# wgurecky/bipymc

Hardware: AMD Instinct MI355X
Metric: chain-updates/sec (higher is better)
Workload: dtype f64

## Files before the change

bipymc_amd/csrc/kernels.h:

```cpp
#pragma once
#ifndef __HIPCC_RTC__
#include <hip/hip_runtime.h>
#include <stdint.h>
#endif

#include "philox.h"
#include "accept_test.h"
#ifndef BPM_ACCEPT_FILTER_DIVERGENT
#define BPM_ACCEPT_FILTER_DIVERGENT 0
#endif

#ifdef BPM_STAMPS
#define BPM_STAMP(i)                                                                          \
    do {                                                                                      \
        __builtin_amdgcn_sched_barrier(0);                                                    \
        unsigned long long _t;                                                                \
        asm volatile("s_memtime %0\n\ts_waitcnt lgkmcnt(0)" : "=s"(_t)::"memory");            \
        __builtin_amdgcn_sched_barrier(0);                                                    \
        bpm_stamp[i] = _t;                                                                    \
    } while (0)
#else
#define BPM_STAMP(i) do { } while (0)
#endif

#if defined(__HIP_DEVICE_COMPILE__) && !defined(__gfx942__) && !defined(__gfx950__)
#error "kernels.h: the ticket hand-overs rely on gfx942 / gfx950 memory behaviour (vmcnt counts stores; agent-scope atomics bypass the L2s): use __ATOMIC_RELEASE / __ATOMIC_ACQUIRE tickets on other targets"
#endif

namespace bpm {
inline namespace BPM_VARIANT_NS {

constexpr int ALGO_DEMC = 0, ALGO_DREAM = 1;
constexpr int TARGET_HOST = 0, TARGET_GAUSS = 1, TARGET_MIXTURE = 2, TARGET_BANANA = 3;
constexpr int STAGE_FUSED = 0, STAGE_PROPOSE = 1, STAGE_COMMIT = 2;
constexpr int WAVE = 64;
#ifndef BPM_BLOCK_WAVE
#define BPM_BLOCK_WAVE 128
#endif
constexpr int block_for(int lpc) { return (lpc == 4 || lpc == 16) ? 256 : BPM_BLOCK_WAVE; }
constexpr bool hot_is_adapt(int hot) { return hot == 3 || hot == 4; }
constexpr bool crp_shape(int lpc, int dpl) { return lpc < WAVE || dpl == 2; }
constexpr int block_for_hot(int lpc, int hot, int dpl) { return (lpc == WAVE && dpl == 2 && hot_is_adapt(hot)) ? 1024 : block_for(lpc); }
constexpr int cr_g1(int lpc) { return lpc == WAVE ? 16 : WAVE / lpc; }
constexpr int MAX_CR = 8;
constexpr int TRACE_I32 = 32;
constexpr int TRACE_F64 = 4;
constexpr int MAX_PARTNERS = 2 * MAX_PAIRS + 3;

struct Layout {
    double* G;
    uint64_t blk;
    uint32_t n_local;
    uint32_t ld;
    uint32_t dim;
    uint32_t world;
    uint32_t magic;
};

__device__ __forceinline__ uint32_t rank_of(const Layout& L, uint32_t c) {
    if (L.world == 1) return 0u;
    uint32_t r = __umulhi(c, L.magic);
    r -= (r * L.n_local > c) ? 1u : 0u;
    return r;
}
__device__ __forceinline__ double* row_ptr(const Layout& L, uint32_t c) {
    return L.G + (c * L.ld + rank_of(L, c) * (2u * L.n_local));
}
__device__ __forceinline__ double* delta_ptr(const Layout& L, uint32_t c) {
    return L.G + (c + rank_of(L, c) * (L.n_local * (L.ld + 1u)) + L.n_local * L.ld);
}
__device__ __forceinline__ double* cridx_ptr(const Layout& L, uint32_t c) {
    return L.G + (c + rank_of(L, c) * (L.n_local * (L.ld + 1u)) + L.n_local * (L.ld + 1u));
}

constexpr int ACC_SHARDS = 1024;
template <int TARGET, int LPC>
constexpr bool lean_scalars() { return LPC < WAVE && TARGET != TARGET_HOST; }
template <int TARGET>
constexpr bool lean_always() { return TARGET == TARGET_BANANA; }

constexpr int PLAN_WORDS = 16;
constexpr int MAX_SEG = 16;
constexpr int MAX_PEERS = MAX_SEG - 1;

constexpr unsigned long long PUSH_CLOSING = 1ull << 62;
constexpr unsigned long long PUSH_ERR_CLOSED = 0x100ull;
struct PushCtrl {
    unsigned long long flag[MAX_SEG];
    unsigned long long err;
    unsigned long long arena_bad[2];
    unsigned long long pad[5];
    unsigned long long probe[MAX_SEG];
};
struct PhaseArgs {
    Layout L;
    double* ll;
    double* hist_row;
    double* llhist_row;
    double* w_mean;
    double* w_m2;
    const double* tparams;
    const double* cr_state;
    unsigned long long* counters;
    uint32_t* acc_count;
    double* prop_buf;
    double* aux_buf;
    int32_t* ids_buf;
#ifdef BPM_TEST_HOOKS
    int32_t* trace_i32;
    double* trace_f64;
    uint8_t* trace_mask;
#endif
    PermKey pk;
    const uint32_t* perm_tab;
    const uint32_t* inv_tab;
    const double* gamma_tab;
    const uint32_t* plan;
    const uint32_t* rec_tab;
    uint32_t rec_off;
    uint32_t thr[MAX_CR];
    unsigned long long* stamps;
    double* pack;
    uint32_t pack_cap, pack_nsub, pack_stride;
    double* x_next;
    uint8_t* accbits;
    const uint8_t* accbits_all;
    uint32_t replay;
    const uint32_t* rec_sorted;
    uint32_t seg_off[MAX_SEG + 1];
    uint32_t n_seg, seg_me;
    uint32_t acc_by_item;
    const unsigned long long* peer_tab;
    uint32_t n_peers;
    uint32_t hist_by_pos;
#ifndef BPM_LEAN_LAST
    uint32_t lean;
#endif
    uint32_t wt;
    uint64_t seed;
    uint64_t t;
    uint32_t k;
    uint32_t N, lo;
    uint32_t upd_off, n_upd, pool_off, M;
    uint32_t mode;
    uint32_t n_items;
    uint32_t algo;
    uint32_t P, n_cr;
    double* cr_part1;
    const double* cr_fold_part;
    const double* cr_fold_tot;
    double* cr_fold_out;
    uint32_t cr_fold_nb;
    uint32_t cr_chunk0, cr_n1;
    uint32_t adapt_on;
    uint32_t cr_gate;
    uint32_t hist_len;
    double gamma_scale, gamma_demc, epsilon, u_epsilon, p_snooker;
#ifdef BPM_LEAN_LAST
    uint32_t lean, pad_lean;
#endif
};

#ifdef BPM_TEST_HOOKS
__host__ __device__ __forceinline__ int32_t* trace_i32_of(const PhaseArgs& a) { return a.trace_i32; }
__host__ __device__ __forceinline__ double* trace_f64_of(const PhaseArgs& a) { return a.trace_f64; }
__host__ __device__ __forceinline__ uint8_t* trace_mask_of(const PhaseArgs& a) { return a.trace_mask; }
__host__ __device__ __forceinline__ void trace_set(PhaseArgs& a, int32_t* i, double* f, uint8_t* m) { a.trace_i32 = i; a.trace_f64 = f; a.trace_mask = m; }
#else
__host__ __device__ constexpr int32_t* trace_i32_of(const PhaseArgs&) { return nullptr; }
__host__ __device__ constexpr double* trace_f64_of(const PhaseArgs&) { return nullptr; }
__host__ __device__ constexpr uint8_t* trace_mask_of(const PhaseArgs&) { return nullptr; }
__host__ __device__ __forceinline__ void trace_set(PhaseArgs&, int32_t*, double*, uint8_t*) {}
#endif

template <int CTRL>
__device__ __forceinline__ int dpp_i32(int v) {
    return __builtin_amdgcn_mov_dpp(v, CTRL, 0xF, 0xF, true);
}
template <int CTRL>
__device__ __forceinline__ double dpp_f64(double v) {
    const int lo = dpp_i32<CTRL>(__double2loint(v));
    const int hi = dpp_i32<CTRL>(__double2hiint(v));
    return __hiloint2double(hi, lo);
}
__device__ __forceinline__ double readlane_f64(double v, int lane) {
    return __hiloint2double(__builtin_amdgcn_readlane(__double2hiint(v), lane),
                            __builtin_amdgcn_readlane(__double2loint(v), lane));
}
constexpr int DPP_ROW_BCAST15 = 0x142, DPP_ROW_BCAST31 = 0x143;
__device__ __forceinline__ double row_sums_step1_f64(double v) { return v + dpp_f64<DPP_ROW_BCAST15>(v); }
__device__ __forceinline__ double row_sums_step2_f64(double v) { return v + dpp_f64<DPP_ROW_BCAST31>(v); }
__device__ __forceinline__ double row_sums_f64(double v) {
    return readlane_f64(row_sums_step2_f64(row_sums_step1_f64(v)), WAVE - 1);
}
template <int LPC>
__device__ __forceinline__ double gsum(double v) {
    static_assert(LPC == 1 || LPC == 4 || LPC == 16 || LPC == 32 || LPC == 64, "subgroup sizes");
    if (LPC >= 4) {
        v += dpp_f64<0xB1>(v);
        v += dpp_f64<0x4E>(v);
    }
    if (LPC >= 16) {
        v += dpp_f64<0x141>(v);
        v += dpp_f64<0x140>(v);
    }
    if (LPC == 32) v += __shfl_xor(v, 16);
    if (LPC == 64) v = row_sums_f64(v);
    return v;
}
template <int LPC>
__device__ __forceinline__ void gsum2(double& v, double& w) {
    static_assert(LPC == 1 || LPC == 4 || LPC == 16 || LPC == 32 || LPC == 64, "subgroup sizes");
    if (LPC >= 4) {
        const double v1 = dpp_f64<0xB1>(v), w1 = dpp_f64<0xB1>(w);
        v += v1; w += w1;
        const double v2 = dpp_f64<0x4E>(v), w2 = dpp_f64<0x4E>(w);
        v += v2; w += w2;
    }
    if (LPC >= 16) {
        const double v3 = dpp_f64<0x141>(v), w3 = dpp_f64<0x141>(w);
        v += v3; w += w3;
        const double v4 = dpp_f64<0x140>(v), w4 = dpp_f64<0x140>(w);
        v += v4; w += w4;
    }
    if (LPC == 32) { const double vs = __shfl_xor(v, 16), ws = __shfl_xor(w, 16); v += vs; w += ws; }
    if (LPC == 64) {
        v = row_sums_step1_f64(v); w = row_sums_step1_f64(w);
        v = row_sums_step2_f64(v); w = row_sums_step2_f64(w);
        v = readlane_f64(v, WAVE - 1); w = readlane_f64(w, WAVE - 1);
    }
}
template <int LPC>
__device__ __forceinline__ int gsum_i(int v) {
    if (LPC >= 4) {
        v += dpp_i32<0xB1>(v);
        v += dpp_i32<0x4E>(v);
    }
    if (LPC >= 16) {
        v += dpp_i32<0x141>(v);
        v += dpp_i32<0x140>(v);
    }
    if (LPC == 32) v += __shfl_xor(v, 16);
    if (LPC == 64) {
        v += dpp_i32<DPP_ROW_BCAST15>(v);
        v += dpp_i32<DPP_ROW_BCAST31>(v);
        v = __builtin_amdgcn_readlane(v, WAVE - 1);
    }
    return v;
}

constexpr uint32_t CR_FINAL_MAX = 512;
__host__ __device__ inline uint32_t cr_chunks_of(uint32_t n_half, uint32_t g1) { return (n_half + g1 - 1u) / g1; }
struct CrTotals { double p[MAX_CR], d[MAX_CR], n[MAX_CR]; };
__device__ __forceinline__ void cr_finalize(bool any, uint32_t n_cr, CrTotals& T) {
    if (!any) return;
    uint32_t nz = 0;
#pragma unroll
    for (int m = 0; m < MAX_CR; ++m) nz += (m < (int)n_cr && T.n[m] != 0.0) ? 1u : 0u;
    if (nz == n_cr) {
#pragma unroll
        for (int m = 0; m < MAX_CR; ++m) if (m < (int)n_cr) T.p[m] = T.d[m] / T.n[m];
    }
    double sum = 0.0;
#pragma unroll
    for (int m = 0; m < MAX_CR; ++m) if (m < (int)n_cr) sum += T.p[m];
#pragma unroll
    for (int m = 0; m < MAX_CR; ++m) if (m < (int)n_cr) T.p[m] = T.p[m] / sum;
}
template <int ROUNDS>
__device__ __forceinline__ double cr_array_sum(const double* arr, uint32_t nb) {
    const uint32_t lane = threadIdx.x & (WAVE - 1);
    double v[ROUNDS];
#pragma unroll
    for (int r = 0; r < ROUNDS; ++r) {
        const uint32_t b = (uint32_t)r * WAVE + lane;
        const double x = arr[b < nb ? b : nb - 1u];
        v[r] = b < nb ? x : 0.0;
    }
    double s = 0.0;
#pragma unroll
    for (int r = 0; r < ROUNDS; ++r) s += v[r];
    return gsum<WAVE>(s);
}
template <int ROUNDS, bool PLAIN = false>
__device__ __forceinline__ void cr_fold(const double* tot, const double* part, uint32_t nb, uint32_t stride, uint32_t n_cr, CrTotals& T) {
    const uint32_t lane = threadIdx.x & (WAVE - 1);
#pragma unroll
    for (int m = 0; m < MAX_CR; ++m) { T.p[m] = tot[m]; T.d[m] = tot[MAX_CR + m]; T.n[m] = tot[2 * MAX_CR + m]; }
    bool any = false;
#pragma unroll
    for (int m0 = 0; m0 < MAX_CR; m0 += 4) {
        if (m0 < (int)n_cr) {
            double vd[4][ROUNDS], vn[4][ROUNDS];
#pragma unroll
            for (int mm = 0; mm < 4; ++mm) {
#pragma unroll
                for (int r = 0; r < ROUNDS; ++r) {
                    const uint32_t b = (uint32_t)r * WAVE + lane;
                    vd[mm][r] = 0.0; vn[mm][r] = 0.0;
                    if (m0 + mm < (int)n_cr && b < nb) {
                        if (PLAIN) {
                            vd[mm][r] = part[(uint64_t)(m0 + mm) * stride + b];
                            vn[mm][r] = part[(uint64_t)(MAX_CR + m0 + mm) * stride + b];
                        } else {
                            vd[mm][r] = __hip_atomic_load(&part[(uint64_t)(m0 + mm) * stride + b], __ATOMIC_RELAXED, __HIP_MEMORY_SCOPE_AGENT);
                            vn[mm][r] = __hip_atomic_load(&part[(uint64_t)(MAX_CR + m0 + mm) * stride + b], __ATOMIC_RELAXED, __HIP_MEMORY_SCOPE_AGENT);
                        }
                    }
                }
            }
#pragma unroll
            for (int mm = 0; mm < 4; ++mm) {
                if (m0 + mm < (int)n_cr) {
// ... 166 lines not shown
template <int LPC, int DPL>
__device__ __forceinline__ void store_row_wt(double* row, int q, uint32_t ld, const double* v) {
#pragma unroll
    for (int u = 0; u < DPL / 2; ++u) {
        const uint32_t pi = (uint32_t)(q + u * LPC);
        if (2 * pi < ld) {
            __hip_atomic_store(row + 2 * pi, v[2 * u], __ATOMIC_RELAXED, __HIP_MEMORY_SCOPE_AGENT);
            __hip_atomic_store(row + 2 * pi + 1, v[2 * u + 1], __ATOMIC_RELAXED, __HIP_MEMORY_SCOPE_AGENT);
        }
    }
}

template <int LPC, int DPL>
__device__ __forceinline__ void store_row_wt16(double* row, int q, uint32_t ld, const double* v) {
#pragma unroll
    for (int u = 0; u < DPL / 2; ++u) {
        const uint32_t pi = (uint32_t)(q + u * LPC);
        if (2 * pi < ld) {
            bpm_d2v t = {v[2 * u], v[2 * u + 1]};
            bpm_d2v* p = reinterpret_cast<bpm_d2v*>(row) + pi;
            asm volatile("global_store_dwordx4 %0, %1, off sc1" ::"v"(p), "v"(t) : "memory");
        }
    }
}

template <int LPC, int DPL>
__device__ __forceinline__ void store_row_sys(double* row, int q, uint32_t ld, const double* v) {
#pragma unroll
    for (int u = 0; u < DPL / 2; ++u) {
        const uint32_t pi = (uint32_t)(q + u * LPC);
        if (2 * pi < ld) {
            __hip_atomic_store(row + 2 * pi, v[2 * u], __ATOMIC_RELAXED, __HIP_MEMORY_SCOPE_SYSTEM);
            __hip_atomic_store(row + 2 * pi + 1, v[2 * u + 1], __ATOMIC_RELAXED, __HIP_MEMORY_SCOPE_SYSTEM);
        }
    }
}

template <int LPC, int DPL>
__device__ __forceinline__ void store_row_stream(double* row, int q, uint32_t ld, const double* v) {
#pragma unroll
    for (int u = 0; u < DPL / 2; ++u) {
        const uint32_t pi = (uint32_t)(q + u * LPC);
        if (2 * pi < ld) {
            bpm_d2v t = {v[2 * u], v[2 * u + 1]};
            __builtin_nontemporal_store(t, reinterpret_cast<bpm_d2v*>(row) + pi);
        }
    }
}

__device__ __forceinline__ void box_muller_pair_f32(uint32_t w1, uint32_t w2, double& n0, double& n1) {
    const float u1 = ((float)w1 + 1.0f) * 2.3283064365386963e-10f;
    const float u2 = (float)w2 * 2.3283064365386963e-10f;
    const float r = __builtin_amdgcn_sqrtf(-2.0f * 0.6931471805599453f * __builtin_amdgcn_logf(u1));
    n0 = (double)(r * __builtin_amdgcn_cosf(u2));
    n1 = (double)(r * __builtin_amdgcn_sinf(u2));
}

template <int K>
__device__ __forceinline__ uint32_t quad_bcast(uint32_t v) {
    return (uint32_t)dpp_i32<K * 0x55>((int)v);
}

template <int LPC, int NPART_CT>
struct Partners {
    uint32_t r[NPART_CT > 0 ? NPART_CT : 1];
    const uint32_t* lds;
    __device__ __forceinline__ uint32_t get(int i) const { return NPART_CT > 0 ? r[i] : lds[i]; }
};

__device__ __forceinline__ uint32_t partner_pos(const PhaseArgs& a, uint32_t c, uint32_t idx, uint32_t n_pair_idx) {
    if (idx < n_pair_idx) {
        const uint32_t p = idx >> 1;
        const u32x4 wb = chain_block(a.seed, c, a.t, SLOT_PAIR0 + (p >> 1));
        uint32_t ia, ib;
        distinct_pair((p & 1) ? wb.z : wb.x, (p & 1) ? wb.w : wb.y, a.M, ia, ib);
        uint32_t pos = (idx & 1) ? ib : ia;
        if (a.mode == 2) pos += (pos >= c) ? 1u : 0u;
        return pos;
    }
    const u32x4 ws = chain_block(a.seed, c, a.t, SLOT_SNK);
    uint32_t iz, i1, i2;
    distinct_three(ws.x, ws.y, ws.z, a.M, iz, i1, i2);
    const uint32_t s = idx - n_pair_idx;
    return s == 0 ? iz : (s == 1 ? i1 : i2);
}

__device__ __forceinline__ uint32_t pos_to_chain(const PhaseArgs& a, uint32_t pos) {
#if defined(BPM_TEST_HOOKS) && defined(BPM_FAKE_NO_PARTNER_HOP)
    return pos;
#else
    return a.perm_tab ? a.perm_tab[pos] : perm_fwd(pos, a.pk);
#endif
}
__device__ __forceinline__ uint32_t own_pos_to_chain(const PhaseArgs& a, uint32_t pos) {
#if defined(BPM_TEST_HOOKS) && defined(BPM_FAKE_NO_OWN_HOP)
    return pos;
#else
    return a.perm_tab ? a.perm_tab[pos] : perm_fwd(pos, a.pk);
#endif
}
__device__ __forceinline__ uint32_t chain_to_pos(const PhaseArgs& a, uint32_t c) {
    return a.inv_tab ? a.inv_tab[c] : perm_inv(c, a.pk);
}

template <int DPL, int NPX>
struct PlanFront {
    uint32_t rec[PLAN_WORDS];
    double x[DPL], ra[NPX][DPL], rb[NPX][DPL];
    double ll_cur, pcr[3], gl[DPL];
    uint32_t acc_prev;
};
typedef uint32_t bpm_u32x16 __attribute__((ext_vector_type(16)));
__device__ __forceinline__ bpm_u32x16 plan_record(const uint32_t* recp) {
    return *reinterpret_cast<const bpm_u32x16*>(__builtin_assume_aligned(recp, 4 * PLAN_WORDS));
}
template <int DPL, int NP>
__device__ __forceinline__ void plan_front(const Layout& L, const bpm_u32x16 rv, int q, PlanFront<DPL, (NP > 0 ? NP : 1)>& fr) {
    static_assert(PLAN_WORDS == 16 && DPL == 2, "one 64-byte record, one 16-byte load per lane and row");
#pragma unroll
    for (int i = 0; i < PLAN_WORDS; ++i) fr.rec[i] = rv[i];
    typedef const __attribute__((address_space(1))) bpm_d2v* grow_t;
    const double* base[1 + 2 * (NP > 0 ? NP : 1)];
    base[0] = row_ptr(L, fr.rec[0]);
#pragma unroll
    for (int i = 0; i < 2 * NP; ++i) base[1 + i] = row_ptr(L, fr.rec[5 + i]);
#ifndef BPM_STAMPS
#pragma unroll
    for (int i = 0; i < 1 + 2 * NP; ++i) asm("" : "+s"(base[i]));
#endif
    const uint32_t last = (L.ld >> 1) - 1u, pi = (uint32_t)q < last ? (uint32_t)q : last;
    bpm_d2v t = ((grow_t)base[0])[pi];
    fr.x[0] = t.x; fr.x[1] = t.y;
#pragma unroll
    for (int p = 0; p < NP; ++p) {
        t = ((grow_t)base[1 + 2 * p])[pi];
        fr.ra[p][0] = t.x; fr.ra[p][1] = t.y;
        t = ((grow_t)base[2 + 2 * p])[pi];
        fr.rb[p][0] = t.x; fr.rb[p][1] = t.y;
    }
    __builtin_amdgcn_sched_barrier(0);
}

struct NoEarly { template <class W> __device__ __forceinline__ void operator()(W&) const {} };
struct PcrGiven { bool on = false; double p[MAX_CR]; };
template <int ALGO, int LPC, int DPL, int NP, int LOAD_LL = 1 , class EARLY = NoEarly, bool FRONT = false>
__device__ __forceinline__ void make_proposal(const PhaseArgs& a, uint32_t c, bool active, int q, int cw,
                                              uint32_t* s_part, Work<DPL>& wk, const uint32_t* rec = nullptr,
                                              unsigned long long* bpm_stamp = nullptr, EARLY early = EARLY(), const PcrGiven pcr_ovr = PcrGiven(),
                                              const PlanFront<DPL, (NP > 0 ? NP : 1)>* fr = nullptr) {
    static_assert(!FRONT || (LPC == WAVE && DPL == 2), "the planned front serves one wavefront per chain with one coordinate pair per lane");
    constexpr bool DREAM = ALGO == ALGO_DREAM;
    constexpr bool FAST = (NP > 0) && (LPC == 1);
    constexpr bool SNK_DIRECT = (LPC == 1);
    const uint32_t dim = a.L.dim, ld = a.L.ld;
    const uint32_t P = NP > 0 ? (uint32_t)NP : a.P;
    if constexpr (FRONT) {
        const bool in_row = 2u * (uint32_t)q < ld;
#pragma unroll
        for (int s = 0; s < DPL; ++s) wk.x[s] = in_row ? fr->x[s] : 0.0;
    } else
    load_row<LPC, DPL>(row_ptr(a.L, c), q, ld, wk.x);
    wk.ll_cur = 0.0;
    wk.acc_prev = 0u;
    if (!a.replay) {
#if defined(BPM_TEST_HOOKS) && defined(BPM_FAKE_NO_LL)
        if (LPC < WAVE) wk.ll_cur = wk.x[0] * 1e-300; else
#endif
        if constexpr (FRONT) wk.ll_cur = fr->ll_cur; else
        if (LOAD_LL == 1 || (LOAD_LL == 2 && !a.lean)) wk.ll_cur = a.ll[c - a.lo];
        if constexpr (FRONT) wk.acc_prev = fr->acc_prev; else
        if (LPC == WAVE) wk.acc_prev = a.acc_count[c - a.lo];
    }
    if (DREAM && a.adapt_on) {
        load_row<LPC, DPL>(a.w_mean + (uint32_t)((c - a.lo) * 2u * ld), q, ld, wk.w_mean);
        load_row<LPC, DPL>(a.w_m2 + (uint32_t)((c - a.lo) * 2u * ld), q, ld, wk.w_m2);
    }
    double pcr[MAX_CR];
    if (DREAM) {
#pragma unroll
        for (int m = 0; m < MAX_CR; ++m)
            pcr[m] = pcr_ovr.on ? pcr_ovr.p[m] : (FRONT ? (m < 3 ? fr->pcr[m < 3 ? m : 0] : 0.0) : a.cr_state[m]);
    }
    double gtab[DPL];
    if (DREAM && LPC == WAVE) {
#pragma unroll
        for (int u = 0; u < DPL; ++u) {
            const uint32_t gi = (uint32_t)(q + u * WAVE);
            const double gl = FRONT ? fr->gl[u] : a.gamma_tab[gi <= dim ? gi : dim];
            gtab[u] = (FRONT || gi <= dim) ? gl : 0.0;
        }
    }
    double gt_lane = 0.0;
    if (DREAM && LPC * DPL < WAVE) {
        const uint32_t wl = (uint32_t)threadIdx.x & (uint32_t)(WAVE - 1);
        gt_lane = a.gamma_tab[wl <= dim ? wl : dim];
    }
    const bool snk_possible = !DREAM && a.p_snooker > 0.0 && a.M >= 3;
    const uint32_t npart = 2 * P + (snk_possible ? 3u : 0u);
    constexpr bool RL = (LPC == WAVE) && (NP > 0) && !FAST;
    const uint32_t npairs = (dim + 1u) >> 1;
    const bool merged = !FRONT && RL && DPL == 2 && (npairs + 2u * (uint32_t)NP + 1u <= (uint32_t)WAVE);
    u32x4 wpair[DPL / 2];
    u32x4 h0;
    constexpr bool QUAD = DREAM && LPC == 4 && DPL == 2 && NP == 3;
    constexpr bool REGS = FAST || RL || QUAD;
    Partners<LPC, REGS ? 2 * NP : 0> part;
    part.lds = s_part + cw * MAX_PARTNERS;
    const bool planned = FRONT || ((LPC == WAVE) && rec != nullptr);
    const bool dims_late = planned && RL && DPL == 2;
    if (FRONT) {
        h0.x = fr->rec[1]; h0.y = fr->rec[2]; h0.z = fr->rec[3]; h0.w = fr->rec[4];
#pragma unroll
        for (int i = 0; i < 2 * NP; ++i) part.r[i] = fr->rec[5 + i];
        if (!dims_late) {
#pragma unroll
            for (int u = 0; u < DPL / 2; ++u) wpair[u] = chain_block<true>(a.seed, c, a.t, SLOT_DIM0 + (uint32_t)(q + u * LPC));
        }
    } else if (planned) {
        h0.x = rec[1]; h0.y = rec[2]; h0.z = rec[3]; h0.w = rec[4];
        if (FAST || RL) {
#pragma unroll
            for (int i = 0; i < 2 * NP; ++i) part.r[i] = rec[5 + i];
        }
        if (!dims_late) {
#pragma unroll
            for (int u = 0; u < DPL / 2; ++u) wpair[u] = chain_block<true>(a.seed, c, a.t, SLOT_DIM0 + (uint32_t)(q + u * LPC));
        }
    } else if (merged) {
        const uint32_t uq = (uint32_t)q, hdr_lane = npairs + 2u * (uint32_t)NP;
        const uint32_t pidx = uq - npairs;
        const uint32_t slot = uq < npairs ? SLOT_DIM0 + uq : (uq < hdr_lane ? SLOT_PAIR0 + (pidx >> 2) : SLOT_HDR0);
        const u32x4 wb = chain_block<true>(a.seed, c, a.t, slot);
        wpair[0] = wb;
        h0.x = (uint32_t)__builtin_amdgcn_readlane((int)wb.x, hdr_lane);
        h0.y = (uint32_t)__builtin_amdgcn_readlane((int)wb.y, hdr_lane);
        h0.z = (uint32_t)__builtin_amdgcn_readlane((int)wb.z, hdr_lane);
        h0.w = (uint32_t)__builtin_amdgcn_readlane((int)wb.w, hdr_lane);
        BPM_STAMP(2);
        uint32_t mine = 0;
        if (uq >= npairs && uq < hdr_lane) {
            const uint32_t p = pidx >> 1;
            uint32_t ia, ib;
            distinct_pair((p & 1) ? wb.z : wb.x, (p & 1) ? wb.w : wb.y, a.M, ia, ib);
            uint32_t pos = (pidx & 1) ? ib : ia;
            if (a.mode == 2) pos += (pos >= c) ? 1u : 0u;
            mine = pos_to_chain(a, a.pool_off + pos);
        }
#pragma unroll
        for (int i = 0; i < 2 * NP; ++i) part.r[i] = (uint32_t)__builtin_amdgcn_readlane((int)mine, npairs + i);
    } else if (QUAD) {
        wpair[0] = chain_block<true>(a.seed, c, a.t, SLOT_DIM0 + (uint32_t)q);
        const u32x4 wb = chain_block<true>(a.seed, c, a.t, q == 1 ? SLOT_PAIR0 : (q == 2 ? SLOT_PAIR0 + 1u : SLOT_HDR0));
        h0.x = quad_bcast<0>(wb.x); h0.y = quad_bcast<0>(wb.y); h0.z = quad_bcast<0>(wb.z); h0.w = quad_bcast<0>(wb.w);
        uint32_t i0 = 0, i1 = 0, i2 = 0, i3 = 0;
        if (q == 1 || q == 2) {
            uint32_t ia, ib;
            distinct_pair(wb.x, wb.y, a.M, ia, ib);
            i0 = pos_to_chain(a, a.pool_off + ia); i1 = pos_to_chain(a, a.pool_off + ib);
            if (q == 1) {
                distinct_pair(wb.z, wb.w, a.M, ia, ib);
                i2 = pos_to_chain(a, a.pool_off + ia); i3 = pos_to_chain(a, a.pool_off + ib);
            }
        }
        part.r[0] = quad_bcast<1>(i0); part.r[1] = quad_bcast<1>(i1); part.r[2] = quad_bcast<1>(i2); part.r[3] = quad_bcast<1>(i3);
        part.r[4] = quad_bcast<2>(i0); part.r[5] = quad_bcast<2>(i1);
    } else {
        h0 = chain_block<(LPC < WAVE)>(a.seed, c, a.t, SLOT_HDR0);
#pragma unroll
        for (int u = 0; u < DPL / 2; ++u) wpair[u] = chain_block<true>(a.seed, c, a.t, SLOT_DIM0 + (uint32_t)(q + u * LPC));
        if (FAST) {
#pragma unroll
            for (int i = 0; i < 2 * NP; ++i) part.r[i] = pos_to_chain(a, a.pool_off + partner_pos(a, c, (uint32_t)i, 2u * NP));
        }
        if (RL) {
            uint32_t mine = 0;
            if (q < 2 * NP) mine = pos_to_chain(a, a.pool_off + partner_pos(a, c, (uint32_t)q, 2u * NP));
#pragma unroll
            for (int i = 0; i < 2 * NP; ++i) part.r[i] = (uint32_t)__builtin_amdgcn_readlane((int)mine, i);
        }
    }
    BPM_STAMP(3);
    wk.u_acc = u01_53(h0.z, h0.w);
    const double u_sel = (double)(h0.x >> 16) * 1.52587890625e-05;
    const double u_gam = (double)(h0.x & 0xFFFFu) * 1.52587890625e-05;
    uint32_t snk_id[3] = {0u, 0u, 0u};
    if (SNK_DIRECT && snk_possible && planned) {
        snk_id[0] = rec[5 + 2 * P]; snk_id[1] = rec[6 + 2 * P]; snk_id[2] = rec[7 + 2 * P];
    } else if (SNK_DIRECT && snk_possible && (u_sel < a.p_snooker || trace_i32_of(a) != nullptr)) {
        const u32x4 ws = chain_block(a.seed, c, a.t, SLOT_SNK);
        uint32_t iz, i1, i2;
        distinct_three(ws.x, ws.y, ws.z, a.M, iz, i1, i2);
        snk_id[0] = pos_to_chain(a, a.pool_off + iz);
        snk_id[1] = pos_to_chain(a, a.pool_off + i1);
        snk_id[2] = pos_to_chain(a, a.pool_off + i2);
    }
    if (!REGS || (snk_possible && !SNK_DIRECT)) {
#pragma unroll 1
        for (uint32_t idx = (uint32_t)q; idx < npart; idx += LPC)
            s_part[cw * MAX_PARTNERS + idx] = planned ? rec[5 + idx] : pos_to_chain(a, a.pool_off + partner_pos(a, c, idx, 2 * P));
        __builtin_amdgcn_fence(__ATOMIC_RELEASE, "wavefront");
        __builtin_amdgcn_wave_barrier();
        __builtin_amdgcn_fence(__ATOMIC_ACQUIRE, "wavefront");
    }

    constexpr int NPX = NP > 0 ? NP : 1;
    double ra[NPX][DPL], rb[NPX][DPL];
    if (FRONT && DREAM && NP > 0) {
#pragma unroll
        for (int p = 0; p < NP; ++p) {
#pragma unroll
            for (int s = 0; s < DPL; ++s) { ra[p][s] = fr->ra[p][s]; rb[p][s] = fr->rb[p][s]; }
        }
    } else if (DREAM && NP > 0) {
#pragma unroll
        for (int p = 0; p < NP; ++p) {
            if (LPC == WAVE) {
                load_row_all<LPC, DPL>(row_ptr(a.L, part.get(2 * p)), q, ld, ra[p]);
                load_row_all<LPC, DPL>(row_ptr(a.L, part.get(2 * p + 1)), q, ld, rb[p]);
            } else {
                load_row<LPC, DPL>(row_ptr(a.L, part.get(2 * p)), q, ld, ra[p]);
                load_row<LPC, DPL>(row_ptr(a.L, part.get(2 * p + 1)), q, ld, rb[p]);
            }
        }
    }
    if (!FRONT) BPM_STAMP(7);
    if (dims_late) wpair[0] = chain_block<true>(a.seed, c, a.t, SLOT_DIM0 + (uint32_t)q);
    if (DREAM) early(wk);

    double eps_n[DPL], eps_u[DPL];
    uint32_t maskbits = 0;
    wk.cr_idx = -1; wk.d_prime = (int)dim; wk.jump = 0; wk.snk = 0; wk.delta = 0.0; wk.log_corr = 0.0;
    uint32_t thr = 65536u;
    if (DREAM) {
        const double uc = u_sel;
        double cum = 0.0;
        int idx = (int)a.n_cr - 1;
        bool found = false;
#pragma unroll
        for (int m = 0; m < MAX_CR; ++m) {
            if (m < (int)a.n_cr) {
                cum += pcr[m];
                if (!found && uc < cum) { idx = m; thr = a.thr[m]; found = true; }
            }
        }
        if (!found) {
#pragma unroll
            for (int m = 0; m < MAX_CR; ++m) if (m == (int)a.n_cr - 1) thr = a.thr[m];
        }
        wk.cr_idx = idx;
    }
    int cnt = 0;
#pragma unroll
    for (int u = 0; u < DPL / 2; ++u) {
        const uint32_t pi = (uint32_t)(q + u * LPC);
        const uint32_t j0 = 2u * pi;
        eps_n[2 * u] = 0.0; eps_n[2 * u + 1] = 0.0; eps_u[2 * u] = 0.0; eps_u[2 * u + 1] = 0.0;
        if (j0 < dim) {
            const u32x4 wj = wpair[u];
            const bool two = j0 + 1 < dim;
            const bool two_eps = two || (FRONT && DREAM);
            if (a.epsilon > 0.0) {
                double n0, n1;
                box_muller_pair_f32(wj.z, wj.w, n0, n1);
                eps_n[2 * u] = a.epsilon * n0;
                if (two_eps) eps_n[2 * u + 1] = a.epsilon * n1;
            }
            if (DREAM) {
                if (a.u_epsilon > 0.0) {
                    eps_u[2 * u] = -a.u_epsilon + (2.0 * a.u_epsilon) * (((double)(wj.y >> 16) + 0.5) * 1.52587890625e-05);
                    if (two_eps) eps_u[2 * u + 1] = -a.u_epsilon + (2.0 * a.u_epsilon) * (((double)(wj.y & 0xFFFFu) + 0.5) * 1.52587890625e-05);
                }
                if ((wj.x >> 16) <= thr) { maskbits |= 1u << (2 * u); ++cnt; }
                if (two && (wj.x & 0xFFFFu) <= thr) { maskbits |= 1u << (2 * u + 1); ++cnt; }
            }
        }
    }
    if (DREAM) {
        if (LPC == WAVE) {
            cnt = 0;
#pragma unroll
            for (int sb = 0; sb < DPL; ++sb) cnt += (int)__popcll(__ballot((maskbits >> sb) & 1u));
        } else {
            cnt = gsum_i<LPC>(cnt);
        }
        if (cnt == 0) {
            const uint32_t f = mulhi32(h0.y, dim);
#pragma unroll
            for (int s = 0; s < DPL; ++s) {
                const uint32_t j = 2u * (uint32_t)(q + (s >> 1) * LPC) + (s & 1);
                if (j == f) maskbits |= 1u << s;
            }
            cnt = 1;
        }
        wk.d_prime = cnt;
    }
    wk.maskbits = maskbits;

    if (DREAM) {
        double gamma;
        if (LPC == WAVE && (uint32_t)cnt < (uint32_t)(WAVE * DPL)) {
            double gsel = gtab[0];
#pragma unroll
            for (int u = 1; u < DPL; ++u) gsel = ((cnt >> 6) == u) ? gtab[u] : gsel;
            gamma = readlane_f64(gsel, cnt & 63);
        } else if (LPC * DPL < WAVE) {
            gamma = __shfl(gt_lane, cnt);
        } else {
            gamma = a.gamma_tab[cnt];
        }
        if (a.k % 5 == 0 && !(u_gam < 0.2)) { gamma = 1.0; wk.jump = 1; }
        wk.gamma = gamma;
        if (LPC == WAVE) {
            int u_hi = __builtin_amdgcn_readfirstlane(__double2hiint(wk.u_acc)), u_lo = __builtin_amdgcn_readfirstlane(__double2loint(wk.u_acc));
            asm volatile("" : "+s"(u_hi), "+s"(u_lo));
            wk.u_acc = __hiloint2double(u_hi, u_lo);
            asm volatile("" ::"s"(a.wt), "s"(a.hist_by_pos), "s"(a.upd_off), "s"(a.hist_row), "s"(a.llhist_row), "s"(a.ll), "s"(a.acc_count));
        }
        double sum[DPL];
        if (NP > 0) {
#pragma unroll
            for (int s = 0; s < DPL; ++s) {
                sum[s] = ra[0][s] - rb[0][s];
#pragma unroll
                for (int p = 1; p < NP; ++p) sum[s] = sum[s] + (ra[p][s] - rb[p][s]);
            }
        } else {
#pragma unroll
            for (int s = 0; s < DPL; ++s) sum[s] = 0.0;
#pragma unroll 1
            for (uint32_t p = 0; p < P; ++p) {
                double ra[DPL], rb[DPL];
                load_row<LPC, DPL>(row_ptr(a.L, part.lds[2 * p]), q, ld, ra);
                load_row<LPC, DPL>(row_ptr(a.L, part.lds[2 * p + 1]), q, ld, rb);
#pragma unroll
                for (int s = 0; s < DPL; ++s) sum[s] = (p == 0) ? (ra[s] - rb[s]) : (sum[s] + (ra[s] - rb[s]));
            }
        }
#pragma unroll
        for (int s = 0; s < DPL; ++s) {
            const double jump = (1.0 + eps_u[s]) * gamma * sum[s] + eps_n[s];
            wk.p[s] = ((maskbits >> s) & 1u) ? (jump + wk.x[s]) : wk.x[s];
        }
        BPM_STAMP(4);
        if (a.adapt_on && a.cr_gate) {
            const double* m2 = wk.w_m2;
            double dl = 0.0;
#pragma unroll
            for (int s = 0; s < DPL; ++s) {
                const uint32_t j = 2u * (uint32_t)(q + (s >> 1) * LPC) + (s & 1);
                if (j < dim) {
                    const double df = wk.x[s] - wk.p[s];
                    dl += m2[s] > 0.0 ? (df * df * (double)a.hist_len) / m2[s] : (df * df) / 1e-24;
                }
            }
            wk.delta = gsum<LPC>(dl);
        }
    } else {
        double gamma = a.gamma_demc;
        if (a.mode != 2 && a.k % 10 == 0 && !(u_gam < 0.1)) { gamma = 1.0; wk.jump = 1; }
        wk.gamma = gamma;
        double ra[DPL], rb[DPL];
        const bool ids_in_regs = REGS && (!snk_possible || SNK_DIRECT);
        const uint32_t ca = ids_in_regs ? part.get(0) : part.lds[0];
        const uint32_t cb = ids_in_regs ? part.get(1) : part.lds[1];
        const bool do_snk = snk_possible && u_sel < a.p_snooker;
        if (LPC == 1) asm volatile("" ::"v"(ca), "v"(cb), "v"(snk_id[0]), "v"(snk_id[1]), "v"(snk_id[2]));
        if constexpr (FRONT && NP == 1) {
            const bool in_row = 2u * (uint32_t)q < ld;
#pragma unroll
            for (int s = 0; s < DPL; ++s) { ra[s] = in_row ? fr->ra[0][s] : 0.0; rb[s] = in_row ? fr->rb[0][s] : 0.0; }
        } else {
        load_row<LPC, DPL>(row_ptr(a.L, ca), q, ld, ra);
        load_row<LPC, DPL>(row_ptr(a.L, cb), q, ld, rb);
        }
        double rz[DPL], r1[DPL], r2[DPL];
#pragma unroll
        for (int s = 0; s < DPL; ++s) { rz[s] = 0.0; r1[s] = 0.0; r2[s] = 0.0; }
        if (do_snk) {
            load_row<LPC, DPL>(row_ptr(a.L, SNK_DIRECT ? snk_id[0] : part.lds[2]), q, ld, rz);
            load_row<LPC, DPL>(row_ptr(a.L, SNK_DIRECT ? snk_id[1] : part.lds[3]), q, ld, r1);
            load_row<LPC, DPL>(row_ptr(a.L, SNK_DIRECT ? snk_id[2] : part.lds[4]), q, ld, r2);
        }
        early(wk);
#pragma unroll
        for (int s = 0; s < DPL; ++s) {
            double pv = gamma * (ra[s] - rb[s]);
            pv = pv + wk.x[s];
            pv = pv + eps_n[s];
            wk.p[s] = pv;
        }
        if (do_snk) {
            double n2 = 0.0, dot = 0.0;
#pragma unroll
            for (int s = 0; s < DPL; ++s) {
                const double df = wk.x[s] - rz[s];
                n2 += df * df;
                dot += (r1[s] - r2[s]) * df;
            }
            n2 = gsum<LPC>(n2);
            dot = gsum<LPC>(dot);
            if (n2 > 0.0) {
                const double gs = (1.2 + u01_32(h0.y)) * (dot / n2);
                double n2p = 0.0;
#pragma unroll
                for (int s = 0; s < DPL; ++s) {
                    const uint32_t j = 2u * (uint32_t)(q + (s >> 1) * LPC) + (s & 1);
                    const double df = wk.x[s] - rz[s];
                    double pv = wk.x[s] + gs * df;
                    pv = pv + eps_n[s];
                    if (j >= dim) pv = wk.x[s];
                    wk.p[s] = pv;
                    const double dn = pv - rz[s];
                    n2p += dn * dn;
                }
                n2p = gsum<LPC>(n2p);
                wk.log_corr = 0.5 * (double)(dim - 1) * (log(n2p) - log(n2));
                wk.snk = 1;
            }
        }
    }
    if (trace_i32_of(a) && active) {
        if (q == 0) {
            int32_t* tr = trace_i32_of(a) + (uint64_t)(c - a.lo) * TRACE_I32;
            tr[0] = wk.cr_idx; tr[1] = wk.d_prime; tr[2] = wk.jump; tr[4] = wk.snk;
            if (REGS) {
#pragma unroll
                for (int i = 0; i < 2 * NP; ++i) tr[5 + i] = (int32_t)part.get(i);
            }
            const bool regs = REGS && (!snk_possible || SNK_DIRECT);
#pragma unroll 1
            for (uint32_t i = regs ? 2u * P : 0u; i < MAX_PARTNERS; ++i) {
                int32_t v = -1;
                const uint32_t ks = i - 2u * P;
                if (i < npart) v = regs ? (int32_t)(ks == 1u ? snk_id[1] : (ks == 2u ? snk_id[2] : snk_id[0])) : (int32_t)part.lds[i];
                tr[5 + i] = v;
            }
        }
        if (trace_mask_of(a)) {
#pragma unroll
            for (int s = 0; s < DPL; ++s) {
                const uint32_t j = 2u * (uint32_t)(q + (s >> 1) * LPC) + (s & 1);
                if (j < dim) trace_mask_of(a)[(uint64_t)(c - a.lo) * dim + j] = (uint8_t)((maskbits >> s) & 1u);
            }
        }
    }
}

template <int ALGO, int LPC, int DPL, int LEAN = 0 , bool CRP_W = false>
__device__ __forceinline__ void finish_update(const PhaseArgs& a, uint32_t c, bool active, int q,
                                              const Work<DPL>& wk, double ll_prop) {
    const uint32_t ld = a.L.ld;
    const uint32_t li = c - a.lo;
    const double ll_cur = wk.ll_cur;
    const double d_acc = (ll_prop + wk.log_corr) - ll_cur;
    bool is_nan;
    constexpr bool FILTER = LPC == WAVE || BPM_ACCEPT_FILTER_DIVERGENT != 0;
    const bool accepted = FILTER ? accept_test(d_acc, wk.u_acc, &is_nan) : accept_exact(d_acc, wk.u_acc, &is_nan);
    const bool lean = LEAN == 2 || (LEAN == 1 && a.lean != 0u);
    if (lean) {
        const unsigned long long m = __ballot(active && accepted && q == 0);
        if ((threadIdx.x & (WAVE - 1)) == 0 && m != 0ull)
            __hip_atomic_fetch_add(&a.acc_count[a.L.n_local + ((blockIdx.x * (blockDim.x / WAVE) + (threadIdx.x / WAVE)) & (ACC_SHARDS - 1))],
                                   (uint32_t)__popcll(m), __ATOMIC_RELAXED, __HIP_MEMORY_SCOPE_AGENT);
    }
    if (!active) return;
    double nv[DPL];
#pragma unroll
    for (int s = 0; s < DPL; ++s) nv[s] = accepted ? wk.p[s] : wk.x[s];
    const double new_ll = accepted ? ll_prop : ll_cur;
    const uint32_t hi = a.hist_by_pos ? wk.pos_own : li;
    if (LPC == WAVE && a.hist_row) store_row_stream<LPC, DPL>(a.hist_row + (uint32_t)(hi * ld), q, ld, nv);
    if (q == 0) {
        if (accepted && !lean) {
#if defined(BPM_TEST_HOOKS) && defined(BPM_FAKE_NO_LL)
            if (LPC < WAVE) {} else
#endif
            if (LPC < WAVE) __hip_atomic_fetch_add(&a.acc_count[li], 1u, __ATOMIC_RELAXED, __HIP_MEMORY_SCOPE_AGENT);
            else if (a.wt) __hip_atomic_store(&a.acc_count[li], wk.acc_prev + 1u, __ATOMIC_RELAXED, __HIP_MEMORY_SCOPE_AGENT);
            else a.acc_count[li] = wk.acc_prev + 1u;
        }
        if (is_nan) atomicAdd(&a.counters[2], 1ull);
        if (a.accbits) a.accbits[a.acc_by_item ? wk.item : li] = accepted ? (uint8_t)1 : (uint8_t)0;
    }
    if (a.x_next) {
        store_row<LPC, DPL>(a.x_next + (uint32_t)(li * ld), q, ld, nv);
        if (accepted && q == 0 && !lean) a.ll[li] = new_ll;
    } else if (accepted) {
        if (a.wt == 2u) {
            store_row_wt16<LPC, DPL>(row_ptr(a.L, c), q, ld, nv);
#if defined(BPM_TEST_HOOKS) && defined(BPM_FAKE_NO_LL)
            if (LPC < WAVE) {} else
#endif
            if (q == 0 && !lean) __hip_atomic_store(&a.ll[li], new_ll, __ATOMIC_RELAXED, __HIP_MEMORY_SCOPE_AGENT);
        } else if (a.wt) {
            store_row_wt<LPC, DPL>(row_ptr(a.L, c), q, ld, nv);
            if (q == 0 && !lean) __hip_atomic_store(&a.ll[li], new_ll, __ATOMIC_RELAXED, __HIP_MEMORY_SCOPE_AGENT);
        } else {
            store_row<LPC, DPL>(row_ptr(a.L, c), q, ld, nv);
            if (q == 0 && !lean) a.ll[li] = new_ll;
        }
    }
    if (a.pack && accepted) {
        double* sub = a.pack + (uint32_t)((li & (a.pack_nsub - 1u)) * a.pack_stride);
        uint32_t slot = 0;
        if (q == 0) slot = atomicAdd(reinterpret_cast<uint32_t*>(sub), 1u);
        slot = __shfl(slot, (threadIdx.x & (WAVE - 1)) - q);
        if (slot < a.pack_cap) {
            if (q == 0) sub[2 + slot] = (double)c;
            store_row<LPC, DPL>(sub + 2 + a.pack_cap + (uint32_t)(slot * ld), q, ld, nv);
        }
    }
    if (a.n_peers) {
        const uint32_t row_off = (uint32_t)(row_ptr(a.L, c) - a.L.G);
        const bool slots = ALGO == ALGO_DREAM && a.adapt_on && a.cr_gate && q == 0;
        const uint32_t d_off = (uint32_t)(delta_ptr(a.L, c) - a.L.G), c_off = (uint32_t)(cridx_ptr(a.L, c) - a.L.G);
        const bool gated = a.adapt_on && a.cr_gate;
#pragma unroll 1
        for (uint32_t p = 0; p < a.n_peers; ++p) {
            double* pg = reinterpret_cast<double*>(a.peer_tab[p]);
            if (accepted) store_row_sys<LPC, DPL>(pg + row_off, q, ld, nv);
            if (slots) {
                __hip_atomic_store(pg + d_off, gated ? wk.delta : 0.0, __ATOMIC_RELAXED, __HIP_MEMORY_SCOPE_SYSTEM);
                __hip_atomic_store(pg + c_off, gated ? (double)wk.cr_idx : -1.0, __ATOMIC_RELAXED, __HIP_MEMORY_SCOPE_SYSTEM);
            }
        }
    }
    if (LPC != WAVE && a.hist_row) store_row_stream<LPC, DPL>(a.hist_row + (uint32_t)(hi * ld), q, ld, nv);
    if (a.llhist_row && q == 0) {
        double* dst_ll = &a.llhist_row[a.hist_by_pos == 1u ? wk.pos_own : li];
        if (LPC < WAVE) __builtin_nontemporal_store(new_ll, dst_ll); else *dst_ll = new_ll;
    }
    if (ALGO == ALGO_DREAM) {
        if (a.adapt_on) {
            double mean[DPL], m2[DPL];
#pragma unroll
            for (int s = 0; s < DPL; ++s) { mean[s] = wk.w_mean[s]; m2[s] = wk.w_m2[s]; }
            const double cntp = (double)(a.hist_len + 1);
#pragma unroll
            for (int s = 0; s < DPL; ++s) {
                const double d1 = nv[s] - mean[s];
                mean[s] = mean[s] + d1 / cntp;
                m2[s] = m2[s] + d1 * (nv[s] - mean[s]);
            }
            if (a.wt) {
                store_row_wt16<LPC, DPL>(a.w_mean + (uint32_t)(li * 2u * ld), q, ld, mean);
                store_row_wt16<LPC, DPL>(a.w_m2 + (uint32_t)(li * 2u * ld), q, ld, m2);
            } else {
                store_row_stream<LPC, DPL>(a.w_mean + (uint32_t)(li * 2u * ld), q, ld, mean);
                store_row_stream<LPC, DPL>(a.w_m2 + (uint32_t)(li * 2u * ld), q, ld, m2);
            }
        }
        if (q == 0 && a.adapt_on && !(CRP_W && a.cr_part1 != nullptr)) {
            const bool gated = a.adapt_on && a.cr_gate;
            if (a.wt) {
                __hip_atomic_store(delta_ptr(a.L, c), gated ? wk.delta : 0.0, __ATOMIC_RELAXED, __HIP_MEMORY_SCOPE_AGENT);
                __hip_atomic_store(cridx_ptr(a.L, c), gated ? (double)wk.cr_idx : -1.0, __ATOMIC_RELAXED, __HIP_MEMORY_SCOPE_AGENT);
            } else {
                *delta_ptr(a.L, c) = gated ? wk.delta : 0.0;
                *cridx_ptr(a.L, c) = gated ? (double)wk.cr_idx : -1.0;
            }
        }
    }
    if (trace_i32_of(a) && q == 0) {
        trace_i32_of(a)[(uint64_t)li * TRACE_I32 + 3] = accepted ? 1 : 0;
        double* tf = trace_f64_of(a) + (uint64_t)li * TRACE_F64;
        bool nan_alpha;
        tf[0] = accept_alpha(d_acc, &nan_alpha); tf[1] = ll_prop; tf[2] = wk.delta; tf[3] = wk.gamma;
    }
    if (a.n_peers) asm volatile("s_waitcnt vmcnt(0)" ::: "memory");
}

template <int LPC>
__device__ __forceinline__ void pin_args(const PhaseArgs& a) {
    if (LPC != WAVE) {
        asm volatile("" ::"s"(a.L.G), "s"(a.L.ld), "s"(a.L.dim), "s"(a.ll), "s"(a.hist_row), "s"(a.llhist_row), "s"(a.tparams),
                     "s"(a.cr_state), "s"(a.acc_count), "s"(a.perm_tab), "s"(a.inv_tab), "s"(a.gamma_tab), "s"(a.plan), "s"(a.pack),
                     "s"(a.thr[0]), "s"(a.thr[1]), "s"(a.thr[2]), "s"(a.seed), "s"(a.t), "s"(a.k), "s"(a.N),
                     "s"(a.lo), "s"(a.upd_off), "s"(a.n_upd), "s"(a.pool_off), "s"(a.M), "s"(a.mode), "s"(a.n_items), "s"(a.n_cr));
        asm volatile("" ::"s"(a.adapt_on), "s"(a.cr_gate), "s"(a.hist_len), "s"(a.epsilon), "s"(a.u_epsilon), "s"(a.L.n_local),
                     "s"(a.L.world), "s"(a.L.magic), "s"(a.counters), "s"(a.pack_cap), "s"(a.pack_nsub), "s"(a.pack_stride));
    }
}

__device__ __forceinline__ bool resolve_chain(const PhaseArgs& a, uint32_t w, uint32_t& c) {
    bool active = w < a.n_items;
    if (a.mode == 0) {
        c = own_pos_to_chain(a, a.upd_off + (active ? w : 0u));
    } else if (a.mode == 2) {
        c = a.lo + (active ? w : 0u);
    } else {
        c = a.lo + (active ? w : 0u);
        const uint32_t pos = chain_to_pos(a, c);
        active = active && (pos - a.upd_off) < a.n_upd;
    }
    return active;
}

#ifdef BPM_STAMPS
__host__ inline bool stamps_allow_hot(const PhaseArgs&) { return true; }
#else
__host__ inline bool stamps_allow_hot(const PhaseArgs& a) { return a.stamps == nullptr; }
#endif
enum Flavour {
    FLAVOUR_GENERAL = 0,
    FLAVOUR_STEADY_PLAN = 1,
    FLAVOUR_STEADY = 2,
    FLAVOUR_ADAPT_PLAN = 3,
    FLAVOUR_ADAPT = 4,
    FLAVOUR_SHARD_PLAN = 5,
    N_FLAVOURS = 7
};
__host__ inline Flavour choose_flavour(const PhaseArgs& a, bool dream, bool can_plan) {
    const bool plan = can_plan && a.rec_tab != nullptr;
    if (!(a.mode == 0 && (a.rec_tab != nullptr) == plan && trace_i32_of(a) == nullptr && a.pack == nullptr && a.x_next == nullptr && a.epsilon > 0.0 &&
          a.perm_tab != nullptr && a.inv_tab != nullptr && a.replay == 0 && (!dream || (a.u_epsilon > 0.0 && a.n_cr == 3))))
        return FLAVOUR_GENERAL;
    const bool single = a.n_peers == 0 && a.L.world == 1 && a.lo == 0 && stamps_allow_hot(a) && a.accbits == nullptr;
    if (single && a.adapt_on == 0) return plan ? FLAVOUR_STEADY_PLAN : FLAVOUR_STEADY;
    if (plan && a.adapt_on == 0 && a.L.world > 1 && a.stamps == nullptr && (a.accbits != nullptr || a.n_peers > 0)) return FLAVOUR_SHARD_PLAN;
    if (single && a.adapt_on != 0 && dream) return plan ? FLAVOUR_ADAPT_PLAN : FLAVOUR_ADAPT;
    return FLAVOUR_GENERAL;
}
constexpr bool flavour_is_steady(int f) { return f == FLAVOUR_STEADY_PLAN || f == FLAVOUR_STEADY; }
template <int ALGO, int TARGET, int LPC, int DPL, int NP, int HOT = 0>
__global__ __launch_bounds__(block_for_hot(LPC, HOT, DPL)) void phase_fused_kernel(
#ifdef BPM_PRELOAD
    const uint32_t* pl_plan, uint32_t pl_upd_off, uint32_t pl_n_items, uint32_t pl_mode,
#endif
    const PhaseArgs a_in) {
    constexpr bool COPY = (HOT != 0);
    constexpr bool SHARD = (HOT == 5 || HOT == 6), ADAPT = (HOT == 3 || HOT == 4), NOPLAN = (HOT == 2 || HOT == 4 || HOT == 6);
    constexpr bool FRONT_CT = LPC == WAVE && DPL == 2 && (HOT == 1 || HOT == 3 || HOT == 5);
#ifdef BPM_PRELOAD
    if (HOT) { __builtin_assume(pl_mode == 0u); __builtin_assume((pl_plan != nullptr) == !NOPLAN); }
#else
    const uint32_t* pl_plan = (HOT && NOPLAN) ? nullptr : a_in.rec_tab;
    const uint32_t pl_upd_off = a_in.rec_off, pl_n_items = a_in.n_items, pl_mode = HOT ? 0u : a_in.mode;
#endif
    constexpr int BLK = block_for_hot(LPC, HOT, DPL);
    constexpr bool CRP = ALGO == ALGO_DREAM && hot_is_adapt(HOT) && crp_shape(LPC, DPL);
    __shared__ uint32_t s_part[(BLK / LPC) * MAX_PARTNERS];
    const int lane = threadIdx.x;
    const int cw = lane / LPC, q = lane % LPC;
    const uint32_t w = blockIdx.x * (BLK / LPC) + cw;
#ifdef BPM_STAMPS
    unsigned long long bpm_stamp[8] = {0, 0, 0, 0, 0, 0, 0, 0};
    unsigned long long bpm_rt0;
    asm volatile("s_memrealtime %0\n\ts_waitcnt lgkmcnt(0)" : "=s"(bpm_rt0)::"memory");
    BPM_STAMP(0);
#endif
    PlanFront<DPL, (NP > 0 ? NP : 1)> fr;
    uint32_t f_c = 0u;
    const uint32_t* f_rec = nullptr;
    Layout f_L = {};
    double *f_ll = nullptr, *f_wm = nullptr, *f_w2 = nullptr;
    const double *f_crs = nullptr, *f_tp = nullptr, *f_gt = nullptr;
    uint32_t* f_acc = nullptr;
    unsigned long long* f_cnt = nullptr;
    uint32_t f_lo = 0u;
    typename Target<TARGET, LPC, DPL>::Consts tc_front;
    if constexpr (FRONT_CT) {
        if (w < pl_n_items) {
            f_L = a_in.L;
            if (SHARD) __builtin_assume(f_L.world > 1u); else f_L.world = 1;
            typedef uint32_t u32x4_a4 __attribute__((ext_vector_type(4), aligned(4)));
            typedef uint32_t u32x2_a4 __attribute__((ext_vector_type(2), aligned(4)));
            u32x4_a4 lw4 = {0u, 0u, 0u, 0u};
            u32x2_a4 lw2 = {0u, 0u};
            if (SHARD) {
                lw4 = *reinterpret_cast<const u32x4_a4*>(&a_in.L.n_local);
                lw2 = *reinterpret_cast<const u32x2_a4*>(&a_in.L.magic);
                f_L.n_local = lw4.x; f_L.ld = lw4.y; f_L.dim = lw4.z; f_L.world = lw4.w; f_L.magic = lw2.x;
                __builtin_assume(f_L.world > 1u);
            }
            f_ll = a_in.ll; f_acc = a_in.acc_count; f_crs = a_in.cr_state; f_tp = a_in.tparams; f_gt = a_in.gamma_tab; f_cnt = a_in.counters;
            if (ADAPT) { f_wm = a_in.w_mean; f_w2 = a_in.w_m2; }
            if (SHARD) f_lo = a_in.lo;
            const uint32_t pos = (uint32_t)__builtin_amdgcn_readfirstlane((int)(pl_upd_off + w));
            f_rec = pl_plan + (uint32_t)(pos * PLAN_WORDS);
            bpm_u32x16 rv = plan_record(f_rec);
#ifndef BPM_STAMPS
#define BPM_FRONT_ALL "s"(f_L.G), "s"(f_L.ld), "s"(f_L.dim), "s"(f_ll), "s"(f_acc), "s"(f_tp), "s"(f_cnt), "s"(a_in.seed), "s"(a_in.t), "s"(a_in.k), "s"(a_in.upd_off), \
                      "s"(a_in.epsilon), "s"(a_in.wt), "s"(a_in.hist_by_pos), "s"(a_in.hist_row), "s"(a_in.llhist_row)
#define BPM_FRONT_DREAM "s"(f_crs), "s"(f_gt), "s"(a_in.u_epsilon), "s"(a_in.thr[0]), "s"(a_in.thr[1]), "s"(a_in.thr[2]), "s"(a_in.thr[3])
            if (ALGO == ALGO_DREAM && ADAPT) asm("" : "+s"(rv) : BPM_FRONT_ALL, BPM_FRONT_DREAM, "s"(f_wm), "s"(f_w2), "s"(a_in.cr_gate), "s"(a_in.hist_len));
            else if (ALGO == ALGO_DREAM && SHARD) asm("" : "+s"(rv) : BPM_FRONT_ALL, BPM_FRONT_DREAM, "s"(f_lo), "s"(lw4), "s"(lw2));
            else if (ALGO == ALGO_DREAM) asm("" : "+s"(rv) : BPM_FRONT_ALL, BPM_FRONT_DREAM);
            else if (SHARD) asm("" : "+s"(rv) : BPM_FRONT_ALL, "s"(a_in.gamma_demc), "s"(a_in.p_snooker), "s"(a_in.M), "s"(a_in.pool_off), "s"(f_lo), "s"(lw4), "s"(lw2));
            else asm("" : "+s"(rv) : BPM_FRONT_ALL, "s"(a_in.gamma_demc), "s"(a_in.p_snooker), "s"(a_in.M), "s"(a_in.pool_off));
#undef BPM_FRONT_ALL
#undef BPM_FRONT_DREAM
#endif
            __builtin_amdgcn_sched_barrier(0);
            f_c = rv[0];
            fr.ll_cur = f_ll[f_c - f_lo];
            fr.acc_prev = f_acc[f_c - f_lo];
            if (ALGO == ALGO_DREAM) {
#pragma unroll
                for (int m = 0; m < 3; ++m) fr.pcr[m] = f_crs[m];
#pragma unroll
                for (int u = 0; u < DPL; ++u) {
                    const uint32_t gi = (uint32_t)(q + u * WAVE);
                    fr.gl[u] = f_gt[gi <= f_L.dim ? gi : f_L.dim];
                }
            }
            tc_front = Target<TARGET, LPC, DPL>::load(q, f_L.dim, f_tp);
            plan_front<DPL, NP>(f_L, rv, q, fr);
#ifndef BPM_STAMPS
            if constexpr (ALGO == ALGO_DREAM && TARGET == TARGET_GAUSS)
                asm("" : "+s"(f_c) : "s"(fr.ll_cur), "s"(fr.acc_prev), "s"(fr.pcr[0]), "s"(fr.pcr[1]), "s"(fr.pcr[2]), "s"(tc_front.c0), "s"(tc_front.a), "s"(tc_front.b));
            else if (ALGO == ALGO_DREAM) asm("" : "+s"(f_c) : "s"(fr.ll_cur), "s"(fr.acc_prev), "s"(fr.pcr[0]), "s"(fr.pcr[1]), "s"(fr.pcr[2]));
            else if constexpr (TARGET == TARGET_GAUSS) asm("" : "+s"(f_c) : "s"(fr.ll_cur), "s"(fr.acc_prev), "s"(tc_front.c0), "s"(tc_front.a), "s"(tc_front.b));
            else asm("" : "+s"(f_c) : "s"(fr.ll_cur), "s"(fr.acc_prev));
#endif
#ifdef BPM_STAMPS
            BPM_STAMP(7);
#endif
        } else if (!CRP) {
            return;
        }
    }
    PhaseArgs a_hot;
    if (COPY) {
        if constexpr (FRONT_CT) {
            a_hot = a_in;
            a_hot.L = f_L; a_hot.ll = f_ll; a_hot.acc_count = f_acc; a_hot.cr_state = f_crs; a_hot.tparams = f_tp; a_hot.gamma_tab = f_gt; a_hot.counters = f_cnt;
            if (ADAPT) { a_hot.w_mean = f_wm; a_hot.w_m2 = f_w2; }
            if (SHARD) a_hot.lo = f_lo;
        } else
        a_hot = a_in;
        a_hot.mode = 0u; trace_set(a_hot, nullptr, nullptr, nullptr); a_hot.pack = nullptr;
        a_hot.replay = 0u; a_hot.x_next = nullptr; a_hot.adapt_on = ADAPT ? 1u : 0u;
#ifndef BPM_STAMPS
        a_hot.stamps = nullptr;
#else
        if (SHARD) a_hot.stamps = nullptr;
#endif
        if (!ADAPT) a_hot.cr_fold_part = nullptr;
        if (!SHARD) { a_hot.accbits = nullptr; a_hot.lo = 0; a_hot.L.world = 1; a_hot.acc_by_item = 0u; a_hot.n_peers = 0u; a_hot.peer_tab = nullptr; }
        if (ALGO == ALGO_DREAM) a_hot.n_cr = 3;
        if (NOPLAN) { a_hot.plan = nullptr; a_hot.rec_tab = nullptr; }
    }
    const PhaseArgs& a = COPY ? a_hot : a_in;
    static_assert(!FRONT_CT || COPY, "the planned front reads the argument block through the private copy");
    if (HOT) {
        __builtin_assume(a_in.mode == 0u); __builtin_assume(a_in.pack == nullptr);
#ifdef BPM_TEST_HOOKS
        __builtin_assume(a_in.trace_i32 == nullptr);
#endif
        __builtin_assume(a_in.x_next == nullptr); __builtin_assume(a_in.adapt_on == (ADAPT ? 1u : 0u));
#ifndef BPM_STAMPS
        __builtin_assume(a_in.stamps == nullptr);
#endif
        if (!SHARD) { __builtin_assume(a_in.lo == 0); __builtin_assume(a_in.L.world == 1); }
        __builtin_assume(a_in.epsilon > 0.0);
        __builtin_assume(a_in.perm_tab != nullptr); __builtin_assume(a_in.inv_tab != nullptr);
        if (ALGO == ALGO_DREAM) { __builtin_assume(a_in.u_epsilon > 0.0); __builtin_assume(a_in.n_cr == 3); }
    }
    pin_args<LPC>(a);
    uint32_t c;
    bool active;
    const uint32_t* rec = nullptr;
    bool run = true;
    double cr_d = 0.0;
    int cr_i = -1;
    if constexpr (FRONT_CT) {
        active = w < pl_n_items;
        c = f_c;
        rec = f_rec;
    } else if (LPC == WAVE && pl_plan && !(CRP && w >= pl_n_items)) {
        active = w < pl_n_items;
        if (!active) return;
        uint32_t pos;
        if (pl_mode == 0) {
            pos = pl_upd_off + w;
        } else {
            pos = a.inv_tab[a.lo + w];
            if ((pos - pl_upd_off) >= a.n_upd) return;
        }
        pos = __builtin_amdgcn_readfirstlane(pos);
        rec = pl_plan + (uint32_t)(pos * PLAN_WORDS);
        c = rec[0];
    } else {
        active = resolve_chain(a, w, c);
    }
    if (LPC == WAVE && !active) {
        if (CRP) run = false; else return;
    }
    PcrGiven pcr_fold;
    if constexpr (CRP) {
        pcr_fold.on = a.cr_fold_part != nullptr;
        if (pcr_fold.on) {
            __shared__ double s_tot[2 * MAX_CR];
            constexpr uint32_t NWV = (uint32_t)(BLK / WAVE);
            const uint32_t n_cr = a.n_cr, wv = (uint32_t)lane / (uint32_t)WAVE;
            for (uint32_t k = wv; k < 2u * n_cr; k += NWV) {
                const uint32_t arr = k < n_cr ? k : (uint32_t)MAX_CR + (k - n_cr);
                const double tsum = cr_array_sum<CR_FINAL_MAX / WAVE>(a.cr_fold_part + (uint64_t)arr * a.cr_fold_nb, a.cr_fold_nb);
                if ((lane & (WAVE - 1)) == 0) s_tot[arr] = tsum;
            }
            __syncthreads();
            CrTotals T;
#pragma unroll
            for (int m = 0; m < MAX_CR; ++m) { T.p[m] = a.cr_fold_tot[m]; T.d[m] = a.cr_fold_tot[MAX_CR + m]; T.n[m] = a.cr_fold_tot[2 * MAX_CR + m]; }
            bool any = false;
#pragma unroll
            for (int m = 0; m < MAX_CR; ++m) {
                if (m < (int)n_cr) {
                    const double td = s_tot[m], tn = s_tot[MAX_CR + m];
                    if (tn > 0.0) { any = true; T.n[m] += tn; T.d[m] += td; }
                }
            }
            cr_finalize(any, n_cr, T);
            if (blockIdx.x == 0 && lane == 0) cr_write_totals(T, n_cr, a.cr_fold_out);
#pragma unroll
            for (int m = 0; m < MAX_CR; ++m)
                pcr_fold.p[m] = __hiloint2double(__builtin_amdgcn_readfirstlane(__double2hiint(T.p[m])), __builtin_amdgcn_readfirstlane(__double2loint(T.p[m])));
        }
    }
  if (run) {
    if (LPC == WAVE) c = __builtin_amdgcn_readfirstlane(c);
    const typename Target<TARGET, LPC, DPL>::Consts tc = FRONT_CT ? tc_front : Target<TARGET, LPC, DPL>::load(q, a.L.dim, a.tparams);
    Work<DPL> wk;
    wk.item = w;
    wk.pos_own = a.upd_off + (active ? w : 0u);
    if (LPC == WAVE) wk.pos_own = (uint32_t)__builtin_amdgcn_readfirstlane((int)wk.pos_own);
    constexpr bool LEAN = lean_scalars<TARGET, LPC>();
    const uint32_t dim_early = a.L.dim;
    constexpr bool LEAN_CT = LEAN && lean_always<TARGET>();
#ifdef BPM_STAMPS
    bpm_stamp[1] = 0; BPM_STAMP(1);
    unsigned long long* const stamp_arg = bpm_stamp;
#else
    unsigned long long* const stamp_arg = nullptr;
#endif
    if constexpr (LEAN) {
        const bool lean_early = LEAN_CT || a.lean != 0u;
        auto early = [tc, q, dim_early, lean_early](Work<DPL>& k) { if (lean_early) k.ll_cur = Target<TARGET, LPC, DPL>::eval(k.x, q, dim_early, tc); };
        make_proposal<ALGO, LPC, DPL, NP, (LEAN_CT ? 0 : 2)>(a, c, active, q, cw, s_part, wk, rec, stamp_arg, early, pcr_fold);
    } else if constexpr (CRP) {
        make_proposal<ALGO, LPC, DPL, NP, 1, NoEarly, FRONT_CT>(a, c, active, q, cw, s_part, wk, rec, stamp_arg, NoEarly(), pcr_fold, &fr);
    } else {
        make_proposal<ALGO, LPC, DPL, NP, 1, NoEarly, FRONT_CT>(a, c, active, q, cw, s_part, wk, rec, stamp_arg, NoEarly(), PcrGiven(), &fr);
    }
    double ll_prop;
    if constexpr (FRONT_CT && TARGET == TARGET_GAUSS && ALGO == ALGO_DREAM) ll_prop = Target<TARGET_GAUSS, LPC, DPL>::template eval<true>(wk.p, q, a.L.dim, tc);
    else ll_prop = Target<TARGET, LPC, DPL>::eval(wk.p, q, a.L.dim, tc);
    BPM_STAMP(5);
    finish_update<ALGO, LPC, DPL, (LEAN_CT ? 2 : (LEAN ? 1 : 0)), CRP>(a, c, active, q, wk, ll_prop);
    if (CRP && active && a.adapt_on && a.cr_gate) { cr_d = wk.delta; cr_i = wk.cr_idx; }
    BPM_STAMP(6);
#ifdef BPM_STAMPS
    if (bpm_stamp[2] == 0) { bpm_stamp[2] = bpm_rt0; bpm_stamp[1] = bpm_stamp[7]; }
    {
        unsigned long long rt;
        asm volatile("s_memrealtime %0\n\ts_waitcnt lgkmcnt(0)" : "=s"(rt)::"memory");
        bpm_stamp[7] = (rt & 0x0FFFFFFFFFFFFFFFull) | ((unsigned long long)(__builtin_amdgcn_s_getreg((31 << 11) | 20) & 0xF) << 60);
    }
    if (a.stamps && lane == 0) for (int i = 0; i < 8; ++i) a.stamps[(uint64_t)w * 8 + i] = bpm_stamp[i];
#endif
  }
    if (CRP && a.cr_part1) {
        constexpr int G1 = cr_g1(LPC);
        if (LPC == WAVE) {
            __shared__ double s_crd[G1];
            __shared__ int s_cri[G1];
            if (q == 0) { s_crd[cw] = cr_d; s_cri[cw] = cr_i; }
            __syncthreads();
            if (cw == 0 && q < (int)a.n_cr) {
                double sd = 0.0, sn = 0.0;
#pragma unroll
                for (int k = 0; k < G1; ++k) cr_chunk_add(sd, sn, q, s_cri[k], s_crd[k]);
                const uint32_t ch = a.cr_chunk0 + blockIdx.x;
                __hip_atomic_store(&a.cr_part1[(uint64_t)q * a.cr_n1 + ch], sd, __ATOMIC_RELAXED, __HIP_MEMORY_SCOPE_AGENT);
                __hip_atomic_store(&a.cr_part1[(uint64_t)(MAX_CR + q) * a.cr_n1 + ch], sn, __ATOMIC_RELAXED, __HIP_MEMORY_SCOPE_AGENT);
            }
        } else {
            const int wl = lane & (WAVE - 1);
            double sd = 0.0, sn = 0.0;
#pragma unroll
            for (int k = 0; k < G1; ++k) {
                const double dk = readlane_f64(cr_d, k * LPC);
                const int ik = __builtin_amdgcn_readlane(cr_i, k * LPC);
                cr_chunk_add(sd, sn, wl, ik, dk);
            }
            const uint32_t ch = a.cr_chunk0 + (blockIdx.x * (BLK / WAVE) + (uint32_t)(lane / WAVE));
            if (wl < (int)a.n_cr && (ch - a.cr_chunk0) * (uint32_t)G1 < a.n_items) {
                __hip_atomic_store(&a.cr_part1[(uint64_t)wl * a.cr_n1 + ch], sd, __ATOMIC_RELAXED, __HIP_MEMORY_SCOPE_AGENT);
                __hip_atomic_store(&a.cr_part1[(uint64_t)(MAX_CR + wl) * a.cr_n1 + ch], sn, __ATOMIC_RELAXED, __HIP_MEMORY_SCOPE_AGENT);
            }
        }
    }
}

template <int ALGO, int LPC, int DPL, int NP>
__global__ __launch_bounds__(block_for(LPC)) void phase_replay_kernel(const PhaseArgs a_in) {
    PhaseArgs a_rep;
    if (LPC == WAVE) {
        a_rep = a_in;
        a_rep.replay = 1u; a_rep.adapt_on = 0u; trace_set(a_rep, nullptr, nullptr, nullptr);
        a_rep.pack = nullptr; a_rep.x_next = nullptr; a_rep.stamps = nullptr; a_rep.mode = 1u; a_rep.n_peers = 0u;
    }
    const PhaseArgs& a = (LPC == WAVE) ? a_rep : a_in;
    __shared__ uint32_t s_part[(block_for(LPC) / LPC) * MAX_PARTNERS];
    const int lane = threadIdx.x;
    const int cw = lane / LPC, q = lane % LPC;
    const uint32_t w = blockIdx.x * (block_for(LPC) / LPC) + cw;
    bool active = w < a.n_upd;
    uint32_t pos = a.upd_off + (active ? w : 0u);
    const uint32_t* rec = nullptr;
    uint32_t c;
    if (LPC == WAVE && a.plan) {
        if (!active) return;
        pos = __builtin_amdgcn_readfirstlane(pos);
        rec = a.plan + (uint32_t)(pos * PLAN_WORDS);
        c = rec[0];
    } else {
        c = pos_to_chain(a, pos);
    }
    active = active && (c - a.lo) >= a.L.n_local && a.accbits_all[c] != 0;
    if (LPC == WAVE && !active) return;
    if (LPC == WAVE) c = __builtin_amdgcn_readfirstlane(c);
    Work<DPL> wk;
    make_proposal<ALGO, LPC, DPL, NP>(a, c, active, q, cw, s_part, wk, rec);
    if (active) store_row<LPC, DPL>(row_ptr(a.L, c), q, a.L.ld, wk.p);
}

#ifndef BPM_REPLAY_WG
#define BPM_REPLAY_WG 256
#endif
constexpr int REPLAY_WG = BPM_REPLAY_WG;
template <int ALGO, int DPL, int NP>
__global__ __launch_bounds__(REPLAY_WG) void phase_replay_sorted_kernel(const PhaseArgs a_in) {
    constexpr int LPC = WAVE;
    PhaseArgs a_rep = a_in;
    a_rep.replay = 1u; a_rep.adapt_on = 0u; trace_set(a_rep, nullptr, nullptr, nullptr);
    a_rep.pack = nullptr; a_rep.x_next = nullptr; a_rep.stamps = nullptr; a_rep.mode = 1u; a_rep.accbits = nullptr;
    const PhaseArgs& a = a_rep;
    __shared__ uint32_t s_part[(REPLAY_WG / WAVE) * MAX_PARTNERS];
    const int lane = threadIdx.x % WAVE, wv = threadIdx.x / WAVE;
    const uint32_t r = blockIdx.y, k = blockIdx.x * (REPLAY_WG / WAVE) + (uint32_t)__builtin_amdgcn_readfirstlane(wv);
    const uint32_t lo = a_in.seg_off[r], hi = a_in.seg_off[r + 1];
    if (r == a_in.seg_me || k >= hi - lo) return;
    const uint32_t e = lo + k;
    const uint32_t* rec = a.rec_sorted + (uint32_t)(e * PLAN_WORDS);
    const uint32_t acc = a.accbits_all[(uint64_t)r * a.L.n_local + k];
    uint32_t c = rec[0];
    if (acc == 0u) return;
    c = (uint32_t)__builtin_amdgcn_readfirstlane((int)c);
    Work<DPL> wk;
    make_proposal<ALGO, LPC, DPL, NP>(a, c, true, lane, wv, s_part, wk, rec);
    store_row<LPC, DPL>(row_ptr(a.L, c), lane, a.L.ld, wk.p);
}

template <int ALGO, int LPC, int DPL, int NP = 0>
__global__ __launch_bounds__(block_for(LPC)) void phase_propose_kernel(const PhaseArgs a) {
    __shared__ uint32_t s_part[(block_for(LPC) / LPC) * MAX_PARTNERS];
    const int lane = threadIdx.x;
    const int cw = lane / LPC, q = lane % LPC;
    const uint32_t w = blockIdx.x * (block_for(LPC) / LPC) + cw;
    uint32_t c;
    const bool active = resolve_chain(a, w, c);
    if (w < a.n_items && q == 0) a.ids_buf[w] = active ? (int32_t)c : -1;
    if (LPC == WAVE && !active) return;
    if (LPC == WAVE) c = __builtin_amdgcn_readfirstlane(c);
    Work<DPL> wk;
    make_proposal<ALGO, LPC, DPL, NP>(a, c, active, q, cw, s_part, wk);
    if (!active) return;
    store_row<LPC, DPL>(a.prop_buf + (uint64_t)w * a.L.ld, q, a.L.ld, wk.p);
    if (q == 0) {
        a.aux_buf[w] = wk.log_corr;
        if (ALGO == ALGO_DREAM) {
            const bool gated = a.adapt_on && a.cr_gate;
            *delta_ptr(a.L, c) = gated ? wk.delta : 0.0;
            *cridx_ptr(a.L, c) = gated ? (double)wk.cr_idx : -1.0;
        }
    }
}

template <int ALGO, int LPC, int DPL>
__global__ __launch_bounds__(block_for(LPC)) void phase_commit_kernel(const PhaseArgs a) {
    const int lane = threadIdx.x;
    const int cw = lane / LPC, q = lane % LPC;
    const uint32_t w = blockIdx.x * (block_for(LPC) / LPC) + cw;
    bool active = w < a.n_items;
    int32_t id = active ? a.ids_buf[w] : -1;
    active = active && id >= 0;
    if (LPC == WAVE && !active) return;
    const uint32_t c = active ? (uint32_t)id : a.lo;
    Work<DPL> wk;
    load_row<LPC, DPL>(row_ptr(a.L, c), q, a.L.ld, wk.x);
    load_row<LPC, DPL>(a.prop_buf + (uint64_t)(active ? w : 0u) * a.L.ld, q, a.L.ld, wk.p);
    wk.log_corr = active ? a.aux_buf[w] : 0.0;
    wk.ll_cur = a.ll[c - a.lo];
    wk.acc_prev = a.acc_count[c - a.lo];
    if (ALGO == ALGO_DREAM && a.adapt_on) {
        load_row<LPC, DPL>(a.w_mean + (uint32_t)((c - a.lo) * 2u * a.L.ld), q, a.L.ld, wk.w_mean);
        load_row<LPC, DPL>(a.w_m2 + (uint32_t)((c - a.lo) * 2u * a.L.ld), q, a.L.ld, wk.w_m2);
    }
    const double ll_prop = active ? a.aux_buf[a.L.n_local + w] : 0.0;
    const u32x4 h0 = chain_block(a.seed, c, a.t, SLOT_HDR0);
    wk.u_acc = u01_53(h0.z, h0.w);
    wk.delta = 0.0; wk.gamma = 0.0; wk.cr_idx = -1; wk.d_prime = 0; wk.jump = 0; wk.snk = 0; wk.maskbits = 0; wk.item = w; wk.pos_own = 0u;
    if (ALGO == ALGO_DREAM && active) {
        wk.delta = *delta_ptr(a.L, c);
        wk.cr_idx = (int)*cridx_ptr(a.L, c);
    }
    PhaseArgs b = a;
    if (ALGO == ALGO_DREAM) b.cr_gate = (wk.cr_idx >= 0) ? 1u : 0u;
    finish_update<ALGO, LPC, DPL>(b, c, active, q, wk, ll_prop);
}

constexpr int CR_L1_THREADS = 256;
template <int G1, int J>
__device__ __forceinline__ int cr_bcast_i(int v) {
    if (G1 == 4) return dpp_i32<J * 0x55>(v);
    if (G1 == 16) return dpp_i32<0x150 + J>(v);
    return __builtin_amdgcn_readlane(v, J);
}
template <int G1, int J>
__device__ __forceinline__ void cr_l1_steps(int idx, double dl, int m0, double& sd0, double& sn0, double& sd1, double& sn1) {
    const int ij = cr_bcast_i<G1, J>(idx);
    const double dj = __hiloint2double(cr_bcast_i<G1, J>(__double2hiint(dl)), cr_bcast_i<G1, J>(__double2loint(dl)));
    cr_chunk_add(sd0, sn0, m0, ij, dj);
    if (G1 == 4) cr_chunk_add(sd1, sn1, m0 + 4, ij, dj);
    if constexpr (J + 1 < G1) cr_l1_steps<G1, J + 1>(idx, dl, m0, sd0, sn0, sd1, sn1);
}
template <int G1>
__global__ __launch_bounds__(CR_L1_THREADS) void cr_level1_kernel(Layout L, PermKey pk, const uint32_t* perm_tab, uint32_t N, uint32_t n_cr, uint32_t n1, double* part1) {
    const uint32_t t = blockIdx.x * CR_L1_THREADS + threadIdx.x;
    const uint32_t ch = t / G1, k = t % G1;
    const uint32_t n_first = (N + 1u) / 2u, c_first = cr_chunks_of(n_first, G1);
    const bool second = ch >= c_first;
    const uint32_t pos = second ? n_first + (ch - c_first) * G1 + k : ch * G1 + k;
    const bool valid = ch < n1 && pos < (second ? N : n_first);
    int idx = -1;
    double dl = 0.0;
    if (valid) {
        const uint32_t c = perm_tab ? perm_tab[pos] : perm_fwd(pos, pk);
        idx = (int)*cridx_ptr(L, c);
        dl = *delta_ptr(L, c);
    }
    static_assert(MAX_CR <= 8, "a chunk's lanes cover the CR values: lane k sums value k (and k + 4 when G1 == 4)");
    double sd0 = 0.0, sn0 = 0.0, sd1 = 0.0, sn1 = 0.0;
    cr_l1_steps<G1, 0>(idx, dl, (int)k, sd0, sn0, sd1, sn1);
    if (ch < n1) {
        if (k < n_cr) {
            __hip_atomic_store(&part1[(uint64_t)k * n1 + ch], sd0, __ATOMIC_RELAXED, __HIP_MEMORY_SCOPE_AGENT);
            __hip_atomic_store(&part1[(uint64_t)(MAX_CR + k) * n1 + ch], sn0, __ATOMIC_RELAXED, __HIP_MEMORY_SCOPE_AGENT);
        }
        if (G1 == 4 && k + 4u < n_cr) {
            __hip_atomic_store(&part1[(uint64_t)(k + 4u) * n1 + ch], sd1, __ATOMIC_RELAXED, __HIP_MEMORY_SCOPE_AGENT);
            __hip_atomic_store(&part1[(uint64_t)(MAX_CR + k + 4u) * n1 + ch], sn1, __ATOMIC_RELAXED, __HIP_MEMORY_SCOPE_AGENT);
        }
    }
}
__global__ __launch_bounds__(WAVE) void cr_mid_kernel(const double* part1, uint32_t n1, uint32_t n_cr, uint32_t n2, double* part2) {
    const uint32_t g = blockIdx.x, lane = threadIdx.x, b = g * WAVE + lane;
#pragma unroll
    for (int m = 0; m < MAX_CR; ++m) {
        if (m < (int)n_cr) {
            double d = 0.0, n = 0.0;
            if (b < n1) {
                d = __hip_atomic_load(&part1[(uint64_t)m * n1 + b], __ATOMIC_RELAXED, __HIP_MEMORY_SCOPE_AGENT);
                n = __hip_atomic_load(&part1[(uint64_t)(MAX_CR + m) * n1 + b], __ATOMIC_RELAXED, __HIP_MEMORY_SCOPE_AGENT);
            }
            d = gsum<WAVE>(d);
            n = gsum<WAVE>(n);
            if (lane == 0) {
                __hip_atomic_store(&part2[(uint64_t)m * n2 + g], d, __ATOMIC_RELAXED, __HIP_MEMORY_SCOPE_AGENT);
                __hip_atomic_store(&part2[(uint64_t)(MAX_CR + m) * n2 + g], n, __ATOMIC_RELAXED, __HIP_MEMORY_SCOPE_AGENT);
            }
        }
    }
}
template <int ROUNDS>
__global__ __launch_bounds__(WAVE) void cr_final_kernel(const double* tot, const double* part, uint32_t nb, uint32_t n_cr, double* cr_state) {
    CrTotals T;
    cr_fold<ROUNDS>(tot, part, nb, nb, n_cr, T);
    if (threadIdx.x == 0) cr_write_totals(T, n_cr, cr_state);
}

__global__ __launch_bounds__(WAVE) void exchange_scatter_kernel(Layout L, double* PK, uint32_t nsub, uint32_t stride, uint32_t cap,
                                                              uint32_t me, uint32_t* xstat) {
    const uint32_t sb = blockIdx.x / cap, slot = blockIdx.x % cap, r = blockIdx.y;
    double* blk = PK + ((uint64_t)r * nsub + sb) * stride;
    const uint32_t cnt = *reinterpret_cast<const uint32_t*>(blk);
    if (slot == 0 && threadIdx.x == 0) {
        if (cnt > cap) atomicOr(&xstat[0], 1u);
        atomicMax(&xstat[1], cnt);
    }
    if (r == me) {
        if (slot == 0 && threadIdx.x == 0) *reinterpret_cast<uint32_t*>(blk) = 0u;
        return;
    }
    if (slot >= cnt) return;
    const uint32_t id = (uint32_t)blk[2 + slot];
    const double* src = blk + 2 + cap + (uint64_t)slot * L.ld;
    double* dst = row_ptr(L, id);
    for (uint32_t j = threadIdx.x; j < L.ld; j += WAVE) dst[j] = src[j];
}

__global__ __launch_bounds__(WAVE) void queue_fence_kernel(uint32_t* sink) {
    if (sink && threadIdx.x == 0xffffu) *sink = blockIdx.x;
}

__global__ __launch_bounds__(WAVE) void push_sync_kernel(PushCtrl* mine, const unsigned long long* ctrl_tab, uint32_t world, uint32_t me,
                                                         unsigned long long seq, uint32_t do_notify, uint32_t do_wait,
                                                         unsigned long long timeout_ticks) {
    const uint32_t p = threadIdx.x;
    if (p >= world || p == me) return;
    if (do_notify) {
        PushCtrl* pc = reinterpret_cast<PushCtrl*>(ctrl_tab[p]);
        __hip_atomic_store(&pc->flag[me], seq, __ATOMIC_RELAXED, __HIP_MEMORY_SCOPE_SYSTEM);
    }
    if (do_wait) {
        if (__hip_atomic_load(&mine->err, __ATOMIC_RELAXED, __HIP_MEMORY_SCOPE_SYSTEM) != 0ull) return;
        const unsigned long long t0 = wall_clock64();
        for (;;) {
            const unsigned long long v = __hip_atomic_load(&mine->flag[p], __ATOMIC_RELAXED, __HIP_MEMORY_SCOPE_SYSTEM);
            if (v >= PUSH_CLOSING) {
                __hip_atomic_store(&mine->err, PUSH_ERR_CLOSED + p, __ATOMIC_RELAXED, __HIP_MEMORY_SCOPE_SYSTEM);
                break;
            }
            if (v >= seq) break;
            if (wall_clock64() - t0 > timeout_ticks) {
                __hip_atomic_store(&mine->err, 1ull + p, __ATOMIC_RELAXED, __HIP_MEMORY_SCOPE_SYSTEM);
                break;
            }
            __builtin_amdgcn_s_sleep(8);
        }
    }
}

__global__ __launch_bounds__(WAVE) void push_close_kernel(PushCtrl* mine, const unsigned long long* ctrl_tab, uint32_t world, uint32_t me, uint32_t do_wait,
                                                          unsigned long long timeout_ticks) {
    const uint32_t p = threadIdx.x;
    if (p >= world || p == me) return;
    PushCtrl* pc = reinterpret_cast<PushCtrl*>(ctrl_tab[p]);
    __hip_atomic_store(&pc->flag[me], PUSH_CLOSING, __ATOMIC_RELAXED, __HIP_MEMORY_SCOPE_SYSTEM);
    if (!do_wait) return;
    const unsigned long long t0 = wall_clock64();
    while (__hip_atomic_load(&mine->flag[p], __ATOMIC_RELAXED, __HIP_MEMORY_SCOPE_SYSTEM) < PUSH_CLOSING) {
        if (wall_clock64() - t0 > timeout_ticks) break;
        __builtin_amdgcn_s_sleep(32);
    }
}

struct ProbeGeo {
    uint64_t blk;
    uint32_t n_local, ld;
    uint32_t om_n;
    uint32_t world, me;
    uint32_t save_stride;
};
constexpr int PROBE_REGIONS = 5;
__device__ __forceinline__ void probe_region(const ProbeGeo& g, uint32_t b, int r, bool& in_om, uint64_t& off, uint32_t& len, uint32_t& save_off) {
    in_om = r >= 3;
    if (r == 0) { off = (uint64_t)b * g.blk; len = g.ld; save_off = 0; }
// ... 652 lines not shown
```

bipymc_amd/csrc/kernels_wide.h:

```cpp
#pragma once
#include "kernels.h"

namespace bpm {
inline namespace BPM_VARIANT_NS {

constexpr int WIDE_CP = 2;
constexpr int WIDE_CHUNK_PAIRS = WAVE * WIDE_CP;

template <int TARGET>
struct WideTarget {
    __device__ __forceinline__ void add(const double*, uint32_t, uint32_t, double, double) {}
    __device__ __forceinline__ double finish(const double*, uint32_t) { return 0.0; }
};
template <>
struct WideTarget<TARGET_GAUSS> {
    double s1 = 0.0, s2 = 0.0;
    __device__ __forceinline__ void add(const double* tp, uint32_t pi, uint32_t dim, double v0, double v1) {
        const uint32_t j0 = 2u * pi;
        if (j0 < dim) {
            const double2 is = *reinterpret_cast<const double2*>(tp + 4 + j0);
            const double z0 = v0 * is.x;
            s1 += z0; s2 += z0 * z0;
            if (j0 + 1u < dim) {
                const double z1 = v1 * is.y;
                s1 += z1; s2 += z1 * z1;
            }
        }
    }
    __device__ __forceinline__ double finish(const double* tp, uint32_t) {
        const double t1 = gsum<WAVE>(s1), t2 = gsum<WAVE>(s2);
        return tp[1] - 0.5 * (tp[2] * t2 - tp[3] * t1 * t1);
    }
};
template <>
struct WideTarget<TARGET_MIXTURE> {
    double q0 = 0.0, q1 = 0.0;
    __device__ __forceinline__ void add(const double* tp, uint32_t pi, uint32_t dim, double v0, double v1) {
        if (2u * pi + 1u < dim) {
#pragma unroll
            for (int c = 0; c < 2; ++c) {
                const double* p = tp + 2 + 7 * c;
                const double a = (v0 - p[0]) * p[2];
                const double b = (v1 - p[1]) * p[3];
                const double qq = (a * a - 2.0 * p[4] * a * b + b * b) * p[5];
                if (c == 0) q0 += qq; else q1 += qq;
            }
        }
    }
    __device__ __forceinline__ double finish(const double* tp, uint32_t dim) {
        const double t0 = gsum<WAVE>(q0), t1 = gsum<WAVE>(q1);
        const double npairs = (double)(dim / 2);
        const double c0 = tp[0] + npairs * tp[8] - 0.5 * t0;
        const double c1 = tp[1] + npairs * tp[15] - 0.5 * t1;
        const double m = fmax(c0, c1);
        return m + log(exp(c0 - m) + exp(c1 - m));
    }
};

__device__ __forceinline__ double2 wide_load2(const double* row, uint32_t pi, bool valid) {
    double2 t = make_double2(0.0, 0.0);
    if (valid) t = reinterpret_cast<const double2*>(row)[pi];
    return t;
}
__device__ __forceinline__ void wide_store2_stream(double* row, uint32_t pi, double v0, double v1) {
    bpm_d2v t = {v0, v1};
    __builtin_nontemporal_store(t, reinterpret_cast<bpm_d2v*>(row) + pi);
}
__device__ __forceinline__ void wide_store2_wt16(double* row, uint32_t pi, double v0, double v1) {
    bpm_d2v t = {v0, v1};
    bpm_d2v* p = reinterpret_cast<bpm_d2v*>(row) + pi;
    asm volatile("global_store_dwordx4 %0, %1, off sc1" ::"v"(p), "v"(t) : "memory");
}

struct WideUni {
    uint32_t dim, ld, P;
    uint32_t thr, forced;
    double gamma;
    double epsilon, u_epsilon;
    int snk;
    double gs;
};
template <int ALGO, int NP>
__device__ __forceinline__ void wide_pair_proposal(const PhaseArgs& a, const WideUni& U, uint32_t c, uint32_t pi, bool valid, double2 x, uint32_t mine,
                                                   double& p0, double& p1, uint32_t& mbits) {
    constexpr bool DREAM = ALGO == ALGO_DREAM;
    const uint32_t j0 = 2u * pi;
    const bool two = j0 + 1u < U.dim;
    const u32x4 wj = chain_block<true>(a.seed, c, a.t, SLOT_DIM0 + pi);
    double en0 = 0.0, en1 = 0.0, eu0 = 0.0, eu1 = 0.0;
    mbits = 0u;
    if (valid) {
        if (U.epsilon > 0.0) {
            double n0, n1;
            box_muller_pair_f32(wj.z, wj.w, n0, n1);
            en0 = U.epsilon * n0;
            if (two) en1 = U.epsilon * n1;
        }
        if (DREAM) {
            if (U.u_epsilon > 0.0) {
                eu0 = -U.u_epsilon + (2.0 * U.u_epsilon) * (((double)(wj.y >> 16) + 0.5) * 1.52587890625e-05);
                if (two) eu1 = -U.u_epsilon + (2.0 * U.u_epsilon) * (((double)(wj.y & 0xFFFFu) + 0.5) * 1.52587890625e-05);
            }
            if ((wj.x >> 16) <= U.thr || j0 == U.forced) mbits |= 1u;
            if (two && ((wj.x & 0xFFFFu) <= U.thr || j0 + 1u == U.forced)) mbits |= 2u;
        }
    }
    if (DREAM) {
        double s0 = 0.0, s1 = 0.0;
        if (NP > 0) {
            double2 ra[NP > 0 ? NP : 1], rb[NP > 0 ? NP : 1];
#pragma unroll
            for (int p = 0; p < NP; ++p) {
                ra[p] = wide_load2(row_ptr(a.L, (uint32_t)__builtin_amdgcn_readlane((int)mine, 2 * p)), pi, valid);
                rb[p] = wide_load2(row_ptr(a.L, (uint32_t)__builtin_amdgcn_readlane((int)mine, 2 * p + 1)), pi, valid);
            }
            s0 = ra[0].x - rb[0].x; s1 = ra[0].y - rb[0].y;
#pragma unroll
            for (int p = 1; p < NP; ++p) { s0 = s0 + (ra[p].x - rb[p].x); s1 = s1 + (ra[p].y - rb[p].y); }
        } else {
#pragma unroll 1
            for (uint32_t p = 0; p < U.P; ++p) {
                const double2 ra = wide_load2(row_ptr(a.L, (uint32_t)__shfl((int)mine, (int)(2u * p))), pi, valid);
                const double2 rb = wide_load2(row_ptr(a.L, (uint32_t)__shfl((int)mine, (int)(2u * p + 1u))), pi, valid);
                s0 = (p == 0) ? (ra.x - rb.x) : (s0 + (ra.x - rb.x));
                s1 = (p == 0) ? (ra.y - rb.y) : (s1 + (ra.y - rb.y));
            }
        }
        const double jump0 = (1.0 + eu0) * U.gamma * s0 + en0;
        const double jump1 = (1.0 + eu1) * U.gamma * s1 + en1;
        p0 = (mbits & 1u) ? (jump0 + x.x) : x.x;
        p1 = (mbits & 2u) ? (jump1 + x.y) : x.y;
    } else if (!U.snk) {
        const double2 ra = wide_load2(row_ptr(a.L, (uint32_t)__builtin_amdgcn_readlane((int)mine, 0)), pi, valid);
        const double2 rb = wide_load2(row_ptr(a.L, (uint32_t)__builtin_amdgcn_readlane((int)mine, 1)), pi, valid);
        double q0 = U.gamma * (ra.x - rb.x), q1 = U.gamma * (ra.y - rb.y);
        q0 = q0 + x.x; q1 = q1 + x.y;
        q0 = q0 + en0; q1 = q1 + en1;
        p0 = q0; p1 = q1;
    } else {
        const double2 rz = wide_load2(row_ptr(a.L, (uint32_t)__builtin_amdgcn_readlane((int)mine, 2)), pi, valid);
        double q0 = x.x + U.gs * (x.x - rz.x), q1 = x.y + U.gs * (x.y - rz.y);
        q0 = q0 + en0; q1 = q1 + en1;
        p0 = (j0 < U.dim) ? q0 : x.x;
        p1 = two ? q1 : x.y;
    }
}

template <int ALGO, int TARGET, int NP, int STAGE>
__global__ __launch_bounds__(BPM_BLOCK_WAVE) void phase_wide_kernel(
#ifdef BPM_PRELOAD
    const uint32_t* pl_plan, uint32_t pl_upd_off, uint32_t pl_n_items, uint32_t pl_mode,
#endif
    const PhaseArgs a) {
    constexpr bool DREAM = ALGO == ALGO_DREAM;
    constexpr bool FUSED = STAGE == STAGE_FUSED;
    const uint32_t lane = threadIdx.x & (WAVE - 1);
    const uint32_t w = (uint32_t)__builtin_amdgcn_readfirstlane((int)(blockIdx.x * (blockDim.x / WAVE) + (threadIdx.x / WAVE)));
    if (w >= a.n_items) return;
    uint32_t c;
    if (a.mode == 0) {
        c = own_pos_to_chain(a, a.upd_off + w);
    } else {
        c = a.lo + w;
        if (a.mode == 1) {
            const uint32_t pos = chain_to_pos(a, c);
            if ((pos - a.upd_off) >= a.n_upd) {
                if (!FUSED && lane == 0) a.ids_buf[w] = -1;
                return;
            }
        }
    }
    c = (uint32_t)__builtin_amdgcn_readfirstlane((int)c);
    if (!FUSED && lane == 0) a.ids_buf[w] = (int32_t)c;
    const uint32_t li = c - a.lo;
    WideUni U;
    U.dim = a.L.dim; U.ld = a.L.ld; U.P = NP > 0 ? (uint32_t)NP : a.P;
    U.thr = 65536u; U.forced = U.dim; U.epsilon = a.epsilon; U.u_epsilon = a.u_epsilon; U.snk = 0; U.gs = 0.0;
    const uint32_t npairs = (U.dim + 1u) >> 1;
    const uint32_t n_chunks = (npairs + WIDE_CHUNK_PAIRS - 1u) / WIDE_CHUNK_PAIRS;
    const double* xrow = row_ptr(a.L, c);
    const u32x4 h0 = chain_block(a.seed, c, a.t, SLOT_HDR0);
    const bool snk_possible = !DREAM && a.p_snooker > 0.0 && a.M >= 3;
    const uint32_t npart = 2u * U.P + (snk_possible ? 3u : 0u);
    uint32_t mine = 0;
    if (lane < npart) mine = pos_to_chain(a, a.pool_off + partner_pos(a, c, lane, 2u * U.P));
    double ll_cur = 0.0;
    uint32_t acc_prev = 0u;
    if (FUSED) { ll_cur = a.ll[li]; acc_prev = a.acc_count[li]; }
    const double u_sel = (double)(h0.x >> 16) * 1.52587890625e-05;
    const double u_gam = (double)(h0.x & 0xFFFFu) * 1.52587890625e-05;
    int cr_idx = -1, d_prime = (int)U.dim, jump = 0;
    if (DREAM) {
        double cum = 0.0;
        int idx = (int)a.n_cr - 1;
        bool found = false;
#pragma unroll
        for (int m = 0; m < MAX_CR; ++m) {
            if (m < (int)a.n_cr) {
                cum += a.cr_state[m];
                if (!found && u_sel < cum) { idx = m; found = true; }
            }
        }
        cr_idx = idx;
#pragma unroll
        for (int m = 0; m < MAX_CR; ++m) if (m == idx) U.thr = a.thr[m];
        int cnt = (int)U.dim;
        if (U.thr < 65536u) {
            cnt = 0;
#pragma unroll 1
            for (uint32_t k = 0; k < n_chunks; ++k) {
#pragma unroll
                for (int u = 0; u < WIDE_CP; ++u) {
                    const uint32_t pi = k * WIDE_CHUNK_PAIRS + (uint32_t)u * WAVE + lane;
                    const uint32_t j0 = 2u * pi;
                    bool b0 = false, b1 = false;
                    if (j0 < U.dim) {
                        const u32x4 wj = chain_block<true>(a.seed, c, a.t, SLOT_DIM0 + pi);
                        b0 = (wj.x >> 16) <= U.thr;
                        b1 = (j0 + 1u < U.dim) && (wj.x & 0xFFFFu) <= U.thr;
                    }
                    cnt += (int)__popcll(__ballot(b0)) + (int)__popcll(__ballot(b1));
                }
            }
        }
        if (cnt == 0) { U.forced = mulhi32(h0.y, U.dim); cnt = 1; }
        d_prime = cnt;
        double gamma = a.gamma_tab[cnt];
        if (a.k % 5 == 0 && !(u_gam < 0.2)) { gamma = 1.0; jump = 1; }
        U.gamma = gamma;
    } else {
        double gamma = a.gamma_demc;
        if (a.mode != 2 && a.k % 10 == 0 && !(u_gam < 0.1)) { gamma = 1.0; jump = 1; }
        U.gamma = gamma;
    }
    double sn_n2 = 0.0;
    if (snk_possible && u_sel < a.p_snooker) {
        const double* zrow = row_ptr(a.L, (uint32_t)__builtin_amdgcn_readlane((int)mine, 2));
        const double* r1row = row_ptr(a.L, (uint32_t)__builtin_amdgcn_readlane((int)mine, 3));
        const double* r2row = row_ptr(a.L, (uint32_t)__builtin_amdgcn_readlane((int)mine, 4));
        double n2 = 0.0, dot = 0.0;
#pragma unroll 1
        for (uint32_t k = 0; k < n_chunks; ++k) {
#pragma unroll
            for (int u = 0; u < WIDE_CP; ++u) {
                const uint32_t pi = k * WIDE_CHUNK_PAIRS + (uint32_t)u * WAVE + lane;
                const bool valid = 2u * pi < U.dim;
                const double2 x = wide_load2(xrow, pi, valid), z = wide_load2(zrow, pi, valid), r1 = wide_load2(r1row, pi, valid), r2 = wide_load2(r2row, pi, valid);
                const double d0 = x.x - z.x, d1 = x.y - z.y;
                n2 += d0 * d0; dot += (r1.x - r2.x) * d0;
                n2 += d1 * d1; dot += (r1.y - r2.y) * d1;
            }
        }
        n2 = gsum<WAVE>(n2);
        dot = gsum<WAVE>(dot);
        if (n2 > 0.0) { U.snk = 1; U.gs = (1.2 + u01_32(h0.y)) * (dot / n2); sn_n2 = n2; }
    }
    WideTarget<TARGET> T;
    double dl = 0.0, n2p = 0.0;
    const bool cr_stat = DREAM && a.adapt_on && a.cr_gate;
    const double* m2row = a.w_m2 + (uint32_t)(li * 2u * U.ld);
    double* hrow = (FUSED && a.hist_row) ? a.hist_row + (uint32_t)(li * U.ld) : nullptr;
    double* prow = FUSED ? nullptr : a.prop_buf + (uint64_t)w * U.ld;
    const double* zrow_b = U.snk ? row_ptr(a.L, (uint32_t)__builtin_amdgcn_readlane((int)mine, 2)) : xrow;
#pragma unroll 1
    for (uint32_t k = 0; k < n_chunks; ++k) {
#pragma unroll
        for (int u = 0; u < WIDE_CP; ++u) {
            const uint32_t pi = k * WIDE_CHUNK_PAIRS + (uint32_t)u * WAVE + lane;
            const bool valid = 2u * pi < U.dim;
            const double2 x = wide_load2(xrow, pi, valid);
            double2 m2 = make_double2(0.0, 0.0);
            if (cr_stat) m2 = wide_load2(m2row, pi, valid);
            double p0, p1;
            uint32_t mb;
            wide_pair_proposal<ALGO, NP>(a, U, c, pi, valid, x, mine, p0, p1, mb);
            if (FUSED) T.add(a.tparams, pi, U.dim, p0, p1);
            if (cr_stat && valid) {
                const double f0 = x.x - p0, f1 = x.y - p1;
                dl += m2.x > 0.0 ? (f0 * f0 * (double)a.hist_len) / m2.x : (f0 * f0) / 1e-24;
                if (2u * pi + 1u < U.dim) dl += m2.y > 0.0 ? (f1 * f1 * (double)a.hist_len) / m2.y : (f1 * f1) / 1e-24;
            }
            if (U.snk) {
                const double2 z = wide_load2(zrow_b, pi, valid);
                const double e0 = p0 - z.x, e1 = p1 - z.y;
                n2p += e0 * e0; n2p += e1 * e1;
            }
            if (valid) {
                if (hrow) wide_store2_stream(hrow, pi, x.x, x.y);
                if (prow) reinterpret_cast<double2*>(prow)[pi] = make_double2(p0, p1);
                if (trace_mask_of(a)) {
                    const uint32_t j0 = 2u * pi;
                    trace_mask_of(a)[(uint64_t)li * U.dim + j0] = (uint8_t)(mb & 1u);
                    if (j0 + 1u < U.dim) trace_mask_of(a)[(uint64_t)li * U.dim + j0 + 1u] = (uint8_t)((mb >> 1) & 1u);
                }
            }
        }
    }
    const double delta = cr_stat ? gsum<WAVE>(dl) : 0.0;
    double log_corr = 0.0;
    if (U.snk) {
        n2p = gsum<WAVE>(n2p);
        log_corr = 0.5 * (double)(U.dim - 1u) * (log(n2p) - log(sn_n2));
    }
    if (trace_i32_of(a)) {
        int32_t* tr = trace_i32_of(a) + (uint64_t)li * TRACE_I32;
        if (lane == 0) { tr[0] = cr_idx; tr[1] = d_prime; tr[2] = jump; tr[4] = U.snk; }
        if (lane < (uint32_t)MAX_PARTNERS) tr[5 + lane] = lane < npart ? (int32_t)mine : -1;
    }
    if (!FUSED) {
        if (lane == 0) {
            a.aux_buf[w] = log_corr;
            if (DREAM) {
                *delta_ptr(a.L, c) = cr_stat ? delta : 0.0;
                *cridx_ptr(a.L, c) = cr_stat ? (double)cr_idx : -1.0;
            }
        }
        return;
    }
    const double ll_prop = T.finish(a.tparams, U.dim);
    const double d_acc = (ll_prop + log_corr) - ll_cur;
    bool is_nan;
    const bool accepted = __builtin_amdgcn_readfirstlane(accept_test(d_acc, u01_53(h0.z, h0.w), &is_nan) ? 1 : 0) != 0;
    const double new_ll = accepted ? ll_prop : ll_cur;
    if (lane == 0) {
        if (accepted) {
            if (a.wt) __hip_atomic_store(&a.acc_count[li], acc_prev + 1u, __ATOMIC_RELAXED, __HIP_MEMORY_SCOPE_AGENT);
            else a.acc_count[li] = acc_prev + 1u;
            if (a.wt) __hip_atomic_store(&a.ll[li], new_ll, __ATOMIC_RELAXED, __HIP_MEMORY_SCOPE_AGENT);
            else a.ll[li] = new_ll;
        }
        if (is_nan) atomicAdd(&a.counters[2], 1ull);
        if (a.llhist_row) a.llhist_row[li] = new_ll;
        if (DREAM && a.adapt_on) {
            if (a.wt) {
                __hip_atomic_store(delta_ptr(a.L, c), cr_stat ? delta : 0.0, __ATOMIC_RELAXED, __HIP_MEMORY_SCOPE_AGENT);
                __hip_atomic_store(cridx_ptr(a.L, c), cr_stat ? (double)cr_idx : -1.0, __ATOMIC_RELAXED, __HIP_MEMORY_SCOPE_AGENT);
            } else {
                *delta_ptr(a.L, c) = cr_stat ? delta : 0.0;
                *cridx_ptr(a.L, c) = cr_stat ? (double)cr_idx : -1.0;
            }
            if (a.n_peers && a.adapt_on && a.cr_gate) {
                const uint32_t d_off = (uint32_t)(delta_ptr(a.L, c) - a.L.G), c_off = (uint32_t)(cridx_ptr(a.L, c) - a.L.G);
#pragma unroll 1
                for (uint32_t p = 0; p < a.n_peers; ++p) {
                    double* pg = reinterpret_cast<double*>(a.peer_tab[p]);
                    __hip_atomic_store(pg + d_off, delta, __ATOMIC_RELAXED, __HIP_MEMORY_SCOPE_SYSTEM);
                    __hip_atomic_store(pg + c_off, (double)cr_idx, __ATOMIC_RELAXED, __HIP_MEMORY_SCOPE_SYSTEM);
                }
            }
        }
        if (trace_i32_of(a)) {
            trace_i32_of(a)[(uint64_t)li * TRACE_I32 + 3] = accepted ? 1 : 0;
            double* tf = trace_f64_of(a) + (uint64_t)li * TRACE_F64;
            bool nan_alpha;
            tf[0] = accept_alpha(d_acc, &nan_alpha); tf[1] = ll_prop; tf[2] = delta; tf[3] = U.gamma;
        }
    }
    const bool welford = DREAM && a.adapt_on;
    if (accepted || welford || a.x_next) {
        double* srow = row_ptr(a.L, c);
        double* nrow = a.x_next ? a.x_next + (uint32_t)(li * U.ld) : nullptr;
        double* wm = a.w_mean + (uint32_t)(li * 2u * U.ld);
        double* w2 = a.w_m2 + (uint32_t)(li * 2u * U.ld);
        const uint32_t row_off = (uint32_t)(srow - a.L.G);
        const double cntp = (double)(a.hist_len + 1);
#pragma unroll 1
        for (uint32_t k = 0; k < n_chunks; ++k) {
#pragma unroll
            for (int u = 0; u < WIDE_CP; ++u) {
                const uint32_t pi = k * WIDE_CHUNK_PAIRS + (uint32_t)u * WAVE + lane;
                const bool valid = 2u * pi < U.dim;
                const double2 x = wide_load2(xrow, pi, valid);
                double n0 = x.x, n1 = x.y;
                if (accepted) {
                    uint32_t mb;
                    wide_pair_proposal<ALGO, NP>(a, U, c, pi, valid, x, mine, n0, n1, mb);
                }
                double2 mean = make_double2(0.0, 0.0), m2 = make_double2(0.0, 0.0);
                if (welford) { mean = wide_load2(wm, pi, valid); m2 = wide_load2(w2, pi, valid); }
                if (valid) {
                    if (nrow) {
                        reinterpret_cast<double2*>(nrow)[pi] = make_double2(n0, n1);
                    } else if (accepted) {
                        if (a.wt == 2u) wide_store2_wt16(srow, pi, n0, n1);
                        else if (a.wt) {
                            __hip_atomic_store(srow + 2u * pi, n0, __ATOMIC_RELAXED, __HIP_MEMORY_SCOPE_AGENT);
                            __hip_atomic_store(srow + 2u * pi + 1u, n1, __ATOMIC_RELAXED, __HIP_MEMORY_SCOPE_AGENT);
                        } else reinterpret_cast<double2*>(srow)[pi] = make_double2(n0, n1);
#pragma unroll 1
                        for (uint32_t p = 0; p < a.n_peers; ++p) {
                            double* pg = reinterpret_cast<double*>(a.peer_tab[p]) + row_off;
                            __hip_atomic_store(pg + 2u * pi, n0, __ATOMIC_RELAXED, __HIP_MEMORY_SCOPE_SYSTEM);
                            __hip_atomic_store(pg + 2u * pi + 1u, n1, __ATOMIC_RELAXED, __HIP_MEMORY_SCOPE_SYSTEM);
                        }
                    }
                    if (accepted && hrow) wide_store2_stream(hrow, pi, n0, n1);
                    if (welford) {
                        const double d0 = n0 - mean.x, d1 = n1 - mean.y;
                        mean.x = mean.x + d0 / cntp; mean.y = mean.y + d1 / cntp;
                        m2.x = m2.x + d0 * (n0 - mean.x); m2.y = m2.y + d1 * (n1 - mean.y);
                        if (a.wt) { wide_store2_wt16(wm, pi, mean.x, mean.y); wide_store2_wt16(w2, pi, m2.x, m2.y); }
                        else { wide_store2_stream(wm, pi, mean.x, mean.y); wide_store2_stream(w2, pi, m2.x, m2.y); }
                    }
                }
            }
        }
    }
    if (a.n_peers) asm volatile("s_waitcnt vmcnt(0)" ::: "memory");
}

template <int ALGO>
__global__ __launch_bounds__(BPM_BLOCK_WAVE) void phase_wide_commit_kernel(const PhaseArgs a) {
    constexpr bool DREAM = ALGO == ALGO_DREAM;
    const uint32_t lane = threadIdx.x & (WAVE - 1);
    const uint32_t w = (uint32_t)__builtin_amdgcn_readfirstlane((int)(blockIdx.x * (blockDim.x / WAVE) + (threadIdx.x / WAVE)));
    if (w >= a.n_items) return;
    const int32_t id = a.ids_buf[w];
    if (id < 0) return;
    const uint32_t c = (uint32_t)__builtin_amdgcn_readfirstlane(id), li = c - a.lo;
    const uint32_t dim = a.L.dim, ld = a.L.ld, npairs = (dim + 1u) >> 1;
    const uint32_t n_chunks = (npairs + WIDE_CHUNK_PAIRS - 1u) / WIDE_CHUNK_PAIRS;
    const double ll_cur = a.ll[li], ll_prop = a.aux_buf[a.L.n_local + w], log_corr = a.aux_buf[w];
    const uint32_t acc_prev = a.acc_count[li];
    const u32x4 h0 = chain_block(a.seed, c, a.t, SLOT_HDR0);
    const double d_acc = (ll_prop + log_corr) - ll_cur;
    bool is_nan;
    const bool accepted = __builtin_amdgcn_readfirstlane(accept_test(d_acc, u01_53(h0.z, h0.w), &is_nan) ? 1 : 0) != 0;
    const double new_ll = accepted ? ll_prop : ll_cur;
    if (lane == 0) {
        if (accepted) { a.acc_count[li] = acc_prev + 1u; a.ll[li] = new_ll; }
        if (is_nan) atomicAdd(&a.counters[2], 1ull);
        if (a.llhist_row) a.llhist_row[li] = new_ll;
        if (trace_i32_of(a)) {
            trace_i32_of(a)[(uint64_t)li * TRACE_I32 + 3] = accepted ? 1 : 0;
            double* tf = trace_f64_of(a) + (uint64_t)li * TRACE_F64;
            bool nan_alpha;
            tf[0] = accept_alpha(d_acc, &nan_alpha); tf[1] = ll_prop; tf[2] = DREAM ? *delta_ptr(a.L, c) : 0.0; tf[3] = 0.0;
        }
    }
    const bool welford = DREAM && a.adapt_on;
    double* srow = row_ptr(a.L, c);
    const double* prow = a.prop_buf + (uint64_t)w * ld;
    double* hrow = a.hist_row ? a.hist_row + (uint32_t)(li * ld) : nullptr;
    double* nrow = a.x_next ? a.x_next + (uint32_t)(li * ld) : nullptr;
    double* wm = a.w_mean + (uint32_t)(li * 2u * ld);
    double* w2 = a.w_m2 + (uint32_t)(li * 2u * ld);
    const double cntp = (double)(a.hist_len + 1);
#pragma unroll 1
    for (uint32_t k = 0; k < n_chunks; ++k) {
#pragma unroll
        for (int u = 0; u < WIDE_CP; ++u) {
            const uint32_t pi = k * WIDE_CHUNK_PAIRS + (uint32_t)u * WAVE + lane;
            const bool valid = 2u * pi < dim;
            const double2 nv = accepted ? wide_load2(prow, pi, valid) : wide_load2(srow, pi, valid);
            double2 mean = make_double2(0.0, 0.0), m2 = make_double2(0.0, 0.0);
            if (welford) { mean = wide_load2(wm, pi, valid); m2 = wide_load2(w2, pi, valid); }
            if (!valid) continue;
            if (nrow) reinterpret_cast<double2*>(nrow)[pi] = nv;
            else if (accepted) reinterpret_cast<double2*>(srow)[pi] = nv;
            if (hrow) wide_store2_stream(hrow, pi, nv.x, nv.y);
            if (welford) {
                const double d0 = nv.x - mean.x, d1 = nv.y - mean.y;
                mean.x = mean.x + d0 / cntp; mean.y = mean.y + d1 / cntp;
                m2.x = m2.x + d0 * (nv.x - mean.x); m2.y = m2.y + d1 * (nv.y - mean.y);
                wide_store2_stream(wm, pi, mean.x, mean.y);
                wide_store2_stream(w2, pi, m2.x, m2.y);
            }
        }
    }
}

template <int TARGET>
__global__ __launch_bounds__(BPM_BLOCK_WAVE) void eval_ll_wide_kernel(const double* X, uint32_t n, uint32_t ld, uint32_t dim, const double* tparams, double* out) {
    const uint32_t lane = threadIdx.x & (WAVE - 1);
    const uint32_t w = (uint32_t)__builtin_amdgcn_readfirstlane((int)(blockIdx.x * (blockDim.x / WAVE) + (threadIdx.x / WAVE)));
    if (w >= n) return;
    const double* row = X + (uint64_t)w * ld;
    const uint32_t npairs = (dim + 1u) >> 1, n_chunks = (npairs + WIDE_CHUNK_PAIRS - 1u) / WIDE_CHUNK_PAIRS;
    WideTarget<TARGET> T;
#pragma unroll 1
    for (uint32_t k = 0; k < n_chunks; ++k) {
#pragma unroll
        for (int u = 0; u < WIDE_CP; ++u) {
            const uint32_t pi = k * WIDE_CHUNK_PAIRS + (uint32_t)u * WAVE + lane;
            const double2 x = wide_load2(row, pi, 2u * pi < dim);
            T.add(tparams, pi, dim, x.x, x.y);
        }
    }
    const double ll = T.finish(tparams, dim);
    if (lane == 0) out[w] = ll;
}

}
}
```

bipymc_amd/csrc/sampler.hip:

```cpp
#include <dlfcn.h>
#include <sys/mman.h>
#include <unistd.h>
#include <hip/hip_runtime.h>
#include <hip/hip_ext.h>
#include <rccl/rccl.h>

#include <algorithm>
#include <cstddef>
#include <chrono>
#include <cmath>
#include <cstdio>
#include <cstdlib>
#include <cstring>
#include <string>
#include <atomic>
#include <map>
#include <mutex>
#include <thread>
#include <type_traits>
#include <vector>

#include "../../include/bipymc_hip.h"
#include "kernels.h"
#include "kernels_wide.h"
// ... 51 lines not shown

static int wait_stream(hipStream_t st, double spin_ms = 50.0) {
    const auto t0 = std::chrono::steady_clock::now();
    for (;;) {
        const hipError_t q = hipStreamQuery(st);
        if (q == hipSuccess) return 0;
        if (q != hipErrorNotReady) { (void)hipGetLastError(); break; }
        if (std::chrono::duration<double, std::milli>(std::chrono::steady_clock::now() - t0).count() > spin_ms) break;
    }
    HIPCK(hipStreamSynchronize(st));
    return 0;
}

struct Rccl {
    void* lib = nullptr;
    decltype(&ncclGetUniqueId) GetUniqueId = nullptr;
    decltype(&ncclCommInitRank) CommInitRank = nullptr;
    decltype(&ncclAllGather) AllGather = nullptr;
    decltype(&ncclAllReduce) AllReduce = nullptr;
    decltype(&ncclCommDestroy) CommDestroy = nullptr;
    decltype(&ncclGetErrorString) GetErrorString = nullptr;
};
static Rccl g_rccl;
static int load_rccl() {
    if (g_rccl.lib) return 0;
    const char* names[] = {"librccl.so.1", "librccl.so", "/opt/rocm/lib/librccl.so.1"};
    void* lib = nullptr;
    for (const char* n : names) {
        lib = dlopen(n, RTLD_NOW | RTLD_GLOBAL);
        if (lib) break;
    }
    if (!lib) return fail(std::string("cannot load RCCL: ") + dlerror());
#define SYM(f)                                                          \
    g_rccl.f = reinterpret_cast<decltype(g_rccl.f)>(dlsym(lib, "nccl" #f)); \
    if (!g_rccl.f) return fail("RCCL symbol nccl" #f " missing");
    SYM(GetUniqueId) SYM(CommInitRank) SYM(AllGather) SYM(AllReduce) SYM(CommDestroy) SYM(GetErrorString)
#undef SYM
    g_rccl.lib = lib;
    return 0;
}
#define NCCLCK(expr)                                                                              \
    do {                                                                                          \
        ncclResult_t _r = (expr);                                                                 \
        if (_r != ncclSuccess) return fail(std::string(#expr) + " failed: " + g_rccl.GetErrorString(_r)); \
    } while (0)

typedef void (*PhaseLaunch)(const PhaseArgs&, hipStream_t);
typedef void (*FusedLaunch)(const PhaseArgs&, int flavour, hipStream_t);
typedef void (*EvalLaunch)(const double*, uint32_t, uint32_t, uint32_t, const double*, double*, hipStream_t);

struct bpm_sampler;
struct Dispatch {
    bpm_sampler* user_cur = nullptr;
    bool user_launch_failed = false;

    bpm::DirectQueue* dq = nullptr;
    bool group_direct = false;
    bool dq_error = false;
    int update_fence = bpm::DirectQueue::FENCED;
    bool wt_stores = false;
    bool call_last_gen = false;
    bool dq_call_last_gen = false;

    hipEvent_t stop_event = nullptr;
    int sig = -1;
    bool release_this = false;
    bool need_acquire = false;

    int64_t n_direct = 0, n_stream = 0;
    int64_t timed_launches = 0;

    void mark_acquire(bool v) { need_acquire = v; }
    void idle() {
        user_cur = nullptr; user_launch_failed = false;
        dq = nullptr; group_direct = false; dq_error = false; update_fence = bpm::DirectQueue::FENCED;
        wt_stores = false; call_last_gen = false; dq_call_last_gen = false;
        stop_event = nullptr; sig = -1; release_this = false;
    }
};
static thread_local Dispatch g_disp;
struct DispatchScope {
    Dispatch& d;
    explicit DispatchScope(bpm_sampler* user_cur = nullptr) : d(g_disp) { d.user_cur = user_cur; }
    ~DispatchScope() { d.idle(); }
    DispatchScope(const DispatchScope&) = delete;
    DispatchScope& operator=(const DispatchScope&) = delete;
};
struct OnHipStream {
    Dispatch& d;
    bpm::DirectQueue* const dq;
    const bool group_direct;
    OnHipStream() : d(g_disp), dq(d.dq), group_direct(d.group_direct) { d.dq = nullptr; d.group_direct = false; }
    ~OnHipStream() { d.dq = dq; d.group_direct = group_direct; }
    OnHipStream(const OnHipStream&) = delete;
    OnHipStream& operator=(const OnHipStream&) = delete;
};
static inline hipEvent_t take_stop_event(Dispatch& d) {
    hipEvent_t e = d.stop_event;
    d.stop_event = nullptr;
    return e;
}
template <class... P>
struct KernargLayout {
    static constexpr size_t n = sizeof...(P);
    size_t off[n] = {}, size[n] = {sizeof(P)...}, bytes = 0;
    constexpr KernargLayout() {
        constexpr size_t al[n] = {alignof(P)...};
        size_t end = 0, al_max = 1;
        for (size_t i = 0; i < n; ++i) {
            off[i] = (end + al[i] - 1) / al[i] * al[i];
            end = off[i] + size[i];
            al_max = std::max(al_max, al[i]);
        }
        bytes = (end + al_max - 1) / al_max * al_max;
    }
};
enum class Then { KEEP, ACQUIRE, NO_ACQUIRE };
template <class... P>
static int launch_side(hipStream_t stream, void (*kernel)(P...), const char* name, dim3 grid, uint32_t block, int fence, Then then, std::common_type_t<P>... args) {
    Dispatch& d = g_disp;
    if (!d.dq) {
        hipLaunchKernelGGL(kernel, grid, dim3(block), 0, stream, args...);
        HIPCK(hipGetLastError());
        return 0;
    }
    constexpr KernargLayout<P...> lay;
    alignas(16) unsigned char ka[lay.bytes] = {};
    size_t i = 0;
    ((void)std::memcpy(ka + lay.off[i++], &args, sizeof(P)), ...);
    const bpm::DqKernel* k = d.dq->kernel(reinterpret_cast<const void*>(kernel));
    if (!k || d.dq->launch(*k, grid.x, grid.y, block, ka, lay.bytes, fence) != 0) return fail(std::string("direct AQL queue: ") + name + ": " + d.dq->why());
    if (then != Then::KEEP) d.mark_acquire(then == Then::ACQUIRE);
    return 0;
}
template <class K>
struct ModuleLaunch;
template <class... P>
struct ModuleLaunch<void(P...)> {
    static hipError_t on(hipStream_t stream, hipFunction_t fn, unsigned grid, unsigned block, unsigned lds_bytes, std::common_type_t<P>... args) {
        void* ptrs[] = {static_cast<void*>(&args)...};
        return hipModuleLaunchKernel(fn, grid, 1, 1, block, 1, 1, lds_bytes, stream, ptrs, nullptr);
    }
};
static inline uint32_t grid_for(uint32_t n_items, int lpc) {
    const uint32_t cpw = (uint32_t)(block_for(lpc) / lpc);
    return (n_items + cpw - 1) / cpw;
}
struct FusedKernarg {
    const uint32_t* pl_plan;
    uint32_t pl_upd_off, pl_n_items, pl_mode, _pad;
    PhaseArgs a;
};
static_assert(offsetof(FusedKernarg, a) == 24 && sizeof(FusedKernarg) == 24 + sizeof(PhaseArgs), "kernarg layout of phase_fused_kernel");
static inline void update_packet(Dispatch& d, const bpm::DqKernel* k, unsigned grid, unsigned block, const void* ka, size_t nbytes) {
    int fence = d.update_fence;
    const int sig = d.sig;
    d.sig = -1;
    if (d.need_acquire) { fence |= bpm::DirectQueue::ACQUIRE; d.need_acquire = false; }
    if (d.release_this) { fence |= bpm::DirectQueue::RELEASE; d.release_this = false; }
    if (!k || d.dq->launch(*k, grid, 1, block, ka, nbytes, fence, sig) != 0) d.dq_error = true;
    ++d.timed_launches; ++d.n_direct;
}
static inline void update_on_stream(Dispatch& d, hipFunction_t fn, unsigned grid, unsigned block, void* ka, size_t nbytes, hipStream_t s) {
    void* extra[] = {HIP_LAUNCH_PARAM_BUFFER_POINTER, ka, HIP_LAUNCH_PARAM_BUFFER_SIZE, &nbytes, HIP_LAUNCH_PARAM_END};
    (void)hipExtModuleLaunchKernel(fn, grid * block, 1, 1, block, 1, 1, 0, s, nullptr, extra, nullptr, take_stop_event(d), 0);
    ++d.timed_launches; ++d.n_stream;
}
template <class K>
static inline void launch_packed(K kernel, hipFunction_t& fn, const PhaseArgs& a, unsigned grid, unsigned block, hipStream_t s) {
    Dispatch& d = g_disp;
    FusedKernarg ka{a.rec_tab, a.rec_off, a.n_items, a.mode, 0u, a};
    if (d.dq) return update_packet(d, d.dq->kernel(reinterpret_cast<const void*>(kernel)), grid, block, &ka, sizeof(ka));
    if (!fn) { if (hipGetFuncBySymbol(&fn, reinterpret_cast<const void*>(kernel)) != hipSuccess) { (void)hipGetLastError(); fn = nullptr; } }
    if (fn) return update_on_stream(d, fn, grid, block, &ka, sizeof(ka), s);
    hipExtLaunchKernelGGL(kernel, dim3(grid), dim3(block), 0, s, nullptr, take_stop_event(d), 0, a.rec_tab, a.rec_off, a.n_items, a.mode, a);
    ++d.timed_launches; ++d.n_stream;
}
template <int ALGO, int T, int NP, int LPC, int DPL, int HOT>
static void launch_hot(const PhaseArgs& a, hipStream_t s) {
    static hipFunction_t fn = nullptr;
    constexpr unsigned blk = (unsigned)block_for_hot(LPC, HOT, DPL), cpw = blk / (unsigned)LPC;
    launch_packed(phase_fused_kernel<ALGO, T, LPC, DPL, NP, HOT>, fn, a, (a.n_items + cpw - 1u) / cpw, blk, s);
}
template <int ALGO, int T, int NP, int LPC, int DPL>
static void launch_fused(const PhaseArgs& a, int flavour, hipStream_t s) {
    constexpr bool CAN_PLAN = (LPC == WAVE && DPL == 2), DREAM_ = ALGO == ALGO_DREAM;
    switch (flavour) {
        case FLAVOUR_STEADY_PLAN: if constexpr (CAN_PLAN) return launch_hot<ALGO, T, NP, LPC, DPL, FLAVOUR_STEADY_PLAN>(a, s); break;
        case FLAVOUR_STEADY: return launch_hot<ALGO, T, NP, LPC, DPL, FLAVOUR_STEADY>(a, s);
        case FLAVOUR_ADAPT_PLAN: if constexpr (CAN_PLAN && DREAM_) return launch_hot<ALGO, T, NP, LPC, DPL, FLAVOUR_ADAPT_PLAN>(a, s); break;
        case FLAVOUR_ADAPT: if constexpr (DREAM_) return launch_hot<ALGO, T, NP, LPC, DPL, FLAVOUR_ADAPT>(a, s); break;
        case FLAVOUR_SHARD_PLAN: if constexpr (CAN_PLAN) return launch_hot<ALGO, T, NP, LPC, DPL, FLAVOUR_SHARD_PLAN>(a, s); break;
        default: break;
    }
    launch_hot<ALGO, T, NP, LPC, DPL, FLAVOUR_GENERAL>(a, s);
}
template <int ALGO, int LPC, int DPL>
static void launch_propose(const PhaseArgs& a, hipStream_t s) {
    constexpr int NPC = ALGO == ALGO_DREAM ? 3 : 1;
    if (a.mode != 2u && a.P == (uint32_t)NPC && !(ALGO != ALGO_DREAM && a.p_snooker > 0.0))
        hipLaunchKernelGGL((phase_propose_kernel<ALGO, LPC, DPL, NPC>), dim3(grid_for(a.n_items, LPC)), dim3(block_for(LPC)), 0, s, a);
    else
        hipLaunchKernelGGL((phase_propose_kernel<ALGO, LPC, DPL>), dim3(grid_for(a.n_items, LPC)), dim3(block_for(LPC)), 0, s, a);
}
template <int ALGO, int LPC, int DPL>
static void launch_commit(const PhaseArgs& a, hipStream_t s) {
    hipLaunchKernelGGL((phase_commit_kernel<ALGO, LPC, DPL>), dim3(grid_for(a.n_items, LPC)), dim3(block_for(LPC)), 0, s, a);
}
template <int T, int LPC, int DPL>
static void launch_eval(const double* X, uint32_t n, uint32_t ld, uint32_t dim, const double* tp, double* out,
                        hipStream_t s) {
    hipLaunchKernelGGL((eval_ll_kernel<T, LPC, DPL>), dim3(grid_for(n, LPC)), dim3(block_for(LPC)), 0, s, X, n, ld, dim, tp, out);
}

struct Shape {
    int lpc, dpl, idx;
};
static bool pick_shape(uint32_t ld, Shape& sh) {
    const uint32_t np = ld / 2;
    if (np <= 1) sh = {1, 2, 0};
    else if (np <= 4) sh = {4, 2, 1};
    else if (np <= 16) sh = {16, 2, 2};
    else if (np <= 64) sh = {64, 2, 3};
    else if (np <= 128) sh = {64, 4, 4};
    else if (np <= 256) sh = {64, 8, 5};
    else sh = {64, 0, 6};
    return true;
}
constexpr int SHAPE_WIDE = 6;
#define SHAPE_TABLE(FN, WIDE, ...)                                                               \
    {FN<__VA_ARGS__ 1, 2>, FN<__VA_ARGS__ 4, 2>, FN<__VA_ARGS__ 16, 2>, FN<__VA_ARGS__ 64, 2>, \
     FN<__VA_ARGS__ 64, 4>, FN<__VA_ARGS__ 64, 8>, WIDE}
#define COMMA ,
template <int ALGO, int T, int NP>
static void launch_wide(const PhaseArgs& a, int, hipStream_t s) {
    const unsigned grid = (unsigned)((a.n_items + (BPM_BLOCK_WAVE / WAVE) - 1) / (BPM_BLOCK_WAVE / WAVE));
    static hipFunction_t fn = nullptr;
    launch_packed(phase_wide_kernel<ALGO, T, NP, STAGE_FUSED>, fn, a, grid, (unsigned)BPM_BLOCK_WAVE, s);
}
template <int ALGO>
static void launch_wide_propose(const PhaseArgs& a, hipStream_t s) {
    const unsigned grid = (unsigned)((a.n_items + (BPM_BLOCK_WAVE / WAVE) - 1) / (BPM_BLOCK_WAVE / WAVE));
    hipLaunchKernelGGL((phase_wide_kernel<ALGO, TARGET_HOST, 0, STAGE_PROPOSE>), dim3(grid), dim3(BPM_BLOCK_WAVE), 0, s, a.rec_tab, a.rec_off, a.n_items, a.mode, a);
}
template <int ALGO>
static void launch_wide_commit(const PhaseArgs& a, hipStream_t s) {
    const unsigned grid = (unsigned)((a.n_items + (BPM_BLOCK_WAVE / WAVE) - 1) / (BPM_BLOCK_WAVE / WAVE));
    hipLaunchKernelGGL((phase_wide_commit_kernel<ALGO>), dim3(grid), dim3(BPM_BLOCK_WAVE), 0, s, a);
}
template <int T>
static void launch_eval_wide(const double* X, uint32_t n, uint32_t ld, uint32_t dim, const double* tp, double* out, hipStream_t s) {
    hipLaunchKernelGGL((eval_ll_wide_kernel<T>), dim3((n + (BPM_BLOCK_WAVE / WAVE) - 1) / (BPM_BLOCK_WAVE / WAVE)), dim3(BPM_BLOCK_WAVE), 0, s, X, n, ld, dim, tp, out);
}
static FusedLaunch g_fused_gauss[3][7] = {SHAPE_TABLE(launch_fused, launch_wide<ALGO_DEMC COMMA TARGET_GAUSS COMMA 1>, ALGO_DEMC COMMA TARGET_GAUSS COMMA 1 COMMA),
                                          SHAPE_TABLE(launch_fused, launch_wide<ALGO_DREAM COMMA TARGET_GAUSS COMMA 3>, ALGO_DREAM COMMA TARGET_GAUSS COMMA 3 COMMA),
                                          SHAPE_TABLE(launch_fused, launch_wide<ALGO_DREAM COMMA TARGET_GAUSS COMMA 0>, ALGO_DREAM COMMA TARGET_GAUSS COMMA 0 COMMA)};
static FusedLaunch g_fused_mixture[3][7] = {SHAPE_TABLE(launch_fused, launch_wide<ALGO_DEMC COMMA TARGET_MIXTURE COMMA 1>, ALGO_DEMC COMMA TARGET_MIXTURE COMMA 1 COMMA),
                                            SHAPE_TABLE(launch_fused, launch_wide<ALGO_DREAM COMMA TARGET_MIXTURE COMMA 3>, ALGO_DREAM COMMA TARGET_MIXTURE COMMA 3 COMMA),
                                            SHAPE_TABLE(launch_fused, launch_wide<ALGO_DREAM COMMA TARGET_MIXTURE COMMA 0>, ALGO_DREAM COMMA TARGET_MIXTURE COMMA 0 COMMA)};
static FusedLaunch g_fused_banana[3] = {launch_fused<ALGO_DEMC, TARGET_BANANA, 1, 1, 2>, launch_fused<ALGO_DREAM, TARGET_BANANA, 3, 1, 2>,
                                        launch_fused<ALGO_DREAM, TARGET_BANANA, 0, 1, 2>};
static PhaseLaunch g_propose[2][7] = {SHAPE_TABLE(launch_propose, launch_wide_propose<ALGO_DEMC>, ALGO_DEMC COMMA),
                                      SHAPE_TABLE(launch_propose, launch_wide_propose<ALGO_DREAM>, ALGO_DREAM COMMA)};
template <int ALGO, int NP, int LPC, int DPL>
static void launch_replay(const PhaseArgs& a, hipStream_t s) {
    hipLaunchKernelGGL((phase_replay_kernel<ALGO, LPC, DPL, NP>), dim3(grid_for(a.n_upd, LPC)), dim3(block_for(LPC)), 0, s, a);
}
template <int ALGO, int NP, int DPL>
static void launch_replay_sorted(const PhaseArgs& a, hipStream_t s) {
    uint32_t max_cnt = 0;
    for (uint32_t r = 0; r < a.n_seg; ++r)
        if (r != a.seg_me) max_cnt = std::max(max_cnt, a.seg_off[r + 1] - a.seg_off[r]);
    if (max_cnt == 0) return;
    hipLaunchKernelGGL((phase_replay_sorted_kernel<ALGO, DPL, NP>), dim3((max_cnt + REPLAY_WG / WAVE - 1) / (REPLAY_WG / WAVE), a.n_seg), dim3(REPLAY_WG),
                       0, s, a);
}
#define RS_ROW(A, P) {launch_replay_sorted<A, P, 2>, launch_replay_sorted<A, P, 4>, launch_replay_sorted<A, P, 8>}
static PhaseLaunch g_replay_sorted[3][3] = {RS_ROW(ALGO_DEMC, 1), RS_ROW(ALGO_DREAM, 3), RS_ROW(ALGO_DREAM, 0)};
static PhaseLaunch g_replay[3][7] = {SHAPE_TABLE(launch_replay, nullptr, ALGO_DEMC COMMA 1 COMMA), SHAPE_TABLE(launch_replay, nullptr, ALGO_DREAM COMMA 3 COMMA),
                                     SHAPE_TABLE(launch_replay, nullptr, ALGO_DREAM COMMA 0 COMMA)};
static PhaseLaunch g_commit[2][7] = {SHAPE_TABLE(launch_commit, launch_wide_commit<ALGO_DEMC>, ALGO_DEMC COMMA),
                                     SHAPE_TABLE(launch_commit, launch_wide_commit<ALGO_DREAM>, ALGO_DREAM COMMA)};
static EvalLaunch g_eval_gauss[7] = SHAPE_TABLE(launch_eval, launch_eval_wide<TARGET_GAUSS>, TARGET_GAUSS COMMA);
static EvalLaunch g_eval_mixture[7] = SHAPE_TABLE(launch_eval, launch_eval_wide<TARGET_MIXTURE>, TARGET_MIXTURE COMMA);

struct bpm_sampler;
struct HistorySnapshot {
    bool valid = false;
    uint64_t epoch = 0;
    int64_t tabs = 0, rows = 0;
    void take(const bpm_sampler* s);
    int check(const bpm_sampler* s, const char* who, const char* first_call) const;
};

#include "device_memory.h"

struct Module {
    hipModule_t mod = nullptr;
    Module() = default;
    Module(Module&& o) noexcept : mod(o.mod) { o.mod = nullptr; }
    Module& operator=(Module&& o) noexcept {
        if (this != &o) { unload(); mod = o.mod; o.mod = nullptr; }
        return *this;
    }
    ~Module() { unload(); }
    hipError_t load(const std::vector<char>& code) { unload(); return hipModuleLoadData(&mod, code.data()); }
// ... 989 lines not shown
    d.flip = 0.5; d.shuffle = 1; d._pad = 0; d.epsilon = -1.0; d.u_epsilon = -1.0; d.gamma = -1.0;
    if (o) d = *o;
    d.flip = std::min(1.0, std::max(0.0, d.flip));
    if (d.epsilon < 0.0) d.epsilon = (s->cfg.algo == BPM_ALGO_DREAM) ? 1e-12 : 1e-15;
    if (d.u_epsilon < 0.0) d.u_epsilon = 1e-2;
    if (!(d.gamma > 0.0)) d.gamma = 2.38 / std::sqrt(2.0 * (double)s->dim);
    s->opts = d;
    s->k_gen = 0;
    s->phase = 0;
    HIPCK(hipMemsetAsync(s->counters, 0, 4 * sizeof(unsigned long long), s->stream));
    HIPCK(hipMemsetAsync(s->acc_count, 0, ((size_t)s->n_local + ACC_SHARDS) * sizeof(uint32_t), s->stream));
    HIPCK(hipStreamSynchronize(s->stream));
    s->run_open = true;
    if (s->cfg.algo != BPM_ALGO_DEMC_SYNC) CK(ensure_perm_table(s, s->t_abs, 1));
    return 0;
}

static int allgather_state(bpm_sampler* s) {
    if (!s->comm) return 0;
    NCCLCK(g_rccl.AllGather(s->G + (uint64_t)s->rank * s->L.blk, s->G, (size_t)s->L.blk, ncclDouble, s->comm, s->stream));
    return 0;
}

static int build_window(bpm_sampler* s, int b, int64_t W, int shuffle) {
    bpm_sampler::TabBuf& B = s->tb[b];
    const int K = s->win_K;
    const int64_t t0 = W * K;
    hipStream_t bs = s->stream;
    PermKeys keys;
    for (int g = 0; g < K; ++g) keys.k[g] = make_perm_key(s->cfg.seed, (uint64_t)(t0 + g), s->N, shuffle != 0);
    for (int g = K; g < PERM_CHUNK; ++g) keys.k[g] = keys.k[0];
    const uint64_t n = (uint64_t)K * s->N;
    static const bool force_mode1 = test_path("mode1");
    uint32_t* const inv_out = (s->world > 1 || force_mode1) ? B.inv : nullptr;
    if (g_disp.dq && !B.sidx) {
        CK(launch_side(bs, perm_table_kernel, "perm_table_kernel", dim3((uint32_t)((n + 255) / 256)), 256, bpm::DirectQueue::FENCED, Then::KEEP, keys, K, s->N, B.perm, inv_out));
        if (B.plan) {
            const PlanParams pp{s->cfg.seed, (uint64_t)t0, (uint32_t)K, s->N, s->cfg.algo == BPM_ALGO_DREAM ? (uint32_t)s->cfg.del_pairs : 1u,
                                (s->cfg.algo == BPM_ALGO_DEMC && s->cfg.p_snooker > 0.0) ? 1u : 0u, 0u, 0u};
            CK(launch_side(bs, plan_kernel, "plan_kernel", dim3((uint32_t)((n + 255) / 256)), 256, bpm::DirectQueue::FENCED, Then::KEEP, pp, B.perm, B.plan, B.sidx));
        }
        B.W = W;
        B.shuffle = shuffle;
        g_disp.mark_acquire(true);
        return 0;
    }
    StreamSection sec(s);
    CK(sec.rc);
    hipLaunchKernelGGL(perm_table_kernel, dim3((unsigned)((n + 255) / 256)), dim3(256), 0, bs, keys, (uint32_t)K, s->N, B.perm, inv_out);
    HIPCK(hipGetLastError());
    if (B.plan) {
        const bool own_only = B.sidx != nullptr && s->push_enabled && s->push_connected;
        B.own_only = own_only;
        if (B.sidx) {
            if (own_only) {
                const uint32_t n_chunks = ((s->N + 1u) / 2u + SLOT_CHUNK - 1u) / SLOT_CHUNK;
                if (!B.chunk_count) CK(regrow(s, &B.chunk_count, (size_t)s->win_K * 2 * n_chunks, 0, false));
                HIPCK(hipMemsetAsync(B.plan_count, 0, (size_t)K * 2 * s->world * sizeof(uint32_t), bs));
                for (uint32_t assign = 0; assign < 2; ++assign)
                    hipLaunchKernelGGL(plan_slot_own_kernel, dim3(n_chunks, 2, (unsigned)K), dim3(SLOT_CHUNK), 0, bs, B.perm, s->N, s->lo, s->n_local, s->world,
                                       s->rank, n_chunks, B.chunk_count, B.sidx, B.plan_count, assign);
            } else {
                hipLaunchKernelGGL(plan_slot_kernel, dim3(2, (unsigned)K), dim3(PLAN_LOCAL_THREADS), 0, bs, B.perm, s->N, s->n_local, s->world,
                                   B.sidx, B.plan_count);
            }
            HIPCK(hipGetLastError());
            HIPCK(hipMemcpyAsync(B.count_h, B.plan_count, (size_t)K * 2 * s->world * sizeof(uint32_t), hipMemcpyDeviceToHost, bs));
        }
        PlanParams pp{s->cfg.seed, (uint64_t)t0, (uint32_t)K, s->N, s->cfg.algo == BPM_ALGO_DREAM ? (uint32_t)s->cfg.del_pairs : 1u,
                      (s->cfg.algo == BPM_ALGO_DEMC && s->cfg.p_snooker > 0.0) ? 1u : 0u, own_only ? s->lo : 0u, own_only ? s->n_local : 0u};
        hipLaunchKernelGGL(plan_kernel, dim3((unsigned)((n + 255) / 256)), dim3(256), 0, bs, pp, B.perm, B.plan, B.sidx);
        HIPCK(hipGetLastError());
    }
    HIPCK(hipEventRecord(B.built, bs));
    CK(sec.end());
    B.W = W;
    B.shuffle = shuffle;
    return 0;
}

static int ensure_perm_table(bpm_sampler* s, int64_t t, int64_t ) {
    const int shuffle = s->opts.shuffle != 0 ? 1 : 0;
    if (s->cur >= 0 && s->tab_shuffle == shuffle && t >= s->tab_t0 && t < s->tab_t0 + s->tab_K) return 0;
    const int K = s->win_K;
    const int64_t W = t / K;
    const int b = (int)(W & 1);
    bpm_sampler::TabBuf& B = s->tb[b];
    const bool want_own = B.sidx != nullptr && s->push_enabled && s->push_connected;
    if (B.W != W || B.shuffle != shuffle || (B.sidx && B.own_only && !want_own)) CK(build_window(s, b, W, shuffle));
    if (B.sidx) HIPCK(hipEventSynchronize(B.built));
    s->cur = b;
    s->perm_tab = B.perm; s->inv_tab = B.inv; s->plan_tab = B.plan; s->plan_count_h = B.count_h;
    s->tab_t0 = W * K;
    s->tab_K = K;
    s->tab_shuffle = shuffle;
    bpm_sampler::TabBuf& Bn = s->tb[b ^ 1];
    if (Bn.W != W + 1 || Bn.shuffle != shuffle || (Bn.sidx && Bn.own_only && !want_own)) CK(build_window(s, b ^ 1, W + 1, shuffle));
    return 0;
}

static int launch_cr_final(bpm_sampler* s, const double* src, uint32_t cnt) {
    const uint32_t n_cr = (uint32_t)s->cfg.n_cr;
    const int fence = s->dq_fence | bpm::DirectQueue::ACQUIRE;
    typedef void (*FinalK)(const double*, const double*, uint32_t, uint32_t, double*);
    const uint32_t rounds = (cnt + WAVE - 1) / WAVE;
    const FinalK kfn = rounds <= 1 ? cr_final_kernel<1> : (rounds <= 2 ? cr_final_kernel<2> : (rounds <= 4 ? cr_final_kernel<4> : cr_final_kernel<8>));
    return launch_side(s->stream, kfn, "cr_final_kernel", dim3(1), WAVE, fence, Then::NO_ACQUIRE, s->cr_state, src, cnt, n_cr, s->cr_state);
}
static int cr_flush_pending(bpm_sampler* s) {
    if (!s->cr_pending) return 0;
    s->cr_pending = false;
    return launch_cr_final(s, s->cr_pend_src, s->cr_pend_cnt);
}

static int prepare_generation(bpm_sampler* s, int64_t n_ahead) {
    const bool dream = s->cfg.algo == BPM_ALGO_DREAM;
    const uint64_t t = (uint64_t)s->t_abs;
    const bool sync = s->cfg.algo == BPM_ALGO_DEMC_SYNC;
    if (!sync) CK(ensure_perm_table(s, s->t_abs, n_ahead));
    const bool flip = flip_draw(s->cfg.seed, t, s->opts.flip);
    const PermKey pk = make_perm_key(s->cfg.seed, t, s->N, s->opts.shuffle != 0);
    const uint32_t n_first = (s->N + 1) / 2, n_second = s->N - n_first;
    uint32_t a_off = 0, a_n = n_first, b_off = n_first, b_n = n_second;
    if (flip) { std::swap(a_off, b_off); std::swap(a_n, b_n); }
    const bool adapt_on = dream && (s->cfg.burnin_gen > s->k_gen);
    s->gen_adapt_on = adapt_on;
    s->gen_cr_reduce = adapt_on && s->rows_logical > s->cfg.n_cr_gen;
    if (adapt_on && s->w_rows != s->rows_logical) {
        if (!history_resident(s))
            return fail("CR adaptation needs the chain history (keep_history=1) to rebuild its moments");
        const double m2_scale = s->hist_rows == s->rows_logical ? 1.0 : (double)s->rows_logical / (double)s->hist_rows;
        const uint64_t n_elem = (uint64_t)s->n_local * s->ld;
        StreamSection sec(s);
        CK(sec.rc);
        CK(normalize_history(s, 0, s->hist_rows));
        hipLaunchKernelGGL(welford_rebuild_kernel, dim3((unsigned)((n_elem + 255) / 256)), dim3(256), 0, s->stream,
                           s->hist, n_elem, n_elem, (uint32_t)s->hist_rows, s->ld, m2_scale, s->w_mean, s->w_m2);
        HIPCK(hipGetLastError());
        CK(sec.end());
        s->w_rows = s->rows_logical;
    }
    CK(ensure_gen_sums(s, s->rows_logical + 1));
    double* hist_row = nullptr;
    double* llhist_row = nullptr;
    if (generation_appends(s)) {
        CK(ensure_history(s, s->hist_rows + 1));
        hist_row = s->hist + (uint64_t)s->hist_rows * s->n_local * s->ld;
        llhist_row = s->llhist + (uint64_t)s->hist_rows * s->n_local;
        s->hist_tag[(size_t)s->hist_rows] = -1;
    }
    for (int ph = 0; ph < 2; ++ph) {
        PhaseArgs& a = s->cur_args[ph];
        std::memset(&a, 0, sizeof(a));
        a.L = s->L;
        a.ll = s->ll;
        a.hist_row = hist_row;
        a.llhist_row = llhist_row;
        a.w_mean = s->w_mean;
        a.w_m2 = s->w_m2;
        a.tparams = s->tparams;
        a.cr_state = s->cr_state;
        a.counters = s->counters;
        a.acc_count = s->acc_count;
        a.prop_buf = s->prop_buf;
        a.aux_buf = s->aux_buf;
        a.ids_buf = s->ids_buf;
        trace_set(a, s->trace_i32, s->trace_f64, s->trace_mask);
        a.pk = pk;
        a.perm_tab = s->perm_tab + (uint64_t)(s->t_abs - s->tab_t0) * s->N;
        a.inv_tab = s->inv_tab + (uint64_t)(s->t_abs - s->tab_t0) * s->N;
        a.plan = (s->plan_tab && !s->sorted_on) ? s->plan_tab + (uint64_t)(s->t_abs - s->tab_t0) * s->N * PLAN_WORDS : nullptr;
        a.rec_tab = a.plan;
        { static const bool no_tab = test_path("noperm");
          if (no_tab) { a.perm_tab = nullptr; a.inv_tab = nullptr; } }
        a.gamma_tab = s->gamma_tab;
        a.stamps = s->stamps;
        for (int m = 0; m < s->cfg.n_cr && m < MAX_CR; ++m)
            a.thr[m] = (uint32_t)std::floor(((double)(m + 1) / (double)s->cfg.n_cr) * 65536.0);
        a.seed = s->cfg.seed;
        a.t = t;
        a.k = (uint32_t)s->k_gen;
        a.N = s->N;
        a.lo = s->lo;
        a.upd_off = ph == 0 ? a_off : b_off;
        a.n_upd = ph == 0 ? a_n : b_n;
        a.pool_off = ph == 0 ? b_off : a_off;
        a.M = ph == 0 ? b_n : a_n;
        static const bool force_mode1 = test_path("mode1");
        const bool by_chain = s->world > 1 || force_mode1;
        a.mode = by_chain ? 1u : 0u;
        a.n_items = by_chain ? s->n_local : a.n_upd;
        a.rec_off = a.upd_off;
        if (s->sorted_on && s->plan_tab) {
            const uint32_t grp = a.upd_off == 0 ? 0u : 1u;
            const uint32_t* cnt = s->plan_count_h + ((uint64_t)(s->t_abs - s->tab_t0) * 2 + grp) * s->world;
            uint32_t acc = a.upd_off;
            for (uint32_t r = 0; r < s->world; ++r) { a.seg_off[r] = acc; acc += cnt[r]; }
            for (uint32_t r = s->world; r <= (uint32_t)MAX_SEG; ++r) a.seg_off[r] = acc;
            if (acc > a.upd_off + a.n_upd || cnt[s->rank] > a.n_upd)
                return fail("owner-sorted update records: the counts of generation " + std::to_string((long long)s->t_abs) + " exceed its half generation (window not built?)");
            a.n_seg = s->world; a.seg_me = s->rank; a.acc_by_item = 1u;
            a.rec_sorted = s->plan_tab + (uint64_t)(s->t_abs - s->tab_t0) * s->N * PLAN_WORDS;
            a.rec_tab = a.rec_sorted + (uint64_t)a.seg_off[s->rank] * PLAN_WORDS;
            a.rec_off = 0u;
            a.n_items = cnt[s->rank];
            a.mode = 0u;
        }
        const bool outlier_phase = dream && s->cfg.outlier_every > 0 && s->k_gen < s->cfg.burnin_gen;
        a.hist_by_pos = (s->hist_by_pos && (s->cfg.target_id != BPM_TARGET_HOST_CALLBACK || g_disp.user_cur == s) && hist_row != nullptr && !by_chain && !sync &&
                         s->trace_i32 == nullptr) ? (outlier_phase ? 2u : 1u) : 0u;
        { static const bool wt8 = test_path("wt8"); a.wt = g_disp.wt_stores ? (wt8 ? 1u : 2u) : 0u; }
        a.lean = s->lean ? 1u : 0u;
        a.algo = (uint32_t)s->cfg.algo;
        a.P = (uint32_t)s->cfg.del_pairs;
        a.n_cr = (uint32_t)s->cfg.n_cr;
        a.adapt_on = adapt_on ? 1u : 0u;
        a.cr_gate = (s->rows_logical > s->cfg.n_cr_gen) ? 1u : 0u;
        a.hist_len = (uint32_t)s->rows_logical;
        a.gamma_scale = s->cfg.gamma_scale;
        a.gamma_demc = s->opts.gamma;
        a.epsilon = s->opts.epsilon;
        a.u_epsilon = s->opts.u_epsilon;
        a.p_snooker = s->cfg.p_snooker;
        if (s->replay_active) a.accbits = s->accbits_all + (uint64_t)s->rank * s->n_local;
        if (s->push_active) { a.peer_tab = s->tab_peerG; a.n_peers = s->world - 1u; }
        if (s->sparse_active) {
            a.pack = s->PK + (uint64_t)s->rank * s->xnsub * s->xstride();
            a.pack_cap = s->xcap;
            a.pack_nsub = s->xnsub;
            a.pack_stride = s->xstride();
        }
        a.cr_part1 = nullptr; a.cr_chunk0 = 0u; a.cr_n1 = s->cr_n1;
        a.cr_fold_part = nullptr; a.cr_fold_tot = nullptr; a.cr_fold_out = nullptr; a.cr_fold_nb = 0u;
        if (sync) {
            a.algo = (uint32_t)BPM_ALGO_DEMC;
            a.mode = 2u;
            a.n_items = ph == 0 ? s->n_local : 0u;
            a.perm_tab = nullptr; a.inv_tab = nullptr; a.pk.on = 0u;
            a.upd_off = 0; a.n_upd = s->N; a.pool_off = 0; a.M = s->N - 1;
            a.x_next = s->x_next;
        }
    }
    static const bool no_hot = test_path("nohot"), cr_slots = test_path("crslots");
    const bool user_driven = g_disp.user_cur == s;
    const UserLikelihood::Fused& mod = s->like.fused;
    s->cur_launch = user_driven ? launch_user_fused : pick_fused(s);
    for (int ph = 0; ph < 2; ++ph) {
        const PhaseArgs& a = s->cur_args[ph];
        int f = (no_hot || sync || s->shape.idx == SHAPE_WIDE || !s->cur_launch) ? FLAVOUR_GENERAL : choose_flavour(a, dream, s->shape.lpc == WAVE && s->shape.dpl == 2);
        if (user_driven && !(((flavour_is_steady(f) && mod.hot != nullptr) || (hot_is_adapt(f) && mod.adapt != nullptr)) && (a.rec_tab != nullptr) == s->plan_on))
            f = FLAVOUR_GENERAL;
        s->cur_hot[ph] = f;
    }
    if (s->cr_p1) s->cr_p1_cur = s->cr_p1 + (size_t)(s->t_abs & 1) * 2 * MAX_CR * s->cr_n1;
    s->gen_cr_inkernel = s->gen_cr_reduce && !cr_slots && crp_shape(s->shape.lpc, s->shape.dpl);
    for (int ph = 0; ph < 2; ++ph)
        if (s->cur_args[ph].n_items > 0 && !hot_is_adapt(s->cur_hot[ph])) s->gen_cr_inkernel = false;
    if (s->gen_cr_inkernel) {
        const uint32_t n_first = (s->N + 1u) / 2u;
        for (int ph = 0; ph < 2; ++ph) {
            PhaseArgs& a = s->cur_args[ph];
            a.cr_part1 = s->cr_p1_cur;
            a.cr_chunk0 = a.upd_off == 0u ? 0u : cr_chunks_of(n_first, s->cr_g1);
        }
    }
    if (user_driven && !s->gen_cr_inkernel)
        for (int ph = 0; ph < 2; ++ph)
            if (hot_is_adapt(s->cur_hot[ph])) s->cur_hot[ph] = FLAVOUR_GENERAL;
    if (s->cr_pending) {
        PhaseArgs& a0 = s->cur_args[0];
        if (s->gen_cr_inkernel && a0.n_items > 0 && a0.cr_part1 != nullptr) {
            a0.cr_fold_part = s->cr_pend_src; a0.cr_fold_nb = s->cr_pend_cnt; a0.cr_fold_tot = s->cr_state; a0.cr_fold_out = s->cr_state_alt;
            std::swap(s->cr_state, s->cr_state_alt);
            s->cur_args[1].cr_state = s->cr_state;
            s->cr_pending = false;
        } else {
            CK(cr_flush_pending(s));
        }
    }
    return 0;
}

static int finish_generation(bpm_sampler* s) {
    if (s->lean) s->ll_stale = true;
    if (s->gen_adapt_on && !s->gen_cr_reduce) s->w_rows += 1;
    if (s->gen_cr_reduce) {
        const uint32_t n_cr = (uint32_t)s->cfg.n_cr;
        const int fence = s->dq_fence | bpm::DirectQueue::ACQUIRE;
        Dispatch& d = g_disp;
        if (d.dq) d.mark_acquire(false);
        const bool level1_from_slots = !s->gen_cr_inkernel;
        if (level1_from_slots) {
            const PhaseArgs& a0 = s->cur_args[0];
            typedef void (*L1K)(Layout, PermKey, const uint32_t*, uint32_t, uint32_t, uint32_t, double*);
            const L1K l1 = s->cr_g1 == 4u ? cr_level1_kernel<4> : (s->cr_g1 == 16u ? cr_level1_kernel<16> : cr_level1_kernel<64>);
            CK(launch_side(s->stream, l1, "cr_level1_kernel", dim3((uint32_t)(((uint64_t)s->cr_n1 * s->cr_g1 + CR_L1_THREADS - 1) / CR_L1_THREADS)), CR_L1_THREADS, fence, Then::KEEP,
                           s->L, a0.pk, a0.perm_tab, s->N, n_cr, s->cr_n1, s->cr_p1_cur));
        }
        const double* src = s->cr_p1_cur;
        uint32_t cnt = s->cr_n1;
        int flip = 0;
        while (cnt > CR_FINAL_MAX) {
            const uint32_t nn = (cnt + WAVE - 1) / WAVE;
            double* dst = s->cr_p2[flip];
            CK(launch_side(s->stream, cr_mid_kernel, "cr_mid_kernel", dim3(nn), WAVE, fence, Then::KEEP, src, cnt, n_cr, nn, dst));
            src = dst; cnt = nn; flip ^= 1;
        }
// ... 2553 lines not shown
```

Baseline: 845.0 million.

## Reorder PhaseArgs into a hot block loaded with wide scalar kernarg reads

Reorders the kernel argument struct so the fields the hot kernel front needs sit in a contiguous, cache-line-aligned block at the start. The Layout is flattened into separate fields so they can join that block. The fused kernel then reads the block with a few wide vector loads, gated on algorithm and adapt flavour, instead of many scattered scalar loads. The aim is to cut kernarg load latency at kernel start. In exchange it adds offset-dependent reinterpret code, static asserts and a wider register footprint.

```diff
diff --git a/bipymc_amd/csrc/kernels.h b/bipymc_amd/csrc/kernels.h
--- a/bipymc_amd/csrc/kernels.h
+++ b/bipymc_amd/csrc/kernels.h
@@ -93,33 +93,47 @@
     unsigned long long probe[MAX_SEG];
 };
 struct PhaseArgs {
-    Layout L;
+    double* L_G;
+    uint32_t L_ld, L_dim;
     double* ll;
+    uint32_t* acc_count;
+    const double* tparams;
+    unsigned long long* counters;
     double* hist_row;
     double* llhist_row;
+    uint64_t seed;
+    uint64_t t;
+    uint32_t k;
+    uint32_t upd_off;
+    double epsilon;
+    uint32_t wt;
+    uint32_t hist_by_pos;
+    const double* cr_state;
+    const double* gamma_tab;
+    double u_epsilon;
     double* w_mean;
     double* w_m2;
-    const double* tparams;
-    const double* cr_state;
-    unsigned long long* counters;
-    uint32_t* acc_count;
+    uint32_t cr_gate;
+    uint32_t hist_len;
+    uint32_t thr[MAX_CR];
+    uint64_t L_blk;
+    uint32_t L_n_local, L_world, L_magic;
+    uint32_t lo;
+    double gamma_demc, p_snooker;
+    uint32_t M, pool_off;
+    uint32_t cr_fold_nb;
+    uint32_t cr_chunk0, cr_n1;
+    uint32_t adapt_on;
+    uint32_t N, n_upd;
     double* prop_buf;
     double* aux_buf;
     int32_t* ids_buf;
-#ifdef BPM_TEST_HOOKS
-    int32_t* trace_i32;
-    double* trace_f64;
-    uint8_t* trace_mask;
-#endif
     PermKey pk;
     const uint32_t* perm_tab;
     const uint32_t* inv_tab;
-    const double* gamma_tab;
     const uint32_t* plan;
     const uint32_t* rec_tab;
     uint32_t rec_off;
-    uint32_t thr[MAX_CR];
-    unsigned long long* stamps;
     double* pack;
     uint32_t pack_cap, pack_nsub, pack_stride;
     double* x_next;
@@ -132,16 +146,7 @@
     uint32_t acc_by_item;
     const unsigned long long* peer_tab;
     uint32_t n_peers;
-    uint32_t hist_by_pos;
-#ifndef BPM_LEAN_LAST
     uint32_t lean;
-#endif
-    uint32_t wt;
-    uint64_t seed;
-    uint64_t t;
-    uint32_t k;
-    uint32_t N, lo;
-    uint32_t upd_off, n_upd, pool_off, M;
     uint32_t mode;
     uint32_t n_items;
     uint32_t algo;
@@ -150,15 +155,21 @@
     const double* cr_fold_part;
     const double* cr_fold_tot;
     double* cr_fold_out;
-    uint32_t cr_fold_nb;
-    uint32_t cr_chunk0, cr_n1;
-    uint32_t adapt_on;
-    uint32_t cr_gate;
-    uint32_t hist_len;
-    double gamma_scale, gamma_demc, epsilon, u_epsilon, p_snooker;
-#ifdef BPM_LEAN_LAST
-    uint32_t lean, pad_lean;
-#endif
+    double gamma_scale;
+    unsigned long long* stamps;
+#ifdef BPM_TEST_HOOKS
+    int32_t* trace_i32;
+    double* trace_f64;
+    uint8_t* trace_mask;
+#endif
+    __host__ __device__ __forceinline__ Layout L() const {
+        Layout l;
+        l.G = L_G; l.blk = L_blk; l.n_local = L_n_local; l.ld = L_ld; l.dim = L_dim; l.world = L_world; l.magic = L_magic;
+        return l;
+    }
+    __host__ __device__ __forceinline__ void set_L(const Layout& l) {
+        L_G = l.G; L_blk = l.blk; L_n_local = l.n_local; L_ld = l.ld; L_dim = l.dim; L_world = l.world; L_magic = l.magic;
+    }
 };
 
 #ifdef BPM_TEST_HOOKS
@@ -631,14 +642,14 @@
     constexpr bool DREAM = ALGO == ALGO_DREAM;
     constexpr bool FAST = (NP > 0) && (LPC == 1);
     constexpr bool SNK_DIRECT = (LPC == 1);
-    const uint32_t dim = a.L.dim, ld = a.L.ld;
+    const uint32_t dim = a.L().dim, ld = a.L().ld;
     const uint32_t P = NP > 0 ? (uint32_t)NP : a.P;
     if constexpr (FRONT) {
         const bool in_row = 2u * (uint32_t)q < ld;
 #pragma unroll
         for (int s = 0; s < DPL; ++s) wk.x[s] = in_row ? fr->x[s] : 0.0;
     } else
-    load_row<LPC, DPL>(row_ptr(a.L, c), q, ld, wk.x);
+    load_row<LPC, DPL>(row_ptr(a.L(), c), q, ld, wk.x);
     wk.ll_cur = 0.0;
     wk.acc_prev = 0u;
     if (!a.replay) {
@@ -794,11 +805,11 @@
 #pragma unroll
         for (int p = 0; p < NP; ++p) {
             if (LPC == WAVE) {
-                load_row_all<LPC, DPL>(row_ptr(a.L, part.get(2 * p)), q, ld, ra[p]);
-                load_row_all<LPC, DPL>(row_ptr(a.L, part.get(2 * p + 1)), q, ld, rb[p]);
+                load_row_all<LPC, DPL>(row_ptr(a.L(), part.get(2 * p)), q, ld, ra[p]);
+                load_row_all<LPC, DPL>(row_ptr(a.L(), part.get(2 * p + 1)), q, ld, rb[p]);
             } else {
-                load_row<LPC, DPL>(row_ptr(a.L, part.get(2 * p)), q, ld, ra[p]);
-                load_row<LPC, DPL>(row_ptr(a.L, part.get(2 * p + 1)), q, ld, rb[p]);
+                load_row<LPC, DPL>(row_ptr(a.L(), part.get(2 * p)), q, ld, ra[p]);
+                load_row<LPC, DPL>(row_ptr(a.L(), part.get(2 * p + 1)), q, ld, rb[p]);
             }
         }
     }
@@ -909,8 +920,8 @@
 #pragma unroll 1
             for (uint32_t p = 0; p < P; ++p) {
                 double ra[DPL], rb[DPL];
-                load_row<LPC, DPL>(row_ptr(a.L, part.lds[2 * p]), q, ld, ra);
-                load_row<LPC, DPL>(row_ptr(a.L, part.lds[2 * p + 1]), q, ld, rb);
+                load_row<LPC, DPL>(row_ptr(a.L(), part.lds[2 * p]), q, ld, ra);
+                load_row<LPC, DPL>(row_ptr(a.L(), part.lds[2 * p + 1]), q, ld, rb);
 #pragma unroll
                 for (int s = 0; s < DPL; ++s) sum[s] = (p == 0) ? (ra[s] - rb[s]) : (sum[s] + (ra[s] - rb[s]));
             }
@@ -949,16 +960,16 @@
 #pragma unroll
             for (int s = 0; s < DPL; ++s) { ra[s] = in_row ? fr->ra[0][s] : 0.0; rb[s] = in_row ? fr->rb[0][s] : 0.0; }
         } else {
-        load_row<LPC, DPL>(row_ptr(a.L, ca), q, ld, ra);
-        load_row<LPC, DPL>(row_ptr(a.L, cb), q, ld, rb);
+        load_row<LPC, DPL>(row_ptr(a.L(), ca), q, ld, ra);
+        load_row<LPC, DPL>(row_ptr(a.L(), cb), q, ld, rb);
         }
         double rz[DPL], r1[DPL], r2[DPL];
 #pragma unroll
         for (int s = 0; s < DPL; ++s) { rz[s] = 0.0; r1[s] = 0.0; r2[s] = 0.0; }
         if (do_snk) {
-            load_row<LPC, DPL>(row_ptr(a.L, SNK_DIRECT ? snk_id[0] : part.lds[2]), q, ld, rz);
-            load_row<LPC, DPL>(row_ptr(a.L, SNK_DIRECT ? snk_id[1] : part.lds[3]), q, ld, r1);
-            load_row<LPC, DPL>(row_ptr(a.L, SNK_DIRECT ? snk_id[2] : part.lds[4]), q, ld, r2);
+            load_row<LPC, DPL>(row_ptr(a.L(), SNK_DIRECT ? snk_id[0] : part.lds[2]), q, ld, rz);
+            load_row<LPC, DPL>(row_ptr(a.L(), SNK_DIRECT ? snk_id[1] : part.lds[3]), q, ld, r1);
+            load_row<LPC, DPL>(row_ptr(a.L(), SNK_DIRECT ? snk_id[2] : part.lds[4]), q, ld, r2);
         }
         early(wk);
 #pragma unroll
@@ -1028,7 +1039,7 @@
 template <int ALGO, int LPC, int DPL, int LEAN = 0 , bool CRP_W = false>
 __device__ __forceinline__ void finish_update(const PhaseArgs& a, uint32_t c, bool active, int q,
                                               const Work<DPL>& wk, double ll_prop) {
-    const uint32_t ld = a.L.ld;
+    const uint32_t ld = a.L().ld;
     const uint32_t li = c - a.lo;
     const double ll_cur = wk.ll_cur;
     const double d_acc = (ll_prop + wk.log_corr) - ll_cur;
@@ -1039,7 +1050,7 @@
     if (lean) {
         const unsigned long long m = __ballot(active && accepted && q == 0);
         if ((threadIdx.x & (WAVE - 1)) == 0 && m != 0ull)
-            __hip_atomic_fetch_add(&a.acc_count[a.L.n_local + ((blockIdx.x * (blockDim.x / WAVE) + (threadIdx.x / WAVE)) & (ACC_SHARDS - 1))],
+            __hip_atomic_fetch_add(&a.acc_count[a.L().n_local + ((blockIdx.x * (blockDim.x / WAVE) + (threadIdx.x / WAVE)) & (ACC_SHARDS - 1))],
                                    (uint32_t)__popcll(m), __ATOMIC_RELAXED, __HIP_MEMORY_SCOPE_AGENT);
     }
     if (!active) return;
@@ -1066,16 +1077,16 @@
         if (accepted && q == 0 && !lean) a.ll[li] = new_ll;
     } else if (accepted) {
         if (a.wt == 2u) {
-            store_row_wt16<LPC, DPL>(row_ptr(a.L, c), q, ld, nv);
+            store_row_wt16<LPC, DPL>(row_ptr(a.L(), c), q, ld, nv);
 #if defined(BPM_TEST_HOOKS) && defined(BPM_FAKE_NO_LL)
             if (LPC < WAVE) {} else
 #endif
             if (q == 0 && !lean) __hip_atomic_store(&a.ll[li], new_ll, __ATOMIC_RELAXED, __HIP_MEMORY_SCOPE_AGENT);
         } else if (a.wt) {
-            store_row_wt<LPC, DPL>(row_ptr(a.L, c), q, ld, nv);
+            store_row_wt<LPC, DPL>(row_ptr(a.L(), c), q, ld, nv);
             if (q == 0 && !lean) __hip_atomic_store(&a.ll[li], new_ll, __ATOMIC_RELAXED, __HIP_MEMORY_SCOPE_AGENT);
         } else {
-            store_row<LPC, DPL>(row_ptr(a.L, c), q, ld, nv);
+            store_row<LPC, DPL>(row_ptr(a.L(), c), q, ld, nv);
             if (q == 0 && !lean) a.ll[li] = new_ll;
         }
     }
@@ -1090,9 +1101,9 @@
         }
     }
     if (a.n_peers) {
-        const uint32_t row_off = (uint32_t)(row_ptr(a.L, c) - a.L.G);
+        const uint32_t row_off = (uint32_t)(row_ptr(a.L(), c) - a.L().G);
         const bool slots = ALGO == ALGO_DREAM && a.adapt_on && a.cr_gate && q == 0;
-        const uint32_t d_off = (uint32_t)(delta_ptr(a.L, c) - a.L.G), c_off = (uint32_t)(cridx_ptr(a.L, c) - a.L.G);
+        const uint32_t d_off = (uint32_t)(delta_ptr(a.L(), c) - a.L().G), c_off = (uint32_t)(cridx_ptr(a.L(), c) - a.L().G);
         const bool gated = a.adapt_on && a.cr_gate;
 #pragma unroll 1
         for (uint32_t p = 0; p < a.n_peers; ++p) {
@@ -1132,11 +1143,11 @@
         if (q == 0 && a.adapt_on && !(CRP_W && a.cr_part1 != nullptr)) {
             const bool gated = a.adapt_on && a.cr_gate;
             if (a.wt) {
-                __hip_atomic_store(delta_ptr(a.L, c), gated ? wk.delta : 0.0, __ATOMIC_RELAXED, __HIP_MEMORY_SCOPE_AGENT);
-                __hip_atomic_store(cridx_ptr(a.L, c), gated ? (double)wk.cr_idx : -1.0, __ATOMIC_RELAXED, __HIP_MEMORY_SCOPE_AGENT);
+                __hip_atomic_store(delta_ptr(a.L(), c), gated ? wk.delta : 0.0, __ATOMIC_RELAXED, __HIP_MEMORY_SCOPE_AGENT);
+                __hip_atomic_store(cridx_ptr(a.L(), c), gated ? (double)wk.cr_idx : -1.0, __ATOMIC_RELAXED, __HIP_MEMORY_SCOPE_AGENT);
             } else {
-                *delta_ptr(a.L, c) = gated ? wk.delta : 0.0;
-                *cridx_ptr(a.L, c) = gated ? (double)wk.cr_idx : -1.0;
+                *delta_ptr(a.L(), c) = gated ? wk.delta : 0.0;
+                *cridx_ptr(a.L(), c) = gated ? (double)wk.cr_idx : -1.0;
             }
         }
     }
@@ -1152,12 +1163,12 @@
 template <int LPC>
 __device__ __forceinline__ void pin_args(const PhaseArgs& a) {
     if (LPC != WAVE) {
-        asm volatile("" ::"s"(a.L.G), "s"(a.L.ld), "s"(a.L.dim), "s"(a.ll), "s"(a.hist_row), "s"(a.llhist_row), "s"(a.tparams),
+        asm volatile("" ::"s"(a.L().G), "s"(a.L().ld), "s"(a.L().dim), "s"(a.ll), "s"(a.hist_row), "s"(a.llhist_row), "s"(a.tparams),
                      "s"(a.cr_state), "s"(a.acc_count), "s"(a.perm_tab), "s"(a.inv_tab), "s"(a.gamma_tab), "s"(a.plan), "s"(a.pack),
                      "s"(a.thr[0]), "s"(a.thr[1]), "s"(a.thr[2]), "s"(a.seed), "s"(a.t), "s"(a.k), "s"(a.N),
                      "s"(a.lo), "s"(a.upd_off), "s"(a.n_upd), "s"(a.pool_off), "s"(a.M), "s"(a.mode), "s"(a.n_items), "s"(a.n_cr));
-        asm volatile("" ::"s"(a.adapt_on), "s"(a.cr_gate), "s"(a.hist_len), "s"(a.epsilon), "s"(a.u_epsilon), "s"(a.L.n_local),
-                     "s"(a.L.world), "s"(a.L.magic), "s"(a.counters), "s"(a.pack_cap), "s"(a.pack_nsub), "s"(a.pack_stride));
+        asm volatile("" ::"s"(a.adapt_on), "s"(a.cr_gate), "s"(a.hist_len), "s"(a.epsilon), "s"(a.u_epsilon), "s"(a.L().n_local),
+                     "s"(a.L().world), "s"(a.L().magic), "s"(a.counters), "s"(a.pack_cap), "s"(a.pack_nsub), "s"(a.pack_stride));
     }
 }
 
@@ -1194,12 +1205,56 @@
     if (!(a.mode == 0 && (a.rec_tab != nullptr) == plan && trace_i32_of(a) == nullptr && a.pack == nullptr && a.x_next == nullptr && a.epsilon > 0.0 &&
           a.perm_tab != nullptr && a.inv_tab != nullptr && a.replay == 0 && (!dream || (a.u_epsilon > 0.0 && a.n_cr == 3))))
         return FLAVOUR_GENERAL;
-    const bool single = a.n_peers == 0 && a.L.world == 1 && a.lo == 0 && stamps_allow_hot(a) && a.accbits == nullptr;
+    const bool single = a.n_peers == 0 && a.L().world == 1 && a.lo == 0 && stamps_allow_hot(a) && a.accbits == nullptr;
     if (single && a.adapt_on == 0) return plan ? FLAVOUR_STEADY_PLAN : FLAVOUR_STEADY;
-    if (plan && a.adapt_on == 0 && a.L.world > 1 && a.stamps == nullptr && (a.accbits != nullptr || a.n_peers > 0)) return FLAVOUR_SHARD_PLAN;
+    if (plan && a.adapt_on == 0 && a.L().world > 1 && a.stamps == nullptr && (a.accbits != nullptr || a.n_peers > 0)) return FLAVOUR_SHARD_PLAN;
     if (single && a.adapt_on != 0 && dream) return plan ? FLAVOUR_ADAPT_PLAN : FLAVOUR_ADAPT;
     return FLAVOUR_GENERAL;
 }
+typedef uint32_t bpm_hot16 __attribute__((ext_vector_type(16), aligned(8)));
+typedef uint32_t bpm_hot8 __attribute__((ext_vector_type(8), aligned(8)));
+typedef uint32_t bpm_hot4 __attribute__((ext_vector_type(4), aligned(8)));
+typedef uint32_t bpm_hot2 __attribute__((ext_vector_type(2), aligned(8)));
+constexpr int HOT_BLOCK_BYTES = 248;
+template <class V, int OFF>
+__device__ __forceinline__ V hot_read(const PhaseArgs& a) {
+    static_assert(OFF % 8 == 0 && OFF + (int)sizeof(V) <= HOT_BLOCK_BYTES, "a run of the hot block");
+    return *reinterpret_cast<const V*>(reinterpret_cast<const char*>(&a) + OFF);
+}
+struct HotWords {
+    uint32_t w[HOT_BLOCK_BYTES / 4];
+#define BPM_HOT_SET(V, N) template <int OFF> __device__ __forceinline__ void set(V v) { _Pragma("unroll") for (int i = 0; i < N; ++i) w[OFF / 4 + i] = v[i]; }
+    BPM_HOT_SET(bpm_hot16, 16) BPM_HOT_SET(bpm_hot8, 8) BPM_HOT_SET(bpm_hot4, 4) BPM_HOT_SET(bpm_hot2, 2)
+#undef BPM_HOT_SET
+    template <class T>
+    __device__ __forceinline__ T* ptr(int off) const {
+        typedef __attribute__((address_space(1))) T GT;
+        return (T*)(GT*)(((unsigned long long)w[off / 4 + 1] << 32) | w[off / 4]);
+    }
+    __device__ __forceinline__ uint64_t u64(int off) const { return ((uint64_t)w[off / 4 + 1] << 32) | w[off / 4]; }
+    __device__ __forceinline__ double f64(int off) const { return __hiloint2double((int)w[off / 4 + 1], (int)w[off / 4]); }
+    __device__ __forceinline__ uint32_t u32(int off) const { return w[off / 4]; }
+#define BPM_HOT_OFF(f) ((int)__builtin_offsetof(PhaseArgs, f))
+    template <bool DREAM, bool ADAPT, bool SHARD>
+    __device__ __forceinline__ void put(PhaseArgs& a) const {
+        a.L_G = ptr<double>(BPM_HOT_OFF(L_G)); a.L_ld = u32(BPM_HOT_OFF(L_ld)); a.L_dim = u32(BPM_HOT_OFF(L_dim));
+        a.ll = ptr<double>(BPM_HOT_OFF(ll)); a.acc_count = ptr<uint32_t>(BPM_HOT_OFF(acc_count)); a.tparams = ptr<const double>(BPM_HOT_OFF(tparams));
+        a.counters = ptr<unsigned long long>(BPM_HOT_OFF(counters)); a.hist_row = ptr<double>(BPM_HOT_OFF(hist_row)); a.llhist_row = ptr<double>(BPM_HOT_OFF(llhist_row));
+        a.seed = u64(BPM_HOT_OFF(seed)); a.t = u64(BPM_HOT_OFF(t)); a.k = u32(BPM_HOT_OFF(k)); a.upd_off = u32(BPM_HOT_OFF(upd_off));
+        a.epsilon = f64(BPM_HOT_OFF(epsilon)); a.wt = u32(BPM_HOT_OFF(wt)); a.hist_by_pos = u32(BPM_HOT_OFF(hist_by_pos));
+        if (DREAM) {
+            a.cr_state = ptr<const double>(BPM_HOT_OFF(cr_state)); a.gamma_tab = ptr<const double>(BPM_HOT_OFF(gamma_tab)); a.u_epsilon = f64(BPM_HOT_OFF(u_epsilon));
+#pragma unroll
+            for (int m = 0; m < 4; ++m) a.thr[m] = w[BPM_HOT_OFF(thr) / 4 + m];
+        } else {
+            a.gamma_demc = f64(BPM_HOT_OFF(gamma_demc)); a.p_snooker = f64(BPM_HOT_OFF(p_snooker)); a.M = u32(BPM_HOT_OFF(M)); a.pool_off = u32(BPM_HOT_OFF(pool_off));
+        }
+        if (ADAPT) {
+            a.w_mean = ptr<double>(BPM_HOT_OFF(w_mean)); a.w_m2 = ptr<double>(BPM_HOT_OFF(w_m2)); a.cr_gate = u32(BPM_HOT_OFF(cr_gate)); a.hist_len = u32(BPM_HOT_OFF(hist_len));
+        }
+        if (SHARD) { a.L_n_local = u32(BPM_HOT_OFF(L_n_local)); a.L_world = u32(BPM_HOT_OFF(L_world)); a.L_magic = u32(BPM_HOT_OFF(L_magic)); a.lo = u32(BPM_HOT_OFF(lo)); }
+    }
+};
 constexpr bool flavour_is_steady(int f) { return f == FLAVOUR_STEADY_PLAN || f == FLAVOUR_STEADY; }
 template <int ALGO, int TARGET, int LPC, int DPL, int NP, int HOT = 0>
 __global__ __launch_bounds__(block_for_hot(LPC, HOT, DPL)) void phase_fused_kernel(
@@ -1231,44 +1286,51 @@
     PlanFront<DPL, (NP > 0 ? NP : 1)> fr;
     uint32_t f_c = 0u;
     const uint32_t* f_rec = nullptr;
+    HotWords hw = {};
+    bpm_hot4 v_cg = {};
     Layout f_L = {};
-    double *f_ll = nullptr, *f_wm = nullptr, *f_w2 = nullptr;
+    double* f_ll = nullptr;
     const double *f_crs = nullptr, *f_tp = nullptr, *f_gt = nullptr;
     uint32_t* f_acc = nullptr;
-    unsigned long long* f_cnt = nullptr;
     uint32_t f_lo = 0u;
     typename Target<TARGET, LPC, DPL>::Consts tc_front;
     if constexpr (FRONT_CT) {
-        if (w < pl_n_items) {
-            f_L = a_in.L;
+        const bpm_hot16 v0 = hot_read<bpm_hot16, 0>(a_in);
+        bpm_hot16 v1 = {}, vds = {};
+        bpm_hot8 vc1 = {}, vad = {}, vde = {};
+        bpm_hot4 vth = {}, vsh = {};
+        bpm_hot2 vc2 = {}, vt2 = {};
+        hw.set<0>(v0);
+        if (ALGO == ALGO_DREAM) {
+            v1 = hot_read<bpm_hot16, 64>(a_in); hw.set<64>(v1);
+            if (ADAPT) {
+                vad = hot_read<bpm_hot8, 128>(a_in); vt2 = hot_read<bpm_hot2, 160>(a_in); v_cg = hot_read<bpm_hot4, BPM_HOT_OFF(cr_fold_nb)>(a_in);
+                hw.set<128>(vad); hw.set<160>(vt2);
+            }
+            else { vth = hot_read<bpm_hot4, 152>(a_in); hw.set<152>(vth); }
+            if (SHARD) { vsh = hot_read<bpm_hot4, 192>(a_in); hw.set<192>(vsh); }
+        } else {
+            vc1 = hot_read<bpm_hot8, 64>(a_in); vc2 = hot_read<bpm_hot2, 96>(a_in); hw.set<64>(vc1); hw.set<96>(vc2);
+            if (SHARD) { vds = hot_read<bpm_hot16, 168>(a_in); hw.set<168>(vds); }
+            else { vde = hot_read<bpm_hot8, 200>(a_in); hw.set<200>(vde); }
+        }
+        const uint32_t w_u = (uint32_t)__builtin_amdgcn_readfirstlane((int)w);
+        if (w_u < pl_n_items) {
+            PhaseArgs fa = {};
+            hw.template put<ALGO == ALGO_DREAM, ADAPT, SHARD>(fa);
+            f_L = fa.L();
             if (SHARD) __builtin_assume(f_L.world > 1u); else f_L.world = 1;
-            typedef uint32_t u32x4_a4 __attribute__((ext_vector_type(4), aligned(4)));
-            typedef uint32_t u32x2_a4 __attribute__((ext_vector_type(2), aligned(4)));
-            u32x4_a4 lw4 = {0u, 0u, 0u, 0u};
-            u32x2_a4 lw2 = {0u, 0u};
-            if (SHARD) {
-                lw4 = *reinterpret_cast<const u32x4_a4*>(&a_in.L.n_local);
-                lw2 = *reinterpret_cast<const u32x2_a4*>(&a_in.L.magic);
-                f_L.n_local = lw4.x; f_L.ld = lw4.y; f_L.dim = lw4.z; f_L.world = lw4.w; f_L.magic = lw2.x;
-                __builtin_assume(f_L.world > 1u);
-            }
-            f_ll = a_in.ll; f_acc = a_in.acc_count; f_crs = a_in.cr_state; f_tp = a_in.tparams; f_gt = a_in.gamma_tab; f_cnt = a_in.counters;
-            if (ADAPT) { f_wm = a_in.w_mean; f_w2 = a_in.w_m2; }
-            if (SHARD) f_lo = a_in.lo;
-            const uint32_t pos = (uint32_t)__builtin_amdgcn_readfirstlane((int)(pl_upd_off + w));
+            f_lo = fa.lo;
+            f_ll = fa.ll; f_acc = fa.acc_count; f_crs = fa.cr_state; f_tp = fa.tparams; f_gt = fa.gamma_tab;
+            const uint32_t pos = pl_upd_off + w_u;
             f_rec = pl_plan + (uint32_t)(pos * PLAN_WORDS);
             bpm_u32x16 rv = plan_record(f_rec);
 #ifndef BPM_STAMPS
-#define BPM_FRONT_ALL "s"(f_L.G), "s"(f_L.ld), "s"(f_L.dim), "s"(f_ll), "s"(f_acc), "s"(f_tp), "s"(f_cnt), "s"(a_in.seed), "s"(a_in.t), "s"(a_in.k), "s"(a_in.upd_off), \
-                      "s"(a_in.epsilon), "s"(a_in.wt), "s"(a_in.hist_by_pos), "s"(a_in.hist_row), "s"(a_in.llhist_row)
-#define BPM_FRONT_DREAM "s"(f_crs), "s"(f_gt), "s"(a_in.u_epsilon), "s"(a_in.thr[0]), "s"(a_in.thr[1]), "s"(a_in.thr[2]), "s"(a_in.thr[3])
-            if (ALGO == ALGO_DREAM && ADAPT) asm("" : "+s"(rv) : BPM_FRONT_ALL, BPM_FRONT_DREAM, "s"(f_wm), "s"(f_w2), "s"(a_in.cr_gate), "s"(a_in.hist_len));
-            else if (ALGO == ALGO_DREAM && SHARD) asm("" : "+s"(rv) : BPM_FRONT_ALL, BPM_FRONT_DREAM, "s"(f_lo), "s"(lw4), "s"(lw2));
-            else if (ALGO == ALGO_DREAM) asm("" : "+s"(rv) : BPM_FRONT_ALL, BPM_FRONT_DREAM);
-            else if (SHARD) asm("" : "+s"(rv) : BPM_FRONT_ALL, "s"(a_in.gamma_demc), "s"(a_in.p_snooker), "s"(a_in.M), "s"(a_in.pool_off), "s"(f_lo), "s"(lw4), "s"(lw2));
-            else asm("" : "+s"(rv) : BPM_FRONT_ALL, "s"(a_in.gamma_demc), "s"(a_in.p_snooker), "s"(a_in.M), "s"(a_in.pool_off));
-#undef BPM_FRONT_ALL
-#undef BPM_FRONT_DREAM
+            if (ALGO == ALGO_DREAM && ADAPT) asm("" : "+s"(rv) : "s"(v0), "s"(v1), "s"(vad), "s"(vt2), "s"(v_cg));
+            else if (ALGO == ALGO_DREAM && SHARD) asm("" : "+s"(rv) : "s"(v0), "s"(v1), "s"(vth), "s"(vsh));
+            else if (ALGO == ALGO_DREAM) asm("" : "+s"(rv) : "s"(v0), "s"(v1), "s"(vth));
+            else if (SHARD) asm("" : "+s"(rv) : "s"(v0), "s"(vc1), "s"(vc2), "s"(vds));
+            else asm("" : "+s"(rv) : "s"(v0), "s"(vc1), "s"(vc2), "s"(vde));
 #endif
             __builtin_amdgcn_sched_barrier(0);
             f_c = rv[0];
@@ -1303,9 +1365,10 @@
     if (COPY) {
         if constexpr (FRONT_CT) {
             a_hot = a_in;
-            a_hot.L = f_L; a_hot.ll = f_ll; a_hot.acc_count = f_acc; a_hot.cr_state = f_crs; a_hot.tparams = f_tp; a_hot.gamma_tab = f_gt; a_hot.counters = f_cnt;
-            if (ADAPT) { a_hot.w_mean = f_wm; a_hot.w_m2 = f_w2; }
-            if (SHARD) a_hot.lo = f_lo;
+            hw.template put<ALGO == ALGO_DREAM, ADAPT, SHARD>(a_hot);
+            if (ADAPT) { a_hot.cr_fold_nb = v_cg.x; a_hot.cr_chunk0 = v_cg.y; a_hot.cr_n1 = v_cg.z; }
+            __builtin_assume(a_hot.epsilon > 0.0);
+            if (ALGO == ALGO_DREAM) __builtin_assume(a_hot.u_epsilon > 0.0);
         } else
         a_hot = a_in;
         a_hot.mode = 0u; trace_set(a_hot, nullptr, nullptr, nullptr); a_hot.pack = nullptr;
@@ -1316,7 +1379,7 @@
         if (SHARD) a_hot.stamps = nullptr;
 #endif
         if (!ADAPT) a_hot.cr_fold_part = nullptr;
-        if (!SHARD) { a_hot.accbits = nullptr; a_hot.lo = 0; a_hot.L.world = 1; a_hot.acc_by_item = 0u; a_hot.n_peers = 0u; a_hot.peer_tab = nullptr; }
+        if (!SHARD) { a_hot.accbits = nullptr; a_hot.lo = 0; a_hot.L_world = 1; a_hot.acc_by_item = 0u; a_hot.n_peers = 0u; a_hot.peer_tab = nullptr; }
         if (ALGO == ALGO_DREAM) a_hot.n_cr = 3;
         if (NOPLAN) { a_hot.plan = nullptr; a_hot.rec_tab = nullptr; }
     }
@@ -1331,7 +1394,7 @@
 #ifndef BPM_STAMPS
         __builtin_assume(a_in.stamps == nullptr);
 #endif
-        if (!SHARD) { __builtin_assume(a_in.lo == 0); __builtin_assume(a_in.L.world == 1); }
+        if (!SHARD) { __builtin_assume(a_in.lo == 0); __builtin_assume(a_in.L_world == 1); }
         __builtin_assume(a_in.epsilon > 0.0);
         __builtin_assume(a_in.perm_tab != nullptr); __builtin_assume(a_in.inv_tab != nullptr);
         if (ALGO == ALGO_DREAM) { __builtin_assume(a_in.u_epsilon > 0.0); __builtin_assume(a_in.n_cr == 3); }
@@ -1399,13 +1462,13 @@
     }
   if (run) {
     if (LPC == WAVE) c = __builtin_amdgcn_readfirstlane(c);
-    const typename Target<TARGET, LPC, DPL>::Consts tc = FRONT_CT ? tc_front : Target<TARGET, LPC, DPL>::load(q, a.L.dim, a.tparams);
+    const typename Target<TARGET, LPC, DPL>::Consts tc = FRONT_CT ? tc_front : Target<TARGET, LPC, DPL>::load(q, a.L().dim, a.tparams);
     Work<DPL> wk;
     wk.item = w;
     wk.pos_own = a.upd_off + (active ? w : 0u);
     if (LPC == WAVE) wk.pos_own = (uint32_t)__builtin_amdgcn_readfirstlane((int)wk.pos_own);
     constexpr bool LEAN = lean_scalars<TARGET, LPC>();
-    const uint32_t dim_early = a.L.dim;
+    const uint32_t dim_early = a.L().dim;
     constexpr bool LEAN_CT = LEAN && lean_always<TARGET>();
 #ifdef BPM_STAMPS
     bpm_stamp[1] = 0; BPM_STAMP(1);
@@ -1423,8 +1486,8 @@
         make_proposal<ALGO, LPC, DPL, NP, 1, NoEarly, FRONT_CT>(a, c, active, q, cw, s_part, wk, rec, stamp_arg, NoEarly(), PcrGiven(), &fr);
     }
     double ll_prop;
-    if constexpr (FRONT_CT && TARGET == TARGET_GAUSS && ALGO == ALGO_DREAM) ll_prop = Target<TARGET_GAUSS, LPC, DPL>::template eval<true>(wk.p, q, a.L.dim, tc);
-    else ll_prop = Target<TARGET, LPC, DPL>::eval(wk.p, q, a.L.dim, tc);
+    if constexpr (FRONT_CT && TARGET == TARGET_GAUSS && ALGO == ALGO_DREAM) ll_prop = Target<TARGET_GAUSS, LPC, DPL>::template eval<true>(wk.p, q, a.L().dim, tc);
+    else ll_prop = Target<TARGET, LPC, DPL>::eval(wk.p, q, a.L().dim, tc);
     BPM_STAMP(5);
     finish_update<ALGO, LPC, DPL, (LEAN_CT ? 2 : (LEAN ? 1 : 0)), CRP>(a, c, active, q, wk, ll_prop);
     if (CRP && active && a.adapt_on && a.cr_gate) { cr_d = wk.delta; cr_i = wk.cr_idx; }
@@ -1497,12 +1560,12 @@
     } else {
         c = pos_to_chain(a, pos);
     }
-    active = active && (c - a.lo) >= a.L.n_local && a.accbits_all[c] != 0;
+    active = active && (c - a.lo) >= a.L().n_local && a.accbits_all[c] != 0;
     if (LPC == WAVE && !active) return;
     if (LPC == WAVE) c = __builtin_amdgcn_readfirstlane(c);
     Work<DPL> wk;
     make_proposal<ALGO, LPC, DPL, NP>(a, c, active, q, cw, s_part, wk, rec);
-    if (active) store_row<LPC, DPL>(row_ptr(a.L, c), q, a.L.ld, wk.p);
+    if (active) store_row<LPC, DPL>(row_ptr(a.L(), c), q, a.L().ld, wk.p);
 }
 
 #ifndef BPM_REPLAY_WG
@@ -1523,13 +1586,13 @@
     if (r == a_in.seg_me || k >= hi - lo) return;
     const uint32_t e = lo + k;
     const uint32_t* rec = a.rec_sorted + (uint32_t)(e * PLAN_WORDS);
-    const uint32_t acc = a.accbits_all[(uint64_t)r * a.L.n_local + k];
+    const uint32_t acc = a.accbits_all[(uint64_t)r * a.L().n_local + k];
     uint32_t c = rec[0];
     if (acc == 0u) return;
     c = (uint32_t)__builtin_amdgcn_readfirstlane((int)c);
     Work<DPL> wk;
     make_proposal<ALGO, LPC, DPL, NP>(a, c, true, lane, wv, s_part, wk, rec);
-    store_row<LPC, DPL>(row_ptr(a.L, c), lane, a.L.ld, wk.p);
+    store_row<LPC, DPL>(row_ptr(a.L(), c), lane, a.L().ld, wk.p);
 }
 
 template <int ALGO, int LPC, int DPL, int NP = 0>
@@ -1546,13 +1609,13 @@
     Work<DPL> wk;
     make_proposal<ALGO, LPC, DPL, NP>(a, c, active, q, cw, s_part, wk);
     if (!active) return;
-    store_row<LPC, DPL>(a.prop_buf + (uint64_t)w * a.L.ld, q, a.L.ld, wk.p);
+    store_row<LPC, DPL>(a.prop_buf + (uint64_t)w * a.L().ld, q, a.L().ld, wk.p);
     if (q == 0) {
         a.aux_buf[w] = wk.log_corr;
         if (ALGO == ALGO_DREAM) {
             const bool gated = a.adapt_on && a.cr_gate;
-            *delta_ptr(a.L, c) = gated ? wk.delta : 0.0;
-            *cridx_ptr(a.L, c) = gated ? (double)wk.cr_idx : -1.0;
+            *delta_ptr(a.L(), c) = gated ? wk.delta : 0.0;
+            *cridx_ptr(a.L(), c) = gated ? (double)wk.cr_idx : -1.0;
         }
     }
 }
@@ -1568,22 +1631,22 @@
     if (LPC == WAVE && !active) return;
     const uint32_t c = active ? (uint32_t)id : a.lo;
     Work<DPL> wk;
-    load_row<LPC, DPL>(row_ptr(a.L, c), q, a.L.ld, wk.x);
-    load_row<LPC, DPL>(a.prop_buf + (uint64_t)(active ? w : 0u) * a.L.ld, q, a.L.ld, wk.p);
+    load_row<LPC, DPL>(row_ptr(a.L(), c), q, a.L().ld, wk.x);
+    load_row<LPC, DPL>(a.prop_buf + (uint64_t)(active ? w : 0u) * a.L().ld, q, a.L().ld, wk.p);
     wk.log_corr = active ? a.aux_buf[w] : 0.0;
     wk.ll_cur = a.ll[c - a.lo];
     wk.acc_prev = a.acc_count[c - a.lo];
     if (ALGO == ALGO_DREAM && a.adapt_on) {
-        load_row<LPC, DPL>(a.w_mean + (uint32_t)((c - a.lo) * 2u * a.L.ld), q, a.L.ld, wk.w_mean);
-        load_row<LPC, DPL>(a.w_m2 + (uint32_t)((c - a.lo) * 2u * a.L.ld), q, a.L.ld, wk.w_m2);
-    }
-    const double ll_prop = active ? a.aux_buf[a.L.n_local + w] : 0.0;
+        load_row<LPC, DPL>(a.w_mean + (uint32_t)((c - a.lo) * 2u * a.L().ld), q, a.L().ld, wk.w_mean);
+        load_row<LPC, DPL>(a.w_m2 + (uint32_t)((c - a.lo) * 2u * a.L().ld), q, a.L().ld, wk.w_m2);
+    }
+    const double ll_prop = active ? a.aux_buf[a.L().n_local + w] : 0.0;
     const u32x4 h0 = chain_block(a.seed, c, a.t, SLOT_HDR0);
     wk.u_acc = u01_53(h0.z, h0.w);
     wk.delta = 0.0; wk.gamma = 0.0; wk.cr_idx = -1; wk.d_prime = 0; wk.jump = 0; wk.snk = 0; wk.maskbits = 0; wk.item = w; wk.pos_own = 0u;
     if (ALGO == ALGO_DREAM && active) {
-        wk.delta = *delta_ptr(a.L, c);
-        wk.cr_idx = (int)*cridx_ptr(a.L, c);
+        wk.delta = *delta_ptr(a.L(), c);
+        wk.cr_idx = (int)*cridx_ptr(a.L(), c);
     }
     PhaseArgs b = a;
     if (ALGO == ALGO_DREAM) b.cr_gate = (wk.cr_idx >= 0) ? 1u : 0u;
diff --git a/bipymc_amd/csrc/kernels_wide.h b/bipymc_amd/csrc/kernels_wide.h
--- a/bipymc_amd/csrc/kernels_wide.h
+++ b/bipymc_amd/csrc/kernels_wide.h
@@ -111,8 +111,8 @@
             double2 ra[NP > 0 ? NP : 1], rb[NP > 0 ? NP : 1];
 #pragma unroll
             for (int p = 0; p < NP; ++p) {
-                ra[p] = wide_load2(row_ptr(a.L, (uint32_t)__builtin_amdgcn_readlane((int)mine, 2 * p)), pi, valid);
-                rb[p] = wide_load2(row_ptr(a.L, (uint32_t)__builtin_amdgcn_readlane((int)mine, 2 * p + 1)), pi, valid);
+                ra[p] = wide_load2(row_ptr(a.L(), (uint32_t)__builtin_amdgcn_readlane((int)mine, 2 * p)), pi, valid);
+                rb[p] = wide_load2(row_ptr(a.L(), (uint32_t)__builtin_amdgcn_readlane((int)mine, 2 * p + 1)), pi, valid);
             }
             s0 = ra[0].x - rb[0].x; s1 = ra[0].y - rb[0].y;
 #pragma unroll
@@ -120,8 +120,8 @@
         } else {
 #pragma unroll 1
             for (uint32_t p = 0; p < U.P; ++p) {
-                const double2 ra = wide_load2(row_ptr(a.L, (uint32_t)__shfl((int)mine, (int)(2u * p))), pi, valid);
-                const double2 rb = wide_load2(row_ptr(a.L, (uint32_t)__shfl((int)mine, (int)(2u * p + 1u))), pi, valid);
+                const double2 ra = wide_load2(row_ptr(a.L(), (uint32_t)__shfl((int)mine, (int)(2u * p))), pi, valid);
+                const double2 rb = wide_load2(row_ptr(a.L(), (uint32_t)__shfl((int)mine, (int)(2u * p + 1u))), pi, valid);
                 s0 = (p == 0) ? (ra.x - rb.x) : (s0 + (ra.x - rb.x));
                 s1 = (p == 0) ? (ra.y - rb.y) : (s1 + (ra.y - rb.y));
             }
@@ -131,14 +131,14 @@
         p0 = (mbits & 1u) ? (jump0 + x.x) : x.x;
         p1 = (mbits & 2u) ? (jump1 + x.y) : x.y;
     } else if (!U.snk) {
-        const double2 ra = wide_load2(row_ptr(a.L, (uint32_t)__builtin_amdgcn_readlane((int)mine, 0)), pi, valid);
-        const double2 rb = wide_load2(row_ptr(a.L, (uint32_t)__builtin_amdgcn_readlane((int)mine, 1)), pi, valid);
+        const double2 ra = wide_load2(row_ptr(a.L(), (uint32_t)__builtin_amdgcn_readlane((int)mine, 0)), pi, valid);
+        const double2 rb = wide_load2(row_ptr(a.L(), (uint32_t)__builtin_amdgcn_readlane((int)mine, 1)), pi, valid);
         double q0 = U.gamma * (ra.x - rb.x), q1 = U.gamma * (ra.y - rb.y);
         q0 = q0 + x.x; q1 = q1 + x.y;
         q0 = q0 + en0; q1 = q1 + en1;
         p0 = q0; p1 = q1;
     } else {
-        const double2 rz = wide_load2(row_ptr(a.L, (uint32_t)__builtin_amdgcn_readlane((int)mine, 2)), pi, valid);
+        const double2 rz = wide_load2(row_ptr(a.L(), (uint32_t)__builtin_amdgcn_readlane((int)mine, 2)), pi, valid);
         double q0 = x.x + U.gs * (x.x - rz.x), q1 = x.y + U.gs * (x.y - rz.y);
         q0 = q0 + en0; q1 = q1 + en1;
         p0 = (j0 < U.dim) ? q0 : x.x;
@@ -174,11 +174,11 @@
     if (!FUSED && lane == 0) a.ids_buf[w] = (int32_t)c;
     const uint32_t li = c - a.lo;
     WideUni U;
-    U.dim = a.L.dim; U.ld = a.L.ld; U.P = NP > 0 ? (uint32_t)NP : a.P;
+    U.dim = a.L().dim; U.ld = a.L().ld; U.P = NP > 0 ? (uint32_t)NP : a.P;
     U.thr = 65536u; U.forced = U.dim; U.epsilon = a.epsilon; U.u_epsilon = a.u_epsilon; U.snk = 0; U.gs = 0.0;
     const uint32_t npairs = (U.dim + 1u) >> 1;
     const uint32_t n_chunks = (npairs + WIDE_CHUNK_PAIRS - 1u) / WIDE_CHUNK_PAIRS;
-    const double* xrow = row_ptr(a.L, c);
+    const double* xrow = row_ptr(a.L(), c);
     const u32x4 h0 = chain_block(a.seed, c, a.t, SLOT_HDR0);
     const bool snk_possible = !DREAM && a.p_snooker > 0.0 && a.M >= 3;
     const uint32_t npart = 2u * U.P + (snk_possible ? 3u : 0u);
@@ -235,9 +235,9 @@
     }
     double sn_n2 = 0.0;
     if (snk_possible && u_sel < a.p_snooker) {
-        const double* zrow = row_ptr(a.L, (uint32_t)__builtin_amdgcn_readlane((int)mine, 2));
-        const double* r1row = row_ptr(a.L, (uint32_t)__builtin_amdgcn_readlane((int)mine, 3));
-        const double* r2row = row_ptr(a.L, (uint32_t)__builtin_amdgcn_readlane((int)mine, 4));
+        const double* zrow = row_ptr(a.L(), (uint32_t)__builtin_amdgcn_readlane((int)mine, 2));
+        const double* r1row = row_ptr(a.L(), (uint32_t)__builtin_amdgcn_readlane((int)mine, 3));
+        const double* r2row = row_ptr(a.L(), (uint32_t)__builtin_amdgcn_readlane((int)mine, 4));
         double n2 = 0.0, dot = 0.0;
 #pragma unroll 1
         for (uint32_t k = 0; k < n_chunks; ++k) {
@@ -261,7 +261,7 @@
     const double* m2row = a.w_m2 + (uint32_t)(li * 2u * U.ld);
     double* hrow = (FUSED && a.hist_row) ? a.hist_row + (uint32_t)(li * U.ld) : nullptr;
     double* prow = FUSED ? nullptr : a.prop_buf + (uint64_t)w * U.ld;
-    const double* zrow_b = U.snk ? row_ptr(a.L, (uint32_t)__builtin_amdgcn_readlane((int)mine, 2)) : xrow;
+    const double* zrow_b = U.snk ? row_ptr(a.L(), (uint32_t)__builtin_amdgcn_readlane((int)mine, 2)) : xrow;
 #pragma unroll 1
     for (uint32_t k = 0; k < n_chunks; ++k) {
 #pragma unroll
@@ -311,8 +311,8 @@
         if (lane == 0) {
             a.aux_buf[w] = log_corr;
             if (DREAM) {
-                *delta_ptr(a.L, c) = cr_stat ? delta : 0.0;
-                *cridx_ptr(a.L, c) = cr_stat ? (double)cr_idx : -1.0;
+                *delta_ptr(a.L(), c) = cr_stat ? delta : 0.0;
+                *cridx_ptr(a.L(), c) = cr_stat ? (double)cr_idx : -1.0;
             }
         }
         return;
@@ -333,14 +333,14 @@
         if (a.llhist_row) a.llhist_row[li] = new_ll;
         if (DREAM && a.adapt_on) {
             if (a.wt) {
-                __hip_atomic_store(delta_ptr(a.L, c), cr_stat ? delta : 0.0, __ATOMIC_RELAXED, __HIP_MEMORY_SCOPE_AGENT);
-                __hip_atomic_store(cridx_ptr(a.L, c), cr_stat ? (double)cr_idx : -1.0, __ATOMIC_RELAXED, __HIP_MEMORY_SCOPE_AGENT);
+                __hip_atomic_store(delta_ptr(a.L(), c), cr_stat ? delta : 0.0, __ATOMIC_RELAXED, __HIP_MEMORY_SCOPE_AGENT);
+                __hip_atomic_store(cridx_ptr(a.L(), c), cr_stat ? (double)cr_idx : -1.0, __ATOMIC_RELAXED, __HIP_MEMORY_SCOPE_AGENT);
             } else {
-                *delta_ptr(a.L, c) = cr_stat ? delta : 0.0;
-                *cridx_ptr(a.L, c) = cr_stat ? (double)cr_idx : -1.0;
+                *delta_ptr(a.L(), c) = cr_stat ? delta : 0.0;
+                *cridx_ptr(a.L(), c) = cr_stat ? (double)cr_idx : -1.0;
             }
             if (a.n_peers && a.adapt_on && a.cr_gate) {
-                const uint32_t d_off = (uint32_t)(delta_ptr(a.L, c) - a.L.G), c_off = (uint32_t)(cridx_ptr(a.L, c) - a.L.G);
+                const uint32_t d_off = (uint32_t)(delta_ptr(a.L(), c) - a.L().G), c_off = (uint32_t)(cridx_ptr(a.L(), c) - a.L().G);
 #pragma unroll 1
                 for (uint32_t p = 0; p < a.n_peers; ++p) {
                     double* pg = reinterpret_cast<double*>(a.peer_tab[p]);
@@ -358,11 +358,11 @@
     }
     const bool welford = DREAM && a.adapt_on;
     if (accepted || welford || a.x_next) {
-        double* srow = row_ptr(a.L, c);
+        double* srow = row_ptr(a.L(), c);
         double* nrow = a.x_next ? a.x_next + (uint32_t)(li * U.ld) : nullptr;
         double* wm = a.w_mean + (uint32_t)(li * 2u * U.ld);
         double* w2 = a.w_m2 + (uint32_t)(li * 2u * U.ld);
-        const uint32_t row_off = (uint32_t)(srow - a.L.G);
+        const uint32_t row_off = (uint32_t)(srow - a.L().G);
         const double cntp = (double)(a.hist_len + 1);
 #pragma unroll 1
         for (uint32_t k = 0; k < n_chunks; ++k) {
@@ -418,9 +418,9 @@
     const int32_t id = a.ids_buf[w];
     if (id < 0) return;
     const uint32_t c = (uint32_t)__builtin_amdgcn_readfirstlane(id), li = c - a.lo;
-    const uint32_t dim = a.L.dim, ld = a.L.ld, npairs = (dim + 1u) >> 1;
+    const uint32_t dim = a.L().dim, ld = a.L().ld, npairs = (dim + 1u) >> 1;
     const uint32_t n_chunks = (npairs + WIDE_CHUNK_PAIRS - 1u) / WIDE_CHUNK_PAIRS;
-    const double ll_cur = a.ll[li], ll_prop = a.aux_buf[a.L.n_local + w], log_corr = a.aux_buf[w];
+    const double ll_cur = a.ll[li], ll_prop = a.aux_buf[a.L().n_local + w], log_corr = a.aux_buf[w];
     const uint32_t acc_prev = a.acc_count[li];
     const u32x4 h0 = chain_block(a.seed, c, a.t, SLOT_HDR0);
     const double d_acc = (ll_prop + log_corr) - ll_cur;
@@ -435,11 +435,11 @@
             trace_i32_of(a)[(uint64_t)li * TRACE_I32 + 3] = accepted ? 1 : 0;
             double* tf = trace_f64_of(a) + (uint64_t)li * TRACE_F64;
             bool nan_alpha;
-            tf[0] = accept_alpha(d_acc, &nan_alpha); tf[1] = ll_prop; tf[2] = DREAM ? *delta_ptr(a.L, c) : 0.0; tf[3] = 0.0;
+            tf[0] = accept_alpha(d_acc, &nan_alpha); tf[1] = ll_prop; tf[2] = DREAM ? *delta_ptr(a.L(), c) : 0.0; tf[3] = 0.0;
         }
     }
     const bool welford = DREAM && a.adapt_on;
-    double* srow = row_ptr(a.L, c);
+    double* srow = row_ptr(a.L(), c);
     const double* prow = a.prop_buf + (uint64_t)w * ld;
     double* hrow = a.hist_row ? a.hist_row + (uint32_t)(li * ld) : nullptr;
     double* nrow = a.x_next ? a.x_next + (uint32_t)(li * ld) : nullptr;
diff --git a/bipymc_amd/csrc/sampler.hip b/bipymc_amd/csrc/sampler.hip
--- a/bipymc_amd/csrc/sampler.hip
+++ b/bipymc_amd/csrc/sampler.hip
@@ -227,6 +227,17 @@
     PhaseArgs a;
 };
 static_assert(offsetof(FusedKernarg, a) == 24 && sizeof(FusedKernarg) == 24 + sizeof(PhaseArgs), "kernarg layout of phase_fused_kernel");
+#define BPM_HOT_AT(field, off) static_assert(offsetof(PhaseArgs, field) == (off), "hot block of PhaseArgs: " #field)
+BPM_HOT_AT(L_G, 0); BPM_HOT_AT(L_ld, 8); BPM_HOT_AT(L_dim, 12); BPM_HOT_AT(ll, 16); BPM_HOT_AT(acc_count, 24); BPM_HOT_AT(tparams, 32); BPM_HOT_AT(counters, 40);
+BPM_HOT_AT(hist_row, 48); BPM_HOT_AT(llhist_row, 56); BPM_HOT_AT(seed, 64); BPM_HOT_AT(t, 72); BPM_HOT_AT(k, 80); BPM_HOT_AT(upd_off, 84); BPM_HOT_AT(epsilon, 88);
+BPM_HOT_AT(wt, 96); BPM_HOT_AT(hist_by_pos, 100);
+BPM_HOT_AT(cr_state, 104); BPM_HOT_AT(gamma_tab, 112); BPM_HOT_AT(u_epsilon, 120); BPM_HOT_AT(w_mean, 128); BPM_HOT_AT(w_m2, 136); BPM_HOT_AT(cr_gate, 144);
+BPM_HOT_AT(hist_len, 148); BPM_HOT_AT(thr, 152);
+BPM_HOT_AT(L_blk, 184); BPM_HOT_AT(L_n_local, 192); BPM_HOT_AT(L_world, 196); BPM_HOT_AT(L_magic, 200); BPM_HOT_AT(lo, 204);
+BPM_HOT_AT(gamma_demc, 208); BPM_HOT_AT(p_snooker, 216); BPM_HOT_AT(M, 224); BPM_HOT_AT(pool_off, 228);
+#undef BPM_HOT_AT
+static_assert((offsetof(FusedKernarg, a) + offsetof(PhaseArgs, thr) + 4 * sizeof(uint32_t)) % 64 == 0 && (offsetof(FusedKernarg, a) + offsetof(PhaseArgs, pool_off) + sizeof(uint32_t)) % 64 == 0 &&
+              bpm::DirectQueue::SLOT_BYTES % 64 == 0, "the hot block's lines 2 and 3 end on lines of the kernarg segment");
 static inline void update_packet(Dispatch& d, const bpm::DqKernel* k, unsigned grid, unsigned block, const void* ka, size_t nbytes) {
     int fence = d.update_fence;
     const int sig = d.sig;
@@ -1522,7 +1533,7 @@
     for (int ph = 0; ph < 2; ++ph) {
         PhaseArgs& a = s->cur_args[ph];
         std::memset(&a, 0, sizeof(a));
-        a.L = s->L;
+        a.set_L(s->L);
         a.ll = s->ll;
         a.hist_row = hist_row;
         a.llhist_row = llhist_row;
```

Result: faster. 894.2 million (median of 6 runs) (+5.8%).
